# NuTufts/ubresnet

Hardware: AMD Instinct MI355X
Metric: images/sec, 512x512 U-ResNet train step (fwd+loss+bwd+Adam) (higher is better)
Workload: dtype bf16; 1 GPU; ub_uresnet 3-class ip16 bf16, batch 16 per GPU (global 16), 512x512x1 synthetic LArTPC crops, Adam(1e-5, wd 1e-4); parallelism=dp1, global_batch=16, optimizer=ubresnet_amd.optim.FlatAdam

## Files before the change

include/ubresnet_hip.h:

```cpp
#ifndef UBRESNET_HIP_H
#define UBRESNET_HIP_H

#include <stdint.h>

#ifdef __cplusplus
extern "C" {
#endif

#define UBR_F32 0
#define UBR_BF16 1
#define UBR_F16 2

#define UBR_OK 0
#define UBR_EINVAL (-1)
#define UBR_ELAUNCH (-2)

#define UBR_MAX_TAPS 64
#define UBR_STAT_SLOTS 32
#define UBR_RED_SLOTS 8

typedef struct {
  void* p;
  int64_t sn, sy, sx;
} ubr_tensor;

typedef struct {
  const float* sub;
  const float* scale;
  const float* shift;
  const float* lo;
} ubr_chan_affine;

typedef struct {
  int32_t dtype;
  int32_t N, H, W, Cin;
  ubr_tensor x;
  ubr_chan_affine xf;
  const void* w;
  int32_t Cout, Cout_pad;
  int32_t ntaps;
  int8_t dy[UBR_MAX_TAPS], dx[UBR_MAX_TAPS];
  uint8_t wt[UBR_MAX_TAPS];
  int32_t S, iy0, ix0;
  int32_t OH, OW;
  ubr_tensor y;
  ubr_tensor addend;
  const float* bias;
  double* stats;
  int32_t epilogue;
  int32_t tile_hint;
  int32_t act;
  int32_t pad_;
  const uint8_t* addend_mask;
  ubr_tensor bnb_c;
  const float *bnb_mean, *bnb_scale, *bnb_shift, *bnb_invstd;
  int32_t nphase;
  int32_t phase_tap0[4], phase_ntaps[4];
  int32_t pad3_;
  int64_t phase_yoff[4], phase_aoff[4];
  int32_t stats_slots;
  int32_t pad2_;
} ubr_conv_desc;

int ubr_conv(const ubr_conv_desc* d, void* stream);
void ubr_conv_last_config(int* fw, int* nt, int* twf, int* pipe);
int ubr_conv_last_kernel(char* buf, int n);

int ubr_pack_weights(int dtype, const float* src, void* dst, int M, int Mpad, int Kvalid, int Kpad,
                     int64_t sm, int64_t sk, int ntaps, const int32_t* tapidx_host, void* stream);

typedef struct {
  const float* src;
  void* dst;
  int64_t sm, sk, tap_stride;
  const float* oscale;
  int32_t M, Mpad, Kvalid, KU, ntaps, pad_;
} ubr_pack_item;
int ubr_pack_weights_batched(int dtype, const ubr_pack_item* items_dev, int nitems, void* stream);

typedef struct {
  const float *gamma, *beta, *running_mean, *running_var;
  const float* conv_bias;
  float *scale, *bias;
  int32_t C;
  float eps;
} ubr_bn_fold_item;
int ubr_bn_fold_batched(const ubr_bn_fold_item* items_dev, int nitems, void* stream);

typedef struct {
  int32_t dtype;
  int32_t N, H, W, C;
  int32_t pad_;
  ubr_tensor x;
  const void* w;
  const float* bias;
  ubr_tensor y;
} ubr_aspp_front_desc;
int ubr_aspp_front(const ubr_aspp_front_desc* d, void* stream);

typedef struct {
  int32_t dtype;
  int32_t N, H, W, Cin;
  ubr_tensor x;
  ubr_chan_affine xf;
  int32_t GH, GW, Cout;
  ubr_tensor g;
  int32_t ntaps;
  int8_t dy[UBR_MAX_TAPS], dx[UBR_MAX_TAPS];
  int32_t S, iy0, ix0;
  float* slabs;
  int32_t nsplit;
  int32_t exclusive;
} ubr_wgrad_desc;

int ubr_wgrad_plan(const ubr_wgrad_desc* d, int32_t* nsplit, int64_t* workspace_bytes);
int ubr_wgrad(const ubr_wgrad_desc* d, void* stream);
void ubr_wgrad_last_config(int* ma, int* nb, int* tpg, int* nsplit_mode, int* bigx);
int ubr_wgrad_last_pc(void);
int ubr_wgrad_reduce(float* slabs , int nsplit, int ntaps, int Cout_pad, int Cin,
                     int Cout_valid, int Cin_valid, float* dst, int64_t sm, int64_t sk,
                     const int32_t* tapidx_host, int accumulate, void* stream);
#define UBR_REDUCE_BATCH 16
typedef struct {
  float* slabs;
  float* dst;
  int32_t nsplit, ntaps, Cout_pad, Cin, Cout_valid, Cin_valid, accumulate, pad_;
  int64_t sm, sk;
  int32_t tapidx[UBR_MAX_TAPS];
} ubr_wgrad_reduce_item;
int ubr_wgrad_reduce_batched(const ubr_wgrad_reduce_item* items_host, int nitems, void* stream);

int ubr_stem_forward(int dtype, const float* x_nchw, int N, int Cin, int H, int W,
                     const float* weight , const float* bias, int Cout,
                     ubr_tensor y, double* stats, void* stream);
int ubr_stem_wgrad(int dtype, const float* x_nchw, int N, int Cin, int H, int W, ubr_tensor g, int Cout,
                   float* partial , int64_t partial_bytes, float* dweight, float* dbias,
                   int accumulate, void* stream);
int64_t ubr_stem_wgrad_workspace(int N, int Cin, int H, int W, int Cout);
int ubr_stem_expand(int dtype, const float* x_nchw, int N, int Cin, int H, int W, void* out, int64_t out_ps, void* stream);

int ubr_bn_finalize(const double* stats, double count, const float* gamma, const float* beta,
                    float* running_mean, float* running_var, int64_t* num_batches_tracked,
                    float momentum, float eps, int C,
                    float* scale, float* shift, float* mean, float* invstd, void* stream);
int ubr_bn_eval_affine(const float* gamma, const float* beta, const float* running_mean,
                       const float* running_var, float eps, int C, float* scale, float* shift,
                       float* mean, float* invstd, void* stream);

int ubr_bn_bwd_reduce(int dtype, int64_t npix, int C, const void* ga, int64_t ga_ps, const void* ga2, int64_t ga2_ps,
                      const void* c, int64_t c_ps, const float* scale, const float* shift, const float* mean,
                      const float* invstd, int relu, double* red, void* stream);
int ubr_bn_bwd_finalize(const double* red, double count, const float* scale , const float* invstd,
                        int C, float* dgamma, float* dbeta, int accumulate, float* k1, float* k2, void* stream);
int ubr_bn_bwd_apply(int dtype, int64_t npix, int C, const void* ga, int64_t ga_ps, const void* ga2, int64_t ga2_ps,
                     const void* c, int64_t c_ps, const float* scale, const float* shift, const float* mean,
                     const float* invstd, int relu, const float* k1, const float* k2,
                     void* gc, int64_t gc_ps, void* stream);

int ubr_bn_bwd_apply_fin(int dtype, int64_t npix, int C, const void* ga, int64_t ga_ps, const void* ga2, int64_t ga2_ps,
                         const void* c, int64_t c_ps, const float* scale, const float* shift, const float* mean,
                         const float* invstd, int relu, const double* red, double count, float* dgamma, float* dbeta,
                         void* gc, int64_t gc_ps, void* stream);

int ubr_block_tail_fwd(int dtype, int64_t npix, int C, const void* c2, int64_t c2_ps, const float* mean2,
                       const float* scale2, const float* shift2, const void* sc, int64_t sc_ps, const float* mean_b,
                       const float* scale_b, const float* shift_b ,
                       void* out, int64_t out_ps, void* stream);
int ubr_block_tail_bwd_reduce(int dtype, int64_t npix, int C, const void* go, int64_t go_ps, const void* go2, int64_t go2_ps,
                              const void* out, int64_t out_ps, const void* c2, int64_t c2_ps,
                              const float* scale2, const float* shift2, const float* mean2, const float* invstd2,
                              const void* cb, int64_t cb_ps, const float* mean_b, const float* invstd_b,
                              double* red2, double* red_b, void* stream);
int ubr_block_tail_bwd_apply(int dtype, int64_t npix, int C, const void* go, int64_t go_ps, const void* go2, int64_t go2_ps,
                             const void* out, int64_t out_ps, const void* c2, int64_t c2_ps,
                             const float* scale2, const float* shift2, const float* mean2, const float* invstd2,
                             const float* k1_2, const float* k2_2,
                             const void* cb, int64_t cb_ps, const float* scale_b, const float* mean_b, const float* invstd_b,
                             const float* k1_b, const float* k2_b,
                             void* g_c2, int64_t g_c2_ps, void* g_sc, int64_t g_sc_ps, void* stream);

typedef struct {
  const double* stats;
  const float *gamma, *beta;
  float *running_mean, *running_var; int64_t* num_batches_tracked;
  float momentum, eps;
  float *scale, *shift, *mean, *invstd;
} ubr_bn_fwd_fin;
int ubr_block_tail_fwd_fin(int dtype, int64_t npix, int C, const void* c2, int64_t c2_ps, const ubr_bn_fwd_fin* bn2,
                           const void* sc, int64_t sc_ps, const ubr_bn_fwd_fin* bn_b, double count,
                           void* out, int64_t out_ps, uint8_t* relu_mask, void* stream);

int ubr_block_tail_fwd_masked(int dtype, int64_t npix, int C, const void* c2, int64_t c2_ps, const float* mean2,
                              const float* scale2, const float* shift2, const void* sc, int64_t sc_ps, const float* mean_b,
                              const float* scale_b, const float* shift_b, void* out, int64_t out_ps, uint8_t* relu_mask, void* stream);
int ubr_block_tail_bwd_reduce_masked(int dtype, int64_t npix, int C, const void* go, int64_t go_ps, const void* go2, int64_t go2_ps,
                                     const uint8_t* relu_mask, const void* c2, int64_t c2_ps,
                                     const float* scale2, const float* shift2, const float* mean2, const float* invstd2,
                                     const void* cb, int64_t cb_ps, const float* mean_b, const float* invstd_b,
                                     double* red2, double* red_b, void* stream);
int ubr_block_tail_bwd_apply_masked(int dtype, int64_t npix, int C, const void* go, int64_t go_ps, const void* go2, int64_t go2_ps,
                                    const uint8_t* relu_mask, const void* c2, int64_t c2_ps,
                                    const float* scale2, const float* shift2, const float* mean2, const float* invstd2,
                                    const float* k1_2, const float* k2_2,
                                    const void* cb, int64_t cb_ps, const float* scale_b, const float* mean_b, const float* invstd_b,
                                    const float* k1_b, const float* k2_b,
                                    void* g_c2, int64_t g_c2_ps, void* g_sc, int64_t g_sc_ps, void* stream);

int ubr_block_tail_bwd_apply_fin(int dtype, int64_t npix, int C, const void* go, int64_t go_ps, const void* go2, int64_t go2_ps,
                                 const uint8_t* relu_mask, const void* c2, int64_t c2_ps,
                                 const float* scale2, const float* shift2, const float* mean2, const float* invstd2,
                                 const double* red2, float* dgamma2, float* dbeta2,
                                 const void* cb, int64_t cb_ps, const float* scale_b, const float* mean_b, const float* invstd_b,
                                 const double* red_b, float* dgamma_b, float* dbeta_b, double count,
                                 void* g_c2, int64_t g_c2_ps, void* g_sc, int64_t g_sc_ps, void* stream);

int ubr_bn_bwd_frozen(int dtype, int64_t npix, int C, const void* ga, int64_t ga_ps, const void* ga2, int64_t ga2_ps,
                      const void* c, int64_t c_ps, const float* scale, const float* shift, const float* mean,
// ... 63 lines not shown
```

ubresnet_amd/_lib.py:

```python
from __future__ import annotations

import ctypes as C
import os
import threading

import torch

HERE = os.path.dirname(os.path.abspath(__file__))
LIB_PATH = os.environ.get("UBR_LIB", os.path.join(HERE, "libubresnet_hip.so"))

F32, BF16, F16 = 0, 1, 2
MAX_TAPS = 64
MAX_TILES = 64
STAT_SLOTS = 32
RED_SLOTS = 8
_DT = {torch.float32: F32, torch.bfloat16: BF16, torch.float16: F16}
_CPU = {F32: 4, BF16: 8, F16: 8}


def dtype_id(dt: torch.dtype) -> int:
    try:
        return _DT[dt]
    except KeyError:
        raise RuntimeError("ubresnet_amd: unsupported compute dtype %s" % dt)


def chans_per_unit(dt: torch.dtype) -> int:
    return _CPU[dtype_id(dt)]


class Tensor(C.Structure):
    _fields_ = [("p", C.c_void_p), ("sn", C.c_int64), ("sy", C.c_int64), ("sx", C.c_int64)]


class ChanAffine(C.Structure):
    _fields_ = [("sub", C.c_void_p), ("scale", C.c_void_p), ("shift", C.c_void_p), ("lo", C.c_void_p)]


class ConvDesc(C.Structure):
    _fields_ = [
        ("dtype", C.c_int32),
        ("N", C.c_int32), ("H", C.c_int32), ("W", C.c_int32), ("Cin", C.c_int32),
        ("x", Tensor),
        ("xf", ChanAffine),
        ("w", C.c_void_p),
        ("Cout", C.c_int32), ("Cout_pad", C.c_int32),
        ("ntaps", C.c_int32),
        ("dy", C.c_int8 * MAX_TAPS), ("dx", C.c_int8 * MAX_TAPS),
        ("wt", C.c_uint8 * MAX_TAPS),
        ("S", C.c_int32), ("iy0", C.c_int32), ("ix0", C.c_int32),
        ("OH", C.c_int32), ("OW", C.c_int32),
        ("y", Tensor),
        ("addend", Tensor),
        ("bias", C.c_void_p),
        ("stats", C.c_void_p),
        ("epilogue", C.c_int32),
        ("tile_hint", C.c_int32),
        ("act", C.c_int32),
        ("pad_", C.c_int32),
        ("addend_mask", C.c_void_p),
        ("bnb_c", Tensor),
        ("bnb_mean", C.c_void_p), ("bnb_scale", C.c_void_p), ("bnb_shift", C.c_void_p), ("bnb_invstd", C.c_void_p),
        ("nphase", C.c_int32), ("phase_tap0", C.c_int32 * 4), ("phase_ntaps", C.c_int32 * 4), ("pad3_", C.c_int32),
        ("phase_yoff", C.c_int64 * 4), ("phase_aoff", C.c_int64 * 4),
        ("stats_slots", C.c_int32), ("pad2_", C.c_int32),
    ]


class AsppFrontDesc(C.Structure):
    _fields_ = [
        ("dtype", C.c_int32),
        ("N", C.c_int32), ("H", C.c_int32), ("W", C.c_int32), ("C", C.c_int32),
        ("pad_", C.c_int32),
        ("x", Tensor),
        ("w", C.c_void_p),
        ("bias", C.c_void_p),
        ("y", Tensor),
    ]


class BnFwdFin(C.Structure):
    _fields_ = [
        ("stats", C.c_void_p), ("gamma", C.c_void_p), ("beta", C.c_void_p),
        ("running_mean", C.c_void_p), ("running_var", C.c_void_p), ("num_batches_tracked", C.c_void_p),
        ("momentum", C.c_float), ("eps", C.c_float),
        ("scale", C.c_void_p), ("shift", C.c_void_p), ("mean", C.c_void_p), ("invstd", C.c_void_p),
    ]


REDUCE_BATCH = 16


class WgradReduceItem(C.Structure):
    _fields_ = [
        ("slabs", C.c_void_p), ("dst", C.c_void_p),
        ("nsplit", C.c_int32), ("ntaps", C.c_int32), ("Cout_pad", C.c_int32), ("Cin", C.c_int32),
        ("Cout_valid", C.c_int32), ("Cin_valid", C.c_int32), ("accumulate", C.c_int32), ("pad_", C.c_int32),
        ("sm", C.c_int64), ("sk", C.c_int64),
        ("tapidx", C.c_int32 * 64),
    ]


class WgradDesc(C.Structure):
    _fields_ = [
        ("dtype", C.c_int32),
        ("N", C.c_int32), ("H", C.c_int32), ("W", C.c_int32), ("Cin", C.c_int32),
        ("x", Tensor),
        ("xf", ChanAffine),
        ("GH", C.c_int32), ("GW", C.c_int32), ("Cout", C.c_int32),
        ("g", Tensor),
        ("ntaps", C.c_int32),
        ("dy", C.c_int8 * MAX_TAPS), ("dx", C.c_int8 * MAX_TAPS),
        ("S", C.c_int32), ("iy0", C.c_int32), ("ix0", C.c_int32),
        ("slabs", C.c_void_p),
        ("nsplit", C.c_int32),
        ("exclusive", C.c_int32),
    ]


SYMBOLS = [
    "ubr_conv", "ubr_conv_last_config", "ubr_conv_last_kernel", "ubr_pack_weights", "ubr_pack_weights_batched", "ubr_bn_fold_batched", "ubr_aspp_front", "ubr_wgrad_plan", "ubr_wgrad", "ubr_wgrad_last_config", "ubr_wgrad_last_pc", "ubr_wgrad_reduce", "ubr_wgrad_reduce_batched",
    "ubr_stem_forward", "ubr_stem_wgrad", "ubr_stem_wgrad_workspace", "ubr_stem_expand",
    "ubr_bn_finalize", "ubr_bn_eval_affine", "ubr_bn_bwd_reduce", "ubr_bn_bwd_finalize", "ubr_bn_bwd_apply",
    "ubr_block_tail_fwd", "ubr_block_tail_bwd_reduce", "ubr_block_tail_bwd_apply",
    "ubr_block_tail_fwd_masked", "ubr_block_tail_bwd_reduce_masked", "ubr_block_tail_bwd_apply_masked",
    "ubr_bn_bwd_apply_fin", "ubr_block_tail_bwd_apply_fin", "ubr_block_tail_fwd_fin",
    "ubr_bn_bwd_frozen", "ubr_block_tail_bwd_frozen", "ubr_bn_bwd_finalize_frozen",
    "ubr_maxpool_fwd", "ubr_maxpool_bwd",
    "ubr_logsoftmax_bwd", "ubr_pixelwise_nll_fwd", "ubr_pixelwise_nll_bwd", "ubr_confusion",
    "ubr_channel_sum", "ubr_cast_f64_to_f32", "ubr_zero", "ubr_adam_step", "ubr_sgd_step", "ubr_crop_tiles", "ubr_stitch_tiles", "ubr_last_error", "ubr_version",
    "ubr_tape_create", "ubr_tape_destroy", "ubr_tape_begin", "ubr_tape_end", "ubr_tape_pause", "ubr_tape_fork", "ubr_tape_mark",
    "ubr_tape_wait_mark", "ubr_tape_size", "ubr_tape_replay", "ubr_tape_set_label", "ubr_tape_replay_timed",
]

_lib = None
_lock = threading.Lock()
vp, i32, i64, f32, f64 = C.c_void_p, C.c_int32, C.c_int64, C.c_float, C.c_double


def _declare(lib):
    lib.ubr_last_error.restype = C.c_char_p
    lib.ubr_version.restype = C.c_int
    lib.ubr_stem_wgrad_workspace.restype = C.c_int64
    lib.ubr_stem_wgrad_workspace.argtypes = [i32] * 5
    lib.ubr_conv.argtypes = [C.POINTER(ConvDesc), vp]
    lib.ubr_conv_last_config.argtypes = [C.POINTER(C.c_int)] * 4
    lib.ubr_conv_last_kernel.argtypes = [C.c_char_p, i32]
    lib.ubr_conv_last_config.restype = None
    lib.ubr_wgrad_last_config.argtypes = [C.POINTER(C.c_int)] * 5
    lib.ubr_wgrad_last_config.restype = None
    lib.ubr_wgrad_last_pc.argtypes = []
    lib.ubr_wgrad_last_pc.restype = C.c_int
    lib.ubr_pack_weights.argtypes = [i32, vp, vp, i32, i32, i32, i32, i64, i64, i32, C.POINTER(C.c_int32), vp]
    lib.ubr_pack_weights_batched.argtypes = [i32, vp, i32, vp]
    lib.ubr_bn_fold_batched.argtypes = [vp, i32, vp]
    lib.ubr_aspp_front.argtypes = [C.POINTER(AsppFrontDesc), vp]
    lib.ubr_wgrad_plan.argtypes = [C.POINTER(WgradDesc), C.POINTER(C.c_int32), C.POINTER(C.c_int64)]
    lib.ubr_wgrad.argtypes = [C.POINTER(WgradDesc), vp]
    lib.ubr_wgrad_reduce.argtypes = [vp, i32, i32, i32, i32, i32, i32, vp, i64, i64, C.POINTER(C.c_int32), i32, vp]
    lib.ubr_wgrad_reduce_batched.argtypes = [C.POINTER(WgradReduceItem), i32, vp]
    lib.ubr_stem_forward.argtypes = [i32, vp, i32, i32, i32, i32, vp, vp, i32, Tensor, vp, vp]
    lib.ubr_stem_wgrad.argtypes = [i32, vp, i32, i32, i32, i32, Tensor, i32, vp, i64, vp, vp, i32, vp]
    lib.ubr_stem_expand.argtypes = [i32, vp, i32, i32, i32, i32, vp, i64, vp]
    lib.ubr_bn_finalize.argtypes = [vp, f64, vp, vp, vp, vp, vp, f32, f32, i32, vp, vp, vp, vp, vp]
    lib.ubr_bn_eval_affine.argtypes = [vp, vp, vp, vp, f32, i32, vp, vp, vp, vp, vp]
    lib.ubr_bn_bwd_reduce.argtypes = [i32, i64, i32, vp, i64, vp, i64, vp, i64, vp, vp, vp, vp, i32, vp, vp]
    lib.ubr_bn_bwd_finalize.argtypes = [vp, f64, vp, vp, i32, vp, vp, i32, vp, vp, vp]
    lib.ubr_bn_bwd_apply.argtypes = [i32, i64, i32, vp, i64, vp, i64, vp, i64, vp, vp, vp, vp, i32, vp, vp, vp, i64, vp]
    lib.ubr_bn_bwd_apply_fin.argtypes = [i32, i64, i32, vp, i64, vp, i64, vp, i64, vp, vp, vp, vp, i32, vp, f64, vp, vp, vp, i64, vp]
    lib.ubr_block_tail_bwd_apply_fin.argtypes = [i32, i64, i32, vp, i64, vp, i64, vp, vp, i64, vp, vp, vp, vp, vp, vp, vp,
                                                 vp, i64, vp, vp, vp, vp, vp, vp, f64, vp, i64, vp, i64, vp]
    lib.ubr_bn_bwd_frozen.argtypes = [i32, i64, i32, vp, i64, vp, i64, vp, i64, vp, vp, vp, vp, i32, vp, vp, i64, vp]
    lib.ubr_block_tail_bwd_frozen.argtypes = [i32, i64, i32, vp, i64, vp, i64, vp, vp, i64, vp, vp, vp, vp, vp,
                                              vp, i64, vp, vp, vp, vp, vp, i64, vp, i64, vp]
    lib.ubr_bn_bwd_finalize_frozen.argtypes = [vp, i32, vp, vp, vp, vp, vp]
    lib.ubr_block_tail_fwd_fin.argtypes = [i32, i64, i32, vp, i64, C.POINTER(BnFwdFin), vp, i64, C.POINTER(BnFwdFin), f64, vp, i64, vp, vp]
    lib.ubr_block_tail_fwd.argtypes = [i32, i64, i32, vp, i64, vp, vp, vp, vp, i64, vp, vp, vp, vp, i64, vp]
    lib.ubr_block_tail_fwd_masked.argtypes = [i32, i64, i32, vp, i64, vp, vp, vp, vp, i64, vp, vp, vp, vp, i64, vp, vp]
    lib.ubr_block_tail_bwd_reduce_masked.argtypes = [i32, i64, i32, vp, i64, vp, i64, vp, vp, i64, vp, vp, vp, vp, vp, i64, vp, vp, vp, vp, vp]
    lib.ubr_block_tail_bwd_apply_masked.argtypes = [i32, i64, i32, vp, i64, vp, i64, vp, vp, i64, vp, vp, vp, vp, vp, vp, vp, i64, vp, vp, vp, vp, vp,
                                                    vp, i64, vp, i64, vp]
    lib.ubr_block_tail_bwd_reduce.argtypes = [i32, i64, i32, vp, i64, vp, i64, vp, i64, vp, i64, vp, vp, vp, vp,
                                              vp, i64, vp, vp, vp, vp, vp]
    lib.ubr_block_tail_bwd_apply.argtypes = [i32, i64, i32, vp, i64, vp, i64, vp, i64, vp, i64, vp, vp, vp, vp, vp, vp,
                                             vp, i64, vp, vp, vp, vp, vp, vp, i64, vp, i64, vp]
    lib.ubr_maxpool_fwd.argtypes = [i32, i32, i32, i32, i32, i32, vp, i64, ChanAffine, vp, i64, vp, i64, vp, vp]
    lib.ubr_maxpool_bwd.argtypes = [i32, i32, i32, i32, i32, i32, vp, i64, ChanAffine, vp, i64, vp, i64, vp, i64, vp, vp]
    lib.ubr_logsoftmax_bwd.argtypes = [i32, i32, i32, i32, i32, vp, vp, vp, i64, vp]
    lib.ubr_pixelwise_nll_fwd.argtypes = [vp, vp, vp, vp, i32, i32, i32, i32, i64, vp, vp, vp]
    lib.ubr_pixelwise_nll_bwd.argtypes = [vp, vp, vp, vp, i32, i32, i32, i32, i64, vp, vp]
    lib.ubr_confusion.argtypes = [vp, vp, i32, i32, i32, i32, vp, vp]
    lib.ubr_channel_sum.argtypes = [i32, i64, i32, vp, i64, vp, vp]
    lib.ubr_cast_f64_to_f32.argtypes = [vp, i32, i32, vp, i32, f64, i32, vp]
    lib.ubr_zero.argtypes = [vp, i64, vp]
    lib.ubr_adam_step.argtypes = [vp, vp, vp, vp, i64, f32, f32, f32, f32, f32, i64, f32, vp]
    lib.ubr_sgd_step.argtypes = [vp, vp, vp, i64, f32, f32, f32, f32, i32, i32, f32, vp]
    lib.ubr_crop_tiles.argtypes = [vp, i32, i32, i32, C.POINTER(C.c_int32), i32, i32, i32, vp, vp]
    lib.ubr_stitch_tiles.argtypes = [vp, i32, i32, i32, C.POINTER(C.c_int32), i32, vp, i32, i32, i32, vp]
    lib.ubr_tape_create.argtypes = []
    lib.ubr_tape_create.restype = vp
    lib.ubr_tape_destroy.argtypes = [vp]
    lib.ubr_tape_destroy.restype = None
    lib.ubr_tape_begin.argtypes = [vp, i32, C.POINTER(vp)]
    lib.ubr_tape_end.argtypes = [vp]
    lib.ubr_tape_pause.argtypes = [vp, i32]
    lib.ubr_tape_fork.argtypes = [vp, i32, i32]
    lib.ubr_tape_mark.argtypes = [vp, i32]
    lib.ubr_tape_wait_mark.argtypes = [vp, i32, vp]
    lib.ubr_tape_size.argtypes = [vp]
    lib.ubr_tape_replay.argtypes = [vp, i32, C.POINTER(vp)]
    lib.ubr_tape_set_label.argtypes = [vp, i32]
    lib.ubr_tape_replay_timed.argtypes = [vp, i32, C.POINTER(vp), C.POINTER(C.c_float), C.POINTER(C.c_int32), i32]
    for name in SYMBOLS:
        fn = getattr(lib, name)
        if name not in ("ubr_last_error", "ubr_version", "ubr_stem_wgrad_workspace", "ubr_conv_last_config", "ubr_wgrad_last_config",
                        "ubr_tape_create", "ubr_tape_destroy"):
            fn.restype = C.c_int


def lib():
    global _lib
    if _lib is None:
        with _lock:
            if _lib is None:
                if not os.path.exists(LIB_PATH):
                    raise RuntimeError(
                        "ubresnet_amd: HIP extension %s is missing; build it with "
                        "`python -m ubresnet_amd.build` (hipcc, gfx950). There is no CPU fallback." % LIB_PATH)
                try:
                    l = C.CDLL(LIB_PATH)
                except OSError as e:
                    raise RuntimeError("ubresnet_amd: cannot load %s: %s" % (LIB_PATH, e))
                _declare(l)
                _lib = l
    return _lib


def check(rc: int, what: str = ""):
    if rc != 0:
        msg = lib().ubr_last_error().decode("utf-8", "replace")
        raise RuntimeError("ubresnet_amd HIP call failed (%d) %s: %s" % (rc, what, msg))


_raw_stream = getattr(torch._C, "_cuda_getCurrentRawStream", None)


def stream_ptr() -> int:
    if _raw_stream is not None:
        return _raw_stream(torch.cuda.current_device())
    return torch.cuda.current_stream().cuda_stream


def require_cuda(t: torch.Tensor, what: str):
    if not t.is_cuda:
        raise RuntimeError("ubresnet_amd: %s must live on a ROCm device (got %s); the HIP path has no CPU fallback"
                           % (what, t.device))


def ptr(t):
    return None if t is None else t.data_ptr()
```

ubresnet_amd/csrc/ubr_conv.hip:

```cpp
#include <stdlib.h>
#include <type_traits>
#include "ubr_common.h"
#include "ubr_host.h"

namespace {

struct ConvK {
  const char* x; long x_sn, x_sy, x_sx;
  const float *in_sub, *in_scale, *in_shift, *in_lo;
  const char* w;
  char* y; long y_sn, y_sy, y_sx;
  const char* ad; long a_sn, a_sy, a_sx;
  const float* bias;
  double* stats;
  int H, W;
  int CU, UPB, lgUPB, nblk;
  int Cout, Cout_pad;
  int ntaps, S, iy0, ix0, OH, OW;
  int dymin, dxmin, HH, HW;
  int tiles_x, tiles_y;
  unsigned tx_magic, ty_magic;
  int nunits, steps;
  int pixb;
  unsigned rw, rw_magic;
  int x_sy32, x_sx32;
  int step_j, step_hy, step_goff, wrap_goff;
  int wl_off, halo_off, red_off, xfc_off;
  int epilogue, act, wide_store, dbg, wlinear, N;
  int buf_stride, ncot;
  const uint8_t* ad_mask; int ad_mask_cu;
  const char* bc; long bc_sn, bc_sy, bc_sx;
  const float *bmean, *bscale, *bshift, *binvstd;
  int nslots;
  int pair_store;
  int fast_epi;
  int ptap0[4], pnunits[4], psteps[4];
  long pyoff[4], paoff[4];
  int8_t dy[UBR_MAX_TAPS], dx[UBR_MAX_TAPS];
  uint8_t wt[UBR_MAX_TAPS];
  unsigned long long* stamps;
};

template <typename T> __device__ __forceinline__ void store4(char* p, const float* v);
template <> __device__ __forceinline__ void store4<float>(char* p, const float* v) {
  *reinterpret_cast<float4*>(p) = make_float4(v[0], v[1], v[2], v[3]);
}
template <> __device__ __forceinline__ void store4<bf16_t>(char* p, const float* v) {
  *reinterpret_cast<uint2*>(p) = make_uint2(ET<bf16_t>::pk2(v[0], v[1]), ET<bf16_t>::pk2(v[2], v[3]));
}
template <> __device__ __forceinline__ void store4<f16_t>(char* p, const float* v) {
  f16x4_t h; h[0] = (_Float16)v[0]; h[1] = (_Float16)v[1]; h[2] = (_Float16)v[2]; h[3] = (_Float16)v[3];
  *reinterpret_cast<uint2*>(p) = __builtin_bit_cast(uint2, h);
}
template <typename T> __device__ __forceinline__ void load4(const char* p, float* v);
template <> __device__ __forceinline__ void load4<float>(const char* p, float* v) {
  float4 f = *reinterpret_cast<const float4*>(p); v[0] = f.x; v[1] = f.y; v[2] = f.z; v[3] = f.w;
}
template <> __device__ __forceinline__ void load4<bf16_t>(const char* p, float* v) {
  uint2 u = *reinterpret_cast<const uint2*>(p);
  v[0] = __uint_as_float(u.x << 16); v[1] = __uint_as_float(u.x & 0xffff0000u);
  v[2] = __uint_as_float(u.y << 16); v[3] = __uint_as_float(u.y & 0xffff0000u);
}
template <> __device__ __forceinline__ void load4<f16_t>(const char* p, float* v) {
  f16x4_t h = __builtin_bit_cast(f16x4_t, *reinterpret_cast<const uint2*>(p));
  v[0] = (float)h[0]; v[1] = (float)h[1]; v[2] = (float)h[2]; v[3] = (float)h[3];
}

template <typename T> __device__ __forceinline__ void round4(const float* v, float* r);
template <> __device__ __forceinline__ void round4<float>(const float* v, float* r) { r[0] = v[0]; r[1] = v[1]; r[2] = v[2]; r[3] = v[3]; }
template <> __device__ __forceinline__ void round4<bf16_t>(const float* v, float* r) {
#pragma unroll
  for (int i = 0; i < 4; ++i) {
    const uint32_t u = __float_as_uint(v[i]);
    const uint32_t rne = (u + 0x7fffu + ((u >> 16) & 1u)) & 0xffff0000u;
    r[i] = __uint_as_float((u & 0x7fffffffu) > 0x7f800000u ? (u | 0x00400000u) & 0xffff0000u : rne);
  }
}
template <> __device__ __forceinline__ void round4<f16_t>(const float* v, float* r) {
#pragma unroll
  for (int i = 0; i < 4; ++i) r[i] = (float)(_Float16)v[i];
}
__device__ __forceinline__ void bnb_accumulate(const float* g, const float* c, const float4& mu, const float4& sc, const float4& sh, const float4& is,
                                               float* s1, float* s2) {
  const float m[4] = {mu.x, mu.y, mu.z, mu.w}, a[4] = {sc.x, sc.y, sc.z, sc.w}, b[4] = {sh.x, sh.y, sh.z, sh.w}, iv[4] = {is.x, is.y, is.z, is.w};
#pragma unroll
  for (int r = 0; r < 4; ++r) {
    const float d = c[r] - m[r];
    const float bn = __builtin_fmaf(d, a[r], b[r]);
    const float xh = d * iv[r];
    const float gy = bn > 0.f ? g[r] : 0.f;
    s1[r] += gy;
    s2[r] += gy * xh;
  }
}

__host__ __device__ constexpr int conv_pixb(int upb) { return upb == 2 ? 32 : upb * 16 + 16; }

#ifndef UBR_THIN_PIXB4
#define UBR_THIN_PIXB4 80
#endif
__host__ __device__ constexpr int thin_pixb(int upb) { return upb == 4 ? UBR_THIN_PIXB4 : conv_pixb(upb); }

__host__ __device__ constexpr int conv_pipe_hslots(int fw, int twf) { return ((4 * fw / twf + 2) * (twf * 16 + 2) * 4 + 255) / 256; }
__host__ __device__ constexpr int conv_pipe_wslots(int nt) { return (36 * nt * 16 + 255) / 256; }

template <typename T> __device__ __forceinline__ uint4 pack_swap_pair(const float* v0, const float* v1);
template <> __device__ __forceinline__ uint4 pack_swap_pair<bf16_t>(const float* v0, const float* v1) {
  uint2 X, Y;
  asm volatile("v_cvt_pk_bf16_f32 %0, %4, %5\n\tv_cvt_pk_bf16_f32 %1, %6, %7\n\tv_cvt_pk_bf16_f32 %2, %8, %9\n\t"
               "v_cvt_pk_bf16_f32 %3, %10, %11\n\ts_nop 1\n\tv_permlane16_swap_b32 %0, %2\n\tv_permlane16_swap_b32 %1, %3\n\ts_nop 3"
               : "=&v"(X.x), "=&v"(X.y), "=&v"(Y.x), "=&v"(Y.y)
               : "v"(v0[0]), "v"(v0[1]), "v"(v0[2]), "v"(v0[3]), "v"(v1[0]), "v"(v1[1]), "v"(v1[2]), "v"(v1[3]));
  return make_uint4(X.x, X.y, Y.x, Y.y);
}
template <> __device__ __forceinline__ uint4 pack_swap_pair<f16_t>(const float* v0, const float* v1) {
  f16x4_t a, b;
#pragma unroll
  for (int r = 0; r < 4; ++r) { a[r] = (_Float16)v0[r]; b[r] = (_Float16)v1[r]; }
  uint2 X = __builtin_bit_cast(uint2, a), Y = __builtin_bit_cast(uint2, b);
  asm volatile("s_nop 1\n\tv_permlane16_swap_b32 %0, %1\n\tv_permlane16_swap_b32 %2, %3\n\ts_nop 3" : "+v"(X.x), "+v"(Y.x), "+v"(X.y), "+v"(Y.y));
  return make_uint4(X.x, X.y, Y.x, Y.y);
}
template <> __device__ __forceinline__ uint4 pack_swap_pair<float>(const float* v0, const float* v1) { return make_uint4(0u, 0u, 0u, 0u); }

template <typename T> __device__ __forceinline__ void store_frag_pair(char* p0, char* p1, bool ok0, bool ok1, const float* v0, const float* v1, int q) {
  if constexpr (std::is_same<T, float>::value) {
    if (ok0) store4<float>(p0, v0);
    if (ok1) store4<float>(p1, v1);
  } else {
    const uint4 v = pack_swap_pair<T>(v0, v1);
    const bool odd = (q & 1) != 0;
    char* p = odd ? (p1 - 8) : p0;
    if (odd ? ok1 : ok0) *reinterpret_cast<uint4*>(p) = v;
  }
}

typedef __attribute__((ext_vector_type(2))) unsigned ubr_u2;
__device__ __forceinline__ unsigned udiv_magic(unsigned n, unsigned magic) { return magic == 0u ? n : __umulhi(n, magic); }

__device__ __forceinline__ void buf_store16(const ubr_u4& v, __amdgpu_buffer_rsrc_t r, int voff, int soff) {
  __builtin_amdgcn_raw_buffer_store_b128(v, r, voff + soff, 0, 0);
}

template <typename T, int FW, int NT, int TWF, bool PIPE>
__global__ __launch_bounds__(256, ((NT == 4 && FW <= 2 && !PIPE) ? 4 : 2)) void conv_igemm_kernel(const ConvK k) {
  ubr_main_prio();
  constexpr int TN = NT * 16;
  constexpr int F = 4 * FW;
  constexpr int TH = F / TWF;
  constexpr int TW = TWF * 16;
  constexpr int CPU = ET<T>::CPU;
  constexpr int ESZ = 16 / CPU;
  static_assert(F % TWF == 0, "tile shape");

  extern __shared__ __attribute__((aligned(16))) char smem[];
  int* tbl = reinterpret_cast<int*>(smem);
  char* wl = smem + k.wl_off;
  char* halo = smem + k.halo_off;
  float* red = reinterpret_cast<float*>(smem + k.red_off);

#ifdef UBR_CONV_STAMPS
  const unsigned long long t_entry = __builtin_amdgcn_s_memtime();
#endif
  const int tid = threadIdx.x, lane = tid & 63, wave = tid >> 6, q = lane >> 4, l16 = lane & 15;
  const int ph = blockIdx.z;
  const int tap0 = k.ptap0[ph], p_nunits = k.pnunits[ph], p_steps = k.psteps[ph];
  char* const yb = k.y + k.pyoff[ph];
  const char* const adb = k.ad != nullptr ? k.ad + k.paoff[ph] : nullptr;
  const unsigned tile_l = blockIdx.x;
  const unsigned tile_r = udiv_magic(tile_l, k.tx_magic);
  const int tx = (int)(tile_l - tile_r * (unsigned)k.tiles_x);
  const int n = (int)udiv_magic(tile_r, k.ty_magic);
  const int ty = (int)(tile_r - (unsigned)n * (unsigned)k.tiles_y);
  const int n0 = blockIdx.y * TN;
  const int tb_tap = min(tap0 + (tid >> k.lgUPB), k.ntaps - 1);
  const int tb_dy = k.dy[tb_tap], tb_dx = k.dx[tb_tap], tb_wt = k.wt[tb_tap];
  const int oy0 = ty * TH, ox0 = tx * TW;
  const int hy0 = oy0 * k.S + k.iy0 + k.dymin, hx0 = ox0 * k.S + k.ix0 + k.dxmin;

  constexpr int HS_P = PIPE ? conv_pipe_hslots(FW, TWF) : 1;
  constexpr int kOOR = (int)0x80000000;
  ubr_u4 hv[HS_P];
  int hoff[HS_P];
  unsigned hok = 0u;
  float xfr[PIPE ? 8 : 1];
  const bool xf_early = PIPE && k.in_scale != nullptr && k.CU * ET<T>::CPU <= 512;
  if constexpr (PIPE) {
    const int c = tid & (k.UPB - 1);
    const int nit = k.HH * (int)k.rw;
    int hy = (int)__umulhi((unsigned)tid, k.rw_magic);
    int j = tid - hy * (int)k.rw;
#pragma unroll
    for (int u = 0; u < HS_P; ++u) {
// ... 374 lines not shown
#pragma unroll
  for (int j = 0; j < NT; ++j) {
    const int ch = n0 + j * 16 + 4 * q;
    float4 bmu = make_float4(0.f, 0.f, 0.f, 0.f), bsc = bmu, bsh = bmu, bis = bmu;
    const bool bnb = k.bc != nullptr && ch < k.Cout;
    if (bnb) {
      bmu = *reinterpret_cast<const float4*>(k.bmean + ch); bsc = *reinterpret_cast<const float4*>(k.bscale + ch);
      bsh = *reinterpret_cast<const float4*>(k.bshift + ch); bis = *reinterpret_cast<const float4*>(k.binvstd + ch);
    }
    auto finish = [&](int i, float* v, int& oy, int& ox) -> bool {
      const int f = wave * FW + i;
      oy = oy0 + f / TWF; ox = ox0 + (f % TWF) * 16 + l16;
      const bool valid = (oy < k.OH) && (ox < k.OW);
#pragma unroll
      for (int r = 0; r < 4; ++r) v[r] = acc[i][j][r] + bs[j][r];
      if (k.act & 1) {
#pragma unroll
        for (int r = 0; r < 4; ++r) v[r] = fmaxf(v[r], 0.f);
      }
      if (adb != nullptr && valid && ch < k.Cout) {
        float a4[4];
        load4<T>(adb + (long)n * k.a_sn + (long)oy * k.a_sy + (long)ox * k.a_sx + (long)ch * ESZ, a4);
        if (k.ad_mask != nullptr) {
          const unsigned mb = (unsigned)k.ad_mask[(((long)n * k.OH + oy) * k.OW + ox) * k.ad_mask_cu + ch / CPU] >> (ch % CPU);
#pragma unroll
          for (int r = 0; r < 4; ++r) a4[r] = ((mb >> r) & 1u) ? a4[r] : 0.f;
        }
#pragma unroll
        for (int r = 0; r < 4; ++r) v[r] += a4[r];
      }
      if (k.act & 2) {
#pragma unroll
        for (int r = 0; r < 4; ++r) v[r] = fmaxf(v[r], 0.f);
      }
      if (k.stats != nullptr && valid) {
        if (k.bc != nullptr) {
          if (bnb) {
            float g4[4], c4[4];
            round4<T>(v, g4);
            load4<T>(k.bc + (long)n * k.bc_sn + (long)oy * k.bc_sy + (long)ox * k.bc_sx + (long)ch * ESZ, c4);
            bnb_accumulate(g4, c4, bmu, bsc, bsh, bis, s1[j], s2[j]);
          }
        } else {
#pragma unroll
          for (int r = 0; r < 4; ++r) { s1[j][r] += v[r]; s2[j][r] += v[r] * v[r]; }
        }
      }
      return valid;
    };
    constexpr bool PAIRS = (FW % 2 == 0) && sizeof(T) == 2;
    if (PAIRS && k.pair_store && k.epilogue == 0) {
#pragma unroll
      for (int i = 0; i < FW; i += 2) {
        float v0[4], v1[4];
        int oy_a, ox_a, oy_b, ox_b;
        const bool ok0 = finish(i, v0, oy_a, ox_a) && ch < k.Cout;
        const bool ok1 = finish(i + (FW > 1 ? 1 : 0), v1, oy_b, ox_b) && ch < k.Cout;
        store_frag_pair<T>(yb + (long)n * k.y_sn + (long)oy_a * k.y_sy + (long)ox_a * k.y_sx + (long)ch * ESZ,
                           yb + (long)n * k.y_sn + (long)oy_b * k.y_sy + (long)ox_b * k.y_sx + (long)ch * ESZ, ok0, ok1, v0, v1, q);
      }
    } else {
#pragma unroll
    for (int i = 0; i < FW; ++i) {
      float v[4];
      int oy, ox;
      const bool valid = finish(i, v, oy, ox);
      if (k.epilogue == 0) {
        if (valid && ch < k.Cout)
          store4<T>(yb + (long)n * k.y_sn + (long)oy * k.y_sy + (long)ox * k.y_sx + (long)ch * ESZ, v);
      } else if (j == 0) {
        float m = -3.0e38f;
#pragma unroll
        for (int r = 0; r < 4; ++r) if (ch + r < k.Cout) m = fmaxf(m, v[r]);
        m = fmaxf(m, __shfl_xor(m, 16, 64));
        m = fmaxf(m, __shfl_xor(m, 32, 64));
        float e = 0.f;
#pragma unroll
        for (int r = 0; r < 4; ++r) if (ch + r < k.Cout) e += expf(v[r] - m);
        e += __shfl_xor(e, 16, 64);
        e += __shfl_xor(e, 32, 64);
        const float lse = m + logf(e);
        if (valid) {
          float* o = reinterpret_cast<float*>(k.y);
#pragma unroll
          for (int r = 0; r < 4; ++r)
            if (ch + r < k.Cout) o[(((long)n * k.Cout + ch + r) * k.OH + oy) * k.OW + ox] = v[r] - lse;
        }
      }
    }
    }
  }

#ifdef UBR_CONV_STAMPS
  const unsigned long long te1 = __builtin_amdgcn_s_memtime();
#endif
  if (k.stats != nullptr) {
#pragma unroll
    for (int j = 0; j < NT; ++j)
#pragma unroll
      for (int r = 0; r < 4; ++r) {
        const float a = wave_quadrow_sum16(s1[j][r]);
        const float b = wave_quadrow_sum16(s2[j][r]);
        if (l16 == 0) {
          red[(wave * TN + j * 16 + 4 * q + r) * 2 + 0] = a;
          red[(wave * TN + j * 16 + 4 * q + r) * 2 + 1] = b;
        }
      }
    __syncthreads();
    if (tid < TN) {
      const int ch = n0 + tid;
      if (ch < k.Cout) {
        double a = 0.0, b = 0.0;
#pragma unroll
        for (int w = 0; w < 4; ++w) { a += (double)red[(w * TN + tid) * 2]; b += (double)red[(w * TN + tid) * 2 + 1]; }
        double* st = k.stats + (size_t)(blockIdx.x % k.nslots) * 2 * k.Cout;
        atomicAdd(&st[ch], a);
        atomicAdd(&st[k.Cout + ch], b);
      }
    }
  }
#ifdef UBR_CONV_STAMPS
  if (PIPE && k.stamps != nullptr) {
    const unsigned long long te2 = __builtin_amdgcn_s_memtime();
    __syncthreads();
    if (tid == 0) {
      unsigned long long* o = k.stamps + ((size_t)blockIdx.y * gridDim.x + blockIdx.x) * 16;
      o[9] = __builtin_amdgcn_s_memtime(); o[11] = te0; o[12] = te1; o[13] = te2;
    }
  }
#endif
}

struct ThinK {
  const char* x; long x_sn; int x_sy, x_sx; unsigned x_bytes;
  const float *in_sub, *in_scale, *in_shift, *in_lo;
  const char* w;
  char* y; long y_sn; int y_sy, y_sx; unsigned y_bytes;
  const char* ad; long a_sn; int a_sy, a_sx; unsigned a_bytes;
  const float* bias; double* stats;
  int H, W, HW, nitems; unsigned hw_magic;
  int tiles_x, tiles_y, ntiles; unsigned tx_magic, ty_magic;
  int steps, nunits, hy_org, hx_org, dymin, dxmin;
  int Cout, Cout_pad, CU, OH, OW;
  int act, epilogue, wlinear, dbg;
  int wl_off, halo_off, red_off;
  int8_t dy[UBR_MAX_TAPS], dx[UBR_MAX_TAPS];
  uint8_t wt[UBR_MAX_TAPS];
  unsigned long long* stamps;
  const uint8_t* ad_mask; int ad_mask_cu; unsigned mask_bytes;
  const char* bc; long bc_sn; int bc_sy, bc_sx; unsigned bc_bytes;
  const float *bmean, *bscale, *bshift, *binvstd;
  int nslots;
  int nphase, pstep0[4], psteps[4], pyoff[4];
};


template <typename T, int FW, int NT, int TWF, int UPB, bool XF, bool LSM, bool ROW7 = false, int EXT = 0>
__global__ __launch_bounds__(256, ((ROW7 || (EXT == 1 && NT == 2)) ? 2 : 3)) void conv_thin_kernel(const ThinK k) {
  ubr_main_prio();
  static_assert(EXT == 0 || (!XF && !LSM), "the training epilogues belong to the data-gradient convs (no transform on load, NHWC output)");
  constexpr int TN = NT * 16;
  constexpr int TH = 4 * FW / TWF;
  constexpr int TW = TWF * 16;
  constexpr int CPU = ET<T>::CPU;
  constexpr int ESZ = 16 / CPU;
  constexpr int LG = UPB == 4 ? 2 : (UPB == 2 ? 1 : 0);
  constexpr int PIXB = thin_pixb(UPB);
  constexpr int HS = ROW7 ? 7 : (UPB == 4 ? 6 : 5);
  constexpr int PPS = 256 / UPB;
  constexpr int WB = 4;
  constexpr int FH = ROW7 ? 8 : 4;
  static_assert(TWF == 2 && FW % FH == 0, "tile shape");
  static_assert(!ROW7 || (FW == 8 && NT == 1 && UPB == 2), "ROW7 is the 16x32-pixel, 16-cout, 16-cin tile");
  constexpr bool WIDE = ESZ == 2;

  extern __shared__ __attribute__((aligned(16))) char smem[];
  int* tbl = reinterpret_cast<int*>(smem);
  char* wl = smem + k.wl_off;
  char* halo = smem + k.halo_off;
  float* red = reinterpret_cast<float*>(smem + k.red_off);

  const int tid = threadIdx.x, lane = tid & 63, wave = tid >> 6, q = lane >> 4, l16 = lane & 15;
  const int n0 = blockIdx.y * TN;
  const int c = tid & (UPB - 1);
  const int nw = 4 * k.steps * TN;

  int hxu[HS], relu[HS];
  int hyu[XF ? HS : 1];
#pragma unroll
  for (int u = 0; u < HS; ++u) {
    const int pix = (tid >> LG) + u * PPS;
    const int hy = (int)udiv_magic((unsigned)pix, k.hw_magic), hx = pix - hy * k.HW;
    const bool in = tid + u * 256 < k.nitems;
    hxu[u] = in ? hx : -(1 << 24);
    relu[u] = hy * k.x_sy + hx * k.x_sx + c * 16;
    if constexpr (XF) hyu[u] = hy;
  }
  char* const halo_w = halo + (tid >> LG) * PIXB + c * 16;

  ubr_u4 hv[HS];
  unsigned hok = 0u;
  auto load_halo = [&](int tile) {
    const unsigned t = (unsigned)__builtin_amdgcn_readfirstlane(tile);
    const unsigned r = udiv_magic(t, k.tx_magic), tx = t - r * (unsigned)k.tiles_x;
    const unsigned n = udiv_magic(r, k.ty_magic), ty = r - n * (unsigned)k.tiles_y;
    const int hy0 = (int)ty * TH + k.hy_org, hx0 = (int)tx * TW + k.hx_org;
    __amdgpu_buffer_rsrc_t xr = __builtin_amdgcn_make_buffer_rsrc((void*)(k.x + (long)n * k.x_sn), 0, (int)k.x_bytes, 0x00020000);
    const int goff = hy0 * k.x_sy + hx0 * k.x_sx;
    hok = 0u;
#pragma unroll
    for (int u = 0; u < HS; ++u) {
      const bool ok = (unsigned)(hx0 + hxu[u]) < (unsigned)k.W;
      int vo = ok ? relu[u] + goff : -1;
      if (k.dbg & 1) vo = -1;
      hv[u] = __builtin_amdgcn_raw_buffer_load_b128(xr, vo, 0, 0);
      if constexpr (XF) hok |= (unsigned)(ok & ((unsigned)(hy0 + hyu[u]) < (unsigned)k.H)) << u;
    }
  };

  const int ntiles = k.ntiles;
  int tile = blockIdx.x;
  load_halo(tile);
  uint4 wv[WB];
  if (k.wlinear) {
    const int nvalid = k.nunits * TN;
#pragma unroll
    for (int u = 0; u < WB; ++u) {
      const int i = tid + u * 256;
      wv[u] = make_uint4(0u, 0u, 0u, 0u);
      if (i < nvalid) wv[u] = ldg16(k.w + (long)i * 16);
    }
  }
  float bs[NT][4];
#pragma unroll
  for (int j = 0; j < NT; ++j)
#pragma unroll
    for (int r = 0; r < 4; ++r) {
      const int ch = n0 + j * 16 + 4 * q + r;
      bs[j][r] = (k.bias != nullptr && ch < k.Cout) ? k.bias[ch] : 0.f;
    }
  float* xfc = red + 4 * TN * 2;
  if constexpr (XF) {
    for (int i = tid; i < 4 * UPB * CPU; i += 256) {
      const int which = i / (UPB * CPU), ch = i - which * (UPB * CPU);
      const float* src = which == 0 ? k.in_sub : (which == 1 ? k.in_scale : (which == 2 ? k.in_shift : k.in_lo));
      xfc[i] = src[ch];
    }
  }
  if constexpr (EXT == 1) {
    for (int i = tid; i < 4 * TN; i += 256) {
      const int which = i / TN, ch = n0 + (i - which * TN);
      const float* src = which == 0 ? k.bmean : (which == 1 ? k.bscale : (which == 2 ? k.bshift : k.binvstd));
      xfc[i] = ch < k.Cout ? src[ch] : 0.f;
    }
  }
  int* wsrc = tbl + 4 * k.steps;
  for (int u = tid; u < 4 * k.steps; u += 256) {
    int off = 0, v = -1;
    if (u < k.nunits) {
      const int tap = u >> LG, cc = u & (UPB - 1);
      off = ((k.dy[tap] - k.dymin) * k.HW + (k.dx[tap] - k.dxmin)) * PIXB + cc * 16;
      v = k.wt[tap] == 255 ? -1 : ((int)k.wt[tap] * k.CU + cc) * k.Cout_pad;
    }
    tbl[u] = off;
    wsrc[u] = v;
  }
  if (k.wlinear) {
#pragma unroll
    for (int u = 0; u < WB; ++u) {
      const int i = tid + u * 256;
      if (i < nw) *reinterpret_cast<uint4*>(wl + (long)i * 16) = wv[u];
    }
    const int nvalid = k.nunits * TN;
    for (int ib = tid + 256 * WB; ib < nw; ib += 256 * WB) {
#pragma unroll
      for (int u = 0; u < WB; ++u) {
        const int i = ib + u * 256;
        wv[u] = make_uint4(0u, 0u, 0u, 0u);
        if (i < nvalid) wv[u] = ldg16(k.w + (long)i * 16);
      }
#pragma unroll
      for (int u = 0; u < WB; ++u) {
        const int i = ib + u * 256;
        if (i < nw) *reinterpret_cast<uint4*>(wl + (long)i * 16) = wv[u];
      }
    }
  } else {
    __syncthreads();
    for (int ib = tid; ib < nw; ib += 256 * WB) {
#pragma unroll
      for (int u = 0; u < WB; ++u) {
        const int i = ib + u * 256;
        wv[u] = make_uint4(0u, 0u, 0u, 0u);
        if (i < nw) {
          const int src = wsrc[i / TN];
          if (src >= 0) wv[u] = ldg16(k.w + ((long)(src + n0 + (i % TN))) * 16);
        }
      }
#pragma unroll
      for (int u = 0; u < WB; ++u) {
        const int i = ib + u * 256;
        if (i < nw) *reinterpret_cast<uint4*>(wl + (long)i * 16) = wv[u];
      }
    }
  }

  if constexpr (XF || EXT == 1) __syncthreads();
  const int fb0 = (((wave * FW) / TWF) * k.HW + l16) * PIXB;
  const int rowb = k.HW * PIXB;
  int vo_out[NT];
#pragma unroll
  for (int j = 0; j < NT; ++j) {
    if constexpr (WIDE) vo_out[j] = ((wave * FW) / TWF) * k.y_sy + ((q & 1) * 16 + l16) * k.y_sx + (n0 + j * 16 + 8 * (q >> 1)) * ESZ;
    else vo_out[j] = ((wave * FW) / TWF) * k.y_sy + l16 * k.y_sx + (n0 + j * 16 + 4 * q) * ESZ;
  }
  int vo_ad[NT];
#pragma unroll
  for (int j = 0; j < NT; ++j) vo_ad[j] = ((wave * FW) / TWF) * k.a_sy + l16 * k.a_sx + (n0 + j * 16 + 4 * q) * ESZ;
  int vo_c[EXT == 1 ? NT : 1], vo_m[EXT == 2 ? NT : 1];
  if constexpr (EXT == 1) {
#pragma unroll
    for (int j = 0; j < NT; ++j) vo_c[j] = ((wave * FW) / TWF) * k.bc_sy + l16 * k.bc_sx + (n0 + j * 16 + 4 * q) * ESZ;
  }
  if constexpr (EXT == 2) {
#pragma unroll
    for (int j = 0; j < NT; ++j) vo_m[j] = (((wave * FW) / TWF) * k.OW + l16) * k.ad_mask_cu + (n0 + j * 16 + 4 * q) / CPU;
  }
  float s1[NT][4], s2[NT][4];
#pragma unroll
  for (int j = 0; j < NT; ++j)
#pragma unroll
    for (int r = 0; r < 4; ++r) { s1[j][r] = 0.f; s2[j][r] = 0.f; }

#ifdef UBR_CONV_STAMPS
  unsigned long long tS = 0, tL = 0, tC = 0, tE = 0, tB = 0, tW = 0, t_ = __builtin_amdgcn_s_memtime();
  const unsigned long long t_begin = t_;
#define UBR_TSTAMP(acc_) do { unsigned long long n_ = __builtin_amdgcn_s_memtime(); acc_ += n_ - t_; t_ = n_; } while (0)
#else
#define UBR_TSTAMP(acc_) do { } while (0)
#endif
  while (tile < ntiles) {
#ifdef UBR_CONV_STAMPS
    asm volatile("s_waitcnt vmcnt(0)" ::: "memory");
    UBR_TSTAMP(tW);
#endif
    float xsub[XF ? CPU : 1], xsc[XF ? CPU : 1], xsh[XF ? CPU : 1], xlo[XF ? CPU : 1];
    if constexpr (XF) {
#pragma unroll
      for (int e = 0; e < CPU; ++e) {
        xsub[e] = xfc[0 * UPB * CPU + c * CPU + e]; xsc[e] = xfc[1 * UPB * CPU + c * CPU + e];
        xsh[e] = xfc[2 * UPB * CPU + c * CPU + e]; xlo[e] = xfc[3 * UPB * CPU + c * CPU + e];
      }
    }
#pragma unroll
    for (int u = 0; u < HS; ++u) {
      uint4 v = __builtin_bit_cast(uint4, hv[u]);
      if constexpr (XF) {
        if ((hok >> u) & 1u) {
          float f[CPU];
          ET<T>::unpack(v, f);
          ubr_bnrelu<CPU>(f, xsub, xsc, xsh, xlo);
          v = ET<T>::pack(f);
        }
      }
      if (tid + u * 256 < k.nitems) *reinterpret_cast<uint4*>(halo_w + u * (PPS * PIXB)) = v;
    }
    UBR_TSTAMP(tS);
    __syncthreads();
    UBR_TSTAMP(tB);
    const unsigned t = (unsigned)__builtin_amdgcn_readfirstlane(tile);
    const unsigned rr = udiv_magic(t, k.tx_magic), tx = t - rr * (unsigned)k.tiles_x;
    const unsigned n = udiv_magic(rr, k.ty_magic), ty = rr - n * (unsigned)k.tiles_y;
    const int oy0 = (int)ty * TH, ox0 = (int)tx * TW;
    const int next = tile + gridDim.x;
    if (next < ntiles) load_halo(next);
    __amdgpu_buffer_rsrc_t yr = __builtin_amdgcn_make_buffer_rsrc((void*)(k.y + (long)n * k.y_sn), 0, (int)k.y_bytes, 0x00020000);
    __amdgpu_buffer_rsrc_t ar = __builtin_amdgcn_make_buffer_rsrc((void*)(k.ad != nullptr ? k.ad + (long)n * k.a_sn : k.x), 0, k.ad != nullptr ? (int)k.a_bytes : 0, 0x00020000);
    const int ybase = oy0 * k.y_sy + ox0 * k.y_sx, abase = oy0 * k.a_sy + ox0 * k.a_sx;
    __amdgpu_buffer_rsrc_t cr = yr, mr = yr;
    int cbase = 0, mbase = 0;
    if constexpr (EXT == 1) {
      cr = __builtin_amdgcn_make_buffer_rsrc((void*)(k.bc + (long)n * k.bc_sn), 0, (int)k.bc_bytes, 0x00020000);
      cbase = oy0 * k.bc_sy + ox0 * k.bc_sx;
    }
    if constexpr (EXT == 2) {
      mr = __builtin_amdgcn_make_buffer_rsrc((void*)(k.ad_mask + (long)n * k.mask_bytes), 0, (int)k.mask_bytes, 0x00020000);
      mbase = (oy0 * k.OW + ox0) * k.ad_mask_cu;
    }
    UBR_TSTAMP(tL);

#pragma unroll 1
    for (int g0 = 0; g0 < FW; g0 += FH) {
      ubr_u4 adv4[FH][NT];
      ubr_u2 adv2[FH][NT];
      if (k.ad != nullptr) {
#pragma unroll
        for (int i = 0; i < FH; ++i)
#pragma unroll
          for (int j = 0; j < NT; ++j) {
            const int so = abase + ((g0 + i) / TWF) * k.a_sy;
            if constexpr (WIDE) adv2[i][j] = __builtin_amdgcn_raw_buffer_load_b64(ar, vo_ad[j] + (i % TWF) * 16 * k.a_sx, so, 0);
            else adv4[i][j] = __builtin_amdgcn_raw_buffer_load_b128(ar, vo_ad[j] + (i % TWF) * 16 * k.a_sx, so, 0);
          }
      }
      unsigned admk[EXT == 2 ? FH : 1][EXT == 2 ? NT : 1];
      ubr_u4 cv4[EXT == 1 ? FH : 1][EXT == 1 ? NT : 1];
      ubr_u2 cv2[EXT == 1 ? FH : 1][EXT == 1 ? NT : 1];
      if constexpr (EXT == 2) {
#pragma unroll
        for (int i = 0; i < FH; ++i)
#pragma unroll
          for (int j = 0; j < NT; ++j)
            admk[i][j] = __builtin_amdgcn_raw_buffer_load_b8(mr, vo_m[j] + (i % TWF) * 16 * k.ad_mask_cu, mbase + ((g0 + i) / TWF) * k.OW * k.ad_mask_cu, 0);
      }
      if constexpr (EXT == 1) {
#pragma unroll
        for (int i = 0; i < FH; ++i)
#pragma unroll
          for (int j = 0; j < NT; ++j) {
            const int so = cbase + ((g0 + i) / TWF) * k.bc_sy;
            if constexpr (WIDE) cv2[i][j] = __builtin_amdgcn_raw_buffer_load_b64(cr, vo_c[j] + (i % TWF) * 16 * k.bc_sx, so, 0);
            else cv4[i][j] = __builtin_amdgcn_raw_buffer_load_b128(cr, vo_c[j] + (i % TWF) * 16 * k.bc_sx, so, 0);
          }
      }
      const int nph = (ROW7 || LSM || EXT != 0) ? 1 : k.nphase;
#pragma unroll 1
      for (int ph = 0; ph < nph; ++ph) {
      const int s_lo = nph > 1 ? k.pstep0[ph] : 0;
      const int s_cnt = nph > 1 ? k.psteps[ph] : k.steps;
      const int y_ph = nph > 1 ? k.pyoff[ph] : 0;
      f32x4 acc[FH][NT];
#pragma unroll
      for (int i = 0; i < FH; ++i)
#pragma unroll
        for (int j = 0; j < NT; ++j) acc[i][j] = f32x4{0.f, 0.f, 0.f, 0.f};
      const char* hb = halo + fb0 + (g0 / TWF) * rowb;
      if constexpr (ROW7) {
        constexpr int ROWB = (TW + 6) * PIXB;
#pragma unroll 1
        for (int pp = 0; pp < 4; ++pp) {
          const char* pb = hb + tbl[4 * pp + q];
          const char* pw = wl + ((4 * pp + q) * TN + l16) * 16;
          uint4 w7[7];
#pragma unroll
          for (int dy = 0; dy < 7; ++dy) w7[dy] = *reinterpret_cast<const uint4*>(pw + dy * (16 * TN * 16));
#pragma unroll
          for (int ir = 0; ir < 10; ++ir) {
            const uint4 b0 = *reinterpret_cast<const uint4*>(pb + ir * ROWB);
            const uint4 b1 = *reinterpret_cast<const uint4*>(pb + ir * ROWB + 16 * PIXB);
#pragma unroll
            for (int r = 0; r < 4; ++r) {
              const int dy = ir - r;
              if (dy >= 0 && dy <= 6) {
                acc[2 * r][0] = mma_step<T>(acc[2 * r][0], w7[dy], b0);
                acc[2 * r + 1][0] = mma_step<T>(acc[2 * r + 1][0], w7[dy], b1);
              }
            }
          }
        }
      } else {
      int off_n = tbl[4 * s_lo + q];
      uint4 wf_n[NT];
#pragma unroll
      for (int j = 0; j < NT; ++j) wf_n[j] = *reinterpret_cast<const uint4*>(wl + (((4 * s_lo + q) * TN) + j * 16 + l16) * 16);
      const int nsteps = s_lo + ((k.dbg & 2) ? 1 : s_cnt);
      for (int s = s_lo; s < nsteps; ++s) {
        const char* pa = hb + off_n;
        uint4 wf[NT];
#pragma unroll
        for (int j = 0; j < NT; ++j) wf[j] = wf_n[j];
        if (s + 1 < nsteps) {
          off_n = tbl[4 * (s + 1) + q];
#pragma unroll
          for (int j = 0; j < NT; ++j) wf_n[j] = *reinterpret_cast<const uint4*>(wl + (((4 * (s + 1) + q) * TN) + j * 16 + l16) * 16);
        }
        uint4 a[FH];
        a[0] = *reinterpret_cast<const uint4*>(pa);
        a[1] = *reinterpret_cast<const uint4*>(pa + 16 * PIXB);
        a[2] = *reinterpret_cast<const uint4*>(pa + rowb);
        a[3] = *reinterpret_cast<const uint4*>(pa + rowb + 16 * PIXB);
#pragma unroll
        for (int i = 0; i < FH; ++i)
#pragma unroll
          for (int j = 0; j < NT; ++j) acc[i][j] = mma_step<T>(acc[i][j], wf[j], a[i]);
      }
      }
      UBR_TSTAMP(tC);

#pragma unroll
      for (int i = 0; i < FH; i += 2) {
#pragma unroll
        for (int j = 0; j < NT; ++j) {
          float v[2][4];
#pragma unroll
          for (int h = 0; h < 2; ++h) {
#pragma unroll
            for (int r = 0; r < 4; ++r) v[h][r] = acc[i + h][j][r] + bs[j][r];
            if (k.act & 1) {
#pragma unroll
              for (int r = 0; r < 4; ++r) v[h][r] = fmaxf(v[h][r], 0.f);
            }
            if (k.ad != nullptr) {
              float a4[4];
              if constexpr (WIDE) {
                const uint2 raw = make_uint2(adv2[i + h][j][0], adv2[i + h][j][1]);
                load4<T>(reinterpret_cast<const char*>(&raw), a4);
              } else {
                const uint4 raw = __builtin_bit_cast(uint4, adv4[i + h][j]);
                ET<T>::unpack(raw, a4);
              }
              if constexpr (EXT == 2) {
                const unsigned mb = (admk[i + h][j] & 0xffu) >> ((n0 + j * 16 + 4 * q) % CPU);
#pragma unroll
                for (int r = 0; r < 4; ++r) v[h][r] = __builtin_fmaf(a4[r], (float)((mb >> r) & 1u), v[h][r]);
              } else {
#pragma unroll
                for (int r = 0; r < 4; ++r) v[h][r] += a4[r];
              }
// ... 514 lines not shown
#pragma unroll
          for (int j = 0; j < NT; ++j) {
            const int ch = n0 + j * 16 + 4 * q;
            float v[4];
#pragma unroll
            for (int r = 0; r < 4; ++r) v[r] = acc[i2][j][r] + bs[j][r];
            if (k.act & 1) {
#pragma unroll
              for (int r = 0; r < 4; ++r) v[r] = fmaxf(v[r], 0.f);
            }
            if (k.ad != nullptr && valid && ch < k.Cout) {
              float a4[4];
              load4<T>(k.ad + (long)n * k.a_sn + (long)oy * k.a_sy + (long)ox * k.a_sx + (long)ch * ESZ, a4);
#pragma unroll
              for (int r = 0; r < 4; ++r) v[r] += a4[r];
            }
            if (k.act & 2) {
#pragma unroll
              for (int r = 0; r < 4; ++r) v[r] = fmaxf(v[r], 0.f);
            }
            if (k.stats != nullptr && valid) {
#pragma unroll
              for (int r = 0; r < 4; ++r) { s1[j][r] += v[r]; s2[j][r] += v[r] * v[r]; }
            }
            if (valid && ch < k.Cout)
              store4<T>(k.y + (long)n * k.y_sn + (long)oy * k.y_sy + (long)ox * k.y_sx + (long)ch * ESZ, v);
          }
        }
      }
      UBR_PSTAMP(tE);
      __syncthreads();
      UBR_PSTAMP(tB);
    }
    if (k.stats != nullptr && stat_n0 >= 0) flush_stats(stat_n0);
#ifdef UBR_CONV_STAMPS
    UBR_PSTAMP(tE);
    if (k.stamps != nullptr && tid == 0) {
      unsigned long long* o = k.stamps + (size_t)blockIdx.x * 16;
      o[0] = tC; o[1] = tE; o[2] = tB; o[3] = t_ - t_begin; o[4] = (unsigned long long)niter;
    }
#endif
  }
}

static thread_local int g_last_conv_cfg[4] = {0, 0, 0, 0};
static thread_local char g_last_conv_name[160] = "";
struct TileCfg { int FW, NT, TWF; };
static const TileCfg kCfgs[] = {
    {8, 1, 2},
    {4, 1, 2},
    {4, 2, 2},
    {4, 4, 2},
    {2, 4, 1},
    {1, 4, 1},
    {2, 2, 1},
    {2, 1, 1},
    {1, 2, 1},
    {1, 1, 1},
};
constexpr int kNumCfgs = sizeof(kCfgs) / sizeof(kCfgs[0]);

template <typename T, int FW, int NT, int TWF, bool PIPE>
int launch_one(const ConvK& k, dim3 grid, size_t lds, hipStream_t st) {
  auto fn = conv_igemm_kernel<T, FW, NT, TWF, PIPE>;
  if (lds > 64 * 1024) {
    static thread_local size_t maxset = 0;
    if (lds > maxset) {
      hipError_t e = hipFuncSetAttribute(reinterpret_cast<const void*>(fn), hipFuncAttributeMaxDynamicSharedMemorySize, (int)lds);
      if (e != hipSuccess) { ubr_set_error("ubr_conv: cannot raise LDS limit to %zu: %s", lds, hipGetErrorString(e)); return UBR_ELAUNCH; }
      maxset = lds;
    }
  }
  ubr_launch(fn, grid, dim3(256), lds, st, k);
  UBR_LAUNCH_CHECK("ubr_conv");
  return UBR_OK;
}

template <typename T, int FW, int NT, int TWF, int UPB, bool XF, bool LSM = false, bool ROW7 = false, int EXT = 0>
int launch_thin(const ThinK& k, dim3 grid, size_t lds, hipStream_t st) {
  auto fn = conv_thin_kernel<T, FW, NT, TWF, UPB, XF, LSM, ROW7, EXT>;
  if (lds > 64 * 1024) {
    static thread_local size_t maxset = 0;
    if (lds > maxset) {
      hipError_t e = hipFuncSetAttribute(reinterpret_cast<const void*>(fn), hipFuncAttributeMaxDynamicSharedMemorySize, (int)lds);
      if (e != hipSuccess) { ubr_set_error("ubr_conv: cannot raise LDS limit to %zu: %s", lds, hipGetErrorString(e)); return UBR_ELAUNCH; }
      maxset = lds;
    }
  }
  ubr_launch(fn, grid, dim3(256), lds, st, k);
  UBR_LAUNCH_CHECK("ubr_conv");
  return UBR_OK;
}

static unsigned magic_u32(unsigned d) { return d <= 1 ? 0u : (unsigned)((0x100000000ull + d - 1) / d); }

template <typename T, int FW, int NT, int TWF>
int try_thin(const ConvK& c, dim3 grid, hipStream_t st, int* rc) {
  constexpr int TH = 4 * FW / TWF, TW = TWF * 16, TN = NT * 16;
  static const bool thin_on = [] { const char* e = getenv("UBR_CONV_THIN"); return !e || atoi(e) != 0; }();
  const int esz = 16 / ET<T>::CPU;
  if (!thin_on || c.nblk != 1 || c.S != 1 || (c.UPB != 2 && c.UPB != 4)) return 0;
  const int nph = (int)grid.z;
  int steps_tot = c.steps, nunits_tot = c.nunits;
  if (nph > 1) {
    if (nph > 4 || c.ad != nullptr || c.stats != nullptr || c.epilogue != 0 || c.bc != nullptr || c.ad_mask != nullptr) return 0;
    steps_tot = 0; nunits_tot = 0;
    for (int p = 0; p < nph; ++p) {
      if (c.pnunits[p] % 4 || c.ptap0[p] * c.UPB != nunits_tot || c.pyoff[p] < 0 || c.pyoff[p] >= (1L << 30)) return 0;
      steps_tot += c.psteps[p]; nunits_tot += c.pnunits[p];
    }
    if (nunits_tot != c.ntaps * c.UPB) return 0;
  }
  int map7[7][7];
  bool row7 = false;
  if constexpr (FW == 8 && NT == 1 && sizeof(T) == 2) {
    static const bool row7_on = [] { const char* e = getenv("UBR_CONV_ROW7"); return !e || atoi(e) != 0; }();
    row7 = row7_on && c.ntaps == 49 && c.UPB == 2 && c.dymin == -3 && c.dxmin == -3 && c.HW == TW + 6 && c.HH == TH + 6;
    if (row7) {
      for (int a = 0; a < 7; ++a) for (int b = 0; b < 7; ++b) map7[a][b] = -1;
      for (int t = 0; t < 49 && row7; ++t) {
        const int a = c.dy[t] + 3, b = c.dx[t] + 3;
        if (a < 0 || a > 6 || b < 0 || b > 6 || map7[a][b] >= 0 || c.wt[t] == 255) row7 = false; else map7[a][b] = c.wt[t];
      }
    }
  }
  const int HSn = row7 ? 7 : (c.UPB == 4 ? 6 : 5);
  if (c.HH * (int)c.rw > 256 * HSn) return 0;
  if (c.OH % TH || c.OW % TW) return 0;
  if (c.epilogue == 0 && esz == 2 && !c.wide_store) return 0;
  if (c.epilogue == 0 && (c.Cout % 4 || c.Cout_pad != (int)grid.y * TN)) return 0;
  if (c.x_sy >= (1L << 24) || c.y_sy >= (1L << 24) || (long)c.H * c.x_sy >= (1L << 31) || (long)c.OH * c.y_sy >= (1L << 31)) return 0;
  if (c.ad != nullptr && (c.a_sy >= (1L << 24) || (long)c.OH * c.a_sy >= (1L << 31))) return 0;
  const int ntiles = c.tiles_x * c.tiles_y * c.N;
  if ((unsigned long long)ntiles * (unsigned)c.tiles_x >= (1ull << 32)) return 0;
  ThinK k{};
  k.x = c.x; k.x_sn = c.x_sn; k.x_sy = (int)c.x_sy; k.x_sx = (int)c.x_sx; k.x_bytes = (unsigned)((long)c.H * c.x_sy);
  k.in_sub = c.in_sub; k.in_scale = c.in_scale; k.in_shift = c.in_shift; k.in_lo = c.in_lo;
  k.w = c.w;
  k.y = c.y; k.y_sn = c.y_sn; k.y_sy = (int)c.y_sy; k.y_sx = (int)c.y_sx; k.y_bytes = (unsigned)((long)c.OH * c.y_sy);
  k.ad = c.ad; k.a_sn = c.a_sn; k.a_sy = (int)c.a_sy; k.a_sx = (int)c.a_sx; k.a_bytes = c.ad ? (unsigned)((long)c.OH * c.a_sy) : 0u;
  k.bias = c.bias; k.stats = c.stats;
  k.H = c.H; k.W = c.W; k.HW = c.HW; k.nitems = c.HH * (int)c.rw; k.hw_magic = magic_u32((unsigned)c.HW);
  k.tiles_x = c.tiles_x; k.tiles_y = c.tiles_y; k.ntiles = ntiles;
  k.tx_magic = magic_u32((unsigned)c.tiles_x); k.ty_magic = magic_u32((unsigned)c.tiles_y);
  k.steps = steps_tot; k.nunits = nunits_tot; k.hy_org = c.iy0 + c.dymin; k.hx_org = c.ix0 + c.dxmin; k.dymin = c.dymin; k.dxmin = c.dxmin;
  k.nphase = nph;
  for (int p = 0, s0 = 0; p < 4; ++p) {
    k.pstep0[p] = s0; k.psteps[p] = p < nph ? c.psteps[p] : 0; k.pyoff[p] = p < nph ? (int)c.pyoff[p] : 0;
    s0 += k.psteps[p];
  }
  k.Cout = c.Cout; k.Cout_pad = c.Cout_pad; k.CU = c.CU; k.OH = c.OH; k.OW = c.OW;
  k.act = c.act; k.epilogue = c.epilogue; k.wlinear = nph > 1 ? 0 : c.wlinear; k.dbg = c.dbg; k.stamps = c.stamps;
  for (int t = 0; t < c.ntaps; ++t) { k.dy[t] = c.dy[t]; k.dx[t] = c.dx[t]; k.wt[t] = c.wt[t]; }
  const int ext = c.bc != nullptr ? 1 : (c.ad_mask != nullptr ? 2 : 0);
  if (ext != 0 && (c.in_scale != nullptr || c.epilogue != 0)) return 0;
  k.nslots = c.nslots;
  if (ext == 1) {
    if (c.bc_sy >= (1L << 24) || (long)c.OH * c.bc_sy >= (1L << 31)) return 0;
    k.bc = c.bc; k.bc_sn = c.bc_sn; k.bc_sy = (int)c.bc_sy; k.bc_sx = (int)c.bc_sx; k.bc_bytes = (unsigned)((long)c.OH * c.bc_sy);
    k.bmean = c.bmean; k.bscale = c.bscale; k.bshift = c.bshift; k.binvstd = c.binvstd;
  }
  if (ext == 2) {
    if ((long)c.OH * c.OW * c.ad_mask_cu >= (1L << 31)) return 0;
    k.ad_mask = c.ad_mask; k.ad_mask_cu = c.ad_mask_cu; k.mask_bytes = (unsigned)((long)c.OH * c.OW * c.ad_mask_cu);
  }
  if (row7) {
    for (int a = 0; a < 7; ++a)
      for (int b = 0; b < 8; ++b) {
        const int t = a * 8 + b;
        k.dy[t] = (int8_t)(a - 3); k.dx[t] = (int8_t)((b < 7 ? b : 6) - 3); k.wt[t] = (uint8_t)(b < 7 ? map7[a][b] : 255);
      }
    k.nunits = 56 * 2; k.steps = 28; k.wlinear = 0;
  }
  const int pixb = thin_pixb(c.UPB);
  size_t off = ((size_t)2 * 16 * k.steps + 15) & ~(size_t)15;
  k.wl_off = (int)off; off += (size_t)4 * k.steps * TN * 16;
  k.halo_off = (int)off; off += ((size_t)c.HH * c.HW * pixb + 15) & ~(size_t)15;
  k.red_off = (int)off; off += (size_t)4 * TN * 2 * sizeof(float) + (size_t)4 * 4 * 8 * sizeof(float);
  const size_t lds = off;
  if (lds > 150 * 1024) return 0;
  const size_t lds_budget = 159 * 1024;
  static const int wg_per_cu = [] { const char* e = getenv("UBR_CONV_THIN_WGS"); return e ? atoi(e) : 0; }();
  int per_cu = (int)(lds_budget / lds);
  const int reg_cap = (row7 || (ext == 1 && NT == 2)) ? 2 : (NT == 1 ? (ext == 1 ? 3 : 4) : 3);
  if (per_cu > reg_cap) per_cu = reg_cap;
  if (wg_per_cu > 0) per_cu = wg_per_cu;
  if (per_cu < 1) per_cu = 1;
  dim3 g(grid.x, grid.y);
  const unsigned cap = 256u * (unsigned)per_cu / (grid.y ? grid.y : 1);
  if (g.x > cap && cap > 0) g.x = cap;
  g_last_conv_cfg[3] = 2;
  const bool xf = c.in_scale != nullptr;
  snprintf(g_last_conv_name, sizeof(g_last_conv_name), "conv_thin_kernel<%s, %d, %d, %d, %d, %s, %s, false, 0>", sizeof(T) == 4 ? "float" : (std::is_same<T, bf16_t>::value ? "bf16_t" : "f16_t"),
           FW, NT, TWF, c.UPB, xf ? "true" : "false", c.epilogue == 1 ? "true" : "false");
  if (ext != 0)
    snprintf(g_last_conv_name, sizeof(g_last_conv_name), "conv_thin_kernel<%s, %d, %d, %d, %d, false, false, %s, %d>", sizeof(T) == 4 ? "float" : (std::is_same<T, bf16_t>::value ? "bf16_t" : "f16_t"),
             FW, NT, TWF, c.UPB, row7 ? "true" : "false", ext);
  if constexpr (FW == 8 && NT == 1 && sizeof(T) == 2) {
    if (row7) {
      if (ext == 0)
      snprintf(g_last_conv_name, sizeof(g_last_conv_name), "conv_thin_kernel<%s, 8, 1, 2, 2, %s, %s, true, 0>", std::is_same<T, bf16_t>::value ? "bf16_t" : "f16_t",
               xf ? "true" : "false", c.epilogue == 1 ? "true" : "false");
      if (c.epilogue == 1) *rc = xf ? launch_thin<T, 8, 1, 2, 2, true, true, true>(k, g, lds, st) : launch_thin<T, 8, 1, 2, 2, false, true, true>(k, g, lds, st);
      else if (ext == 1) *rc = launch_thin<T, 8, 1, 2, 2, false, false, true, 1>(k, g, lds, st);
      else if (ext == 2) *rc = launch_thin<T, 8, 1, 2, 2, false, false, true, 2>(k, g, lds, st);
      else *rc = xf ? launch_thin<T, 8, 1, 2, 2, true, false, true>(k, g, lds, st) : launch_thin<T, 8, 1, 2, 2, false, false, true>(k, g, lds, st);
      return 1;
    }
  }
  if (c.epilogue == 1) {
    if constexpr (FW == 4 && NT == 1) {
      if (c.UPB != 2) return 0;
      *rc = xf ? launch_thin<T, FW, NT, TWF, 2, true, true>(k, g, lds, st) : launch_thin<T, FW, NT, TWF, 2, false, true>(k, g, lds, st);
      return 1;
    } else {
      return 0;
    }
  }
  if (ext == 1) *rc = c.UPB == 2 ? launch_thin<T, FW, NT, TWF, 2, false, false, false, 1>(k, g, lds, st) : launch_thin<T, FW, NT, TWF, 4, false, false, false, 1>(k, g, lds, st);
  else if (ext == 2) *rc = c.UPB == 2 ? launch_thin<T, FW, NT, TWF, 2, false, false, false, 2>(k, g, lds, st) : launch_thin<T, FW, NT, TWF, 4, false, false, false, 2>(k, g, lds, st);
  else if (c.UPB == 2) *rc = xf ? launch_thin<T, FW, NT, TWF, 2, true>(k, g, lds, st) : launch_thin<T, FW, NT, TWF, 2, false>(k, g, lds, st);
  else *rc = xf ? launch_thin<T, FW, NT, TWF, 4, true>(k, g, lds, st) : launch_thin<T, FW, NT, TWF, 4, false>(k, g, lds, st);
  return 1;
}

template <typename T, int FW, int NT, int TWF>
int launch_cfg(const ConvK& k, dim3 grid, size_t lds, hipStream_t st) {
  if constexpr (NT <= 2 && TWF == 2) {
    int rc = UBR_OK;
    if (try_thin<T, FW, NT, TWF>(k, grid, st, &rc)) return rc;
  }
  if constexpr (NT == 4) {
    static const bool enabled = [] { const char* e = getenv("UBR_CONV_PIPE"); return !e || atoi(e) != 0; }();
    if (enabled && k.nblk >= 2 && k.HH * (int)k.rw <= 256 * conv_pipe_hslots(FW, TWF) && 4 * k.steps * NT * 16 <= 256 * conv_pipe_wslots(NT))
      { g_last_conv_cfg[3] = 1; return launch_one<T, FW, NT, TWF, true>(k, grid, lds, st); }
  }
  g_last_conv_cfg[3] = 0;
  return launch_one<T, FW, NT, TWF, false>(k, grid, lds, st);
}

template <typename T, int FW, int TWF, int STEPS>
int launch_pc_steps(const ConvK& k, dim3 grid, size_t lds, hipStream_t st) {
  auto fn = conv_pc_kernel<T, FW, TWF, STEPS>;
  if (lds > 64 * 1024) {
    static thread_local size_t maxset = 0;
    if (lds > maxset) {
      hipError_t e = hipFuncSetAttribute(reinterpret_cast<const void*>(fn), hipFuncAttributeMaxDynamicSharedMemorySize, (int)lds);
      if (e != hipSuccess) { ubr_set_error("ubr_conv: cannot raise LDS limit to %zu: %s", lds, hipGetErrorString(e)); return UBR_ELAUNCH; }
      maxset = lds;
    }
  }
  ubr_launch(fn, grid, dim3(512), lds, st, k);
  UBR_LAUNCH_CHECK("ubr_conv");
  return UBR_OK;
}

template <typename T, int FW, int TWF>
int launch_pc_one(const ConvK& k, dim3 grid, size_t lds, hipStream_t st) {
  if (k.steps == 9) return launch_pc_steps<T, FW, TWF, 9>(k, grid, lds, st);
  if (k.steps == 4) return launch_pc_steps<T, FW, TWF, 4>(k, grid, lds, st);
  return launch_pc_steps<T, FW, TWF, 0>(k, grid, lds, st);
}

template <typename T>
int launch_pc(int pi, const ConvK& k, dim3 grid, size_t lds, hipStream_t st) {
  g_last_conv_cfg[3] = 3;
  switch (pi) {
    case 0: return launch_pc_one<T, 4, 2>(k, grid, lds, st);
    case 1: return launch_pc_one<T, 2, 2>(k, grid, lds, st);
    case 2: return launch_pc_one<T, 4, 1>(k, grid, lds, st);
    case 3: return launch_pc_one<T, 2, 1>(k, grid, lds, st);
  }
  ubr_set_error("ubr_conv: bad producer/consumer tile %d", pi);
  return UBR_EINVAL;
}

template <typename T>
int launch_T(int cfg, const ConvK& k, dim3 grid, size_t lds, hipStream_t st) {
  if (cfg >= 100) return launch_pc<T>(cfg - 100, k, grid, lds, st);
  switch (cfg) {
    case 0: return launch_cfg<T, 8, 1, 2>(k, grid, lds, st);
    case 1: return launch_cfg<T, 4, 1, 2>(k, grid, lds, st);
    case 2: return launch_cfg<T, 4, 2, 2>(k, grid, lds, st);
    case 3: return launch_cfg<T, 4, 4, 2>(k, grid, lds, st);
    case 4: return launch_cfg<T, 2, 4, 1>(k, grid, lds, st);
    case 5: return launch_cfg<T, 1, 4, 1>(k, grid, lds, st);
    case 6: return launch_cfg<T, 2, 2, 1>(k, grid, lds, st);
    case 7: return launch_cfg<T, 2, 1, 1>(k, grid, lds, st);
    case 8: return launch_cfg<T, 1, 2, 1>(k, grid, lds, st);
    case 9: return launch_cfg<T, 1, 1, 1>(k, grid, lds, st);
  }
  ubr_set_error("ubr_conv: bad tile config %d", cfg);
  return UBR_EINVAL;
}

struct Plan { int cfg; size_t lds; int UPB, steps, HH, HW, pixb, wl_off, halo_off, red_off, xfc_off, tiles_x, tiles_y, pc_buf; };

static int eff_ntaps(const ubr_conv_desc* d) {
  if (d->nphase <= 1) return d->ntaps;
  int m = 0;
  for (int p = 0; p < d->nphase && p < 4; ++p) m = d->phase_ntaps[p] > m ? d->phase_ntaps[p] : m;
  return m;
}

static bool plan_tile(const ubr_conv_desc* d, int cfg, int TH, int TW, int TN, int dymin, int dymax, int dxmin, int dxmax, Plan* p) {
  if (d->Cout_pad % TN) return false;
  if (d->epilogue == 1 && TN != 16) return false;
  const int cpu = ubr_cpu(d->dtype);
  const int CU = d->Cin / cpu;
  int UPB = (CU % 4 == 0) ? 4 : (CU % 2 == 0 ? 2 : 1);
  if (UPB == 4 && (d->S == 2 || eff_ntaps(d) >= 16)) UPB = 2;
  const int nunits = eff_ntaps(d) * UPB;
  const int steps = (nunits + 3) / 4;
  const int HH = (TH - 1) * d->S + 1 + (dymax - dymin);
  const int HW = (TW - 1) * d->S + 1 + (dxmax - dxmin);
  const int pixb = conv_pixb(UPB);
  size_t off = ((size_t)2 * 16 * steps + 15) & ~(size_t)15;
  p->wl_off = (int)off; off += (size_t)4 * steps * TN * 16;
  p->halo_off = (int)off; off += (size_t)HH * HW * pixb;
  off = (off + 15) & ~(size_t)15;
  p->red_off = (int)off; off += (size_t)4 * TN * 2 * sizeof(float);
  p->xfc_off = (int)off;
  if (d->xf.scale != nullptr && CU / UPB >= 2) off += (size_t)d->Cin * 4 * sizeof(float);
  p->cfg = cfg; p->lds = off; p->UPB = UPB; p->steps = steps; p->HH = HH; p->HW = HW; p->pixb = pixb;
  p->tiles_x = ubr_cdiv(d->OW, TW); p->tiles_y = ubr_cdiv(d->OH, TH);
  if ((size_t)HH * HW * UPB >= 60000) return false;
  return off <= 160 * 1024;
}

static bool plan_for(const ubr_conv_desc* d, int cfg, int dymin, int dymax, int dxmin, int dxmax, Plan* p) {
  const TileCfg& c = kCfgs[cfg];
  return plan_tile(d, cfg, 4 * c.FW / c.TWF, c.TWF * 16, c.NT * 16, dymin, dymax, dxmin, dxmax, p);
}

struct PcCfg { int FW, TWF; };
static const PcCfg kPc[] = {
    {4, 2},
    {2, 2},
    {4, 1},
    {2, 1},
};
constexpr int kNumPc = sizeof(kPc) / sizeof(kPc[0]);

static bool plan_pc(const ubr_conv_desc* d, int pi, int dymin, int dymax, int dxmin, int dxmax, Plan* p) {
  const PcCfg& c = kPc[pi];
  const int TH = 4 * c.FW / c.TWF, TW = c.TWF * 16, TN = 64;
  const int cpu = ubr_cpu(d->dtype);
  if (d->S != 1 || d->epilogue != 0 || d->ntaps > 9 || d->Cout_pad % TN || d->Cin % (4 * cpu)) return false;
  if (c.TWF == 2 && d->OW < 32) return false;
  const int steps = d->ntaps;
  const int HH = TH + (dymax - dymin), HW = TW + (dxmax - dxmin);
  static const int pixb = [] { const char* e = getenv("UBR_PC_PIXB"); return e ? atoi(e) : 96; }();
  if ((long)HH * HW * 4 > 256L * conv_pipe_hslots(c.FW, c.TWF)) return false;
  if (4L * steps * TN > 256L * conv_pipe_wslots(4)) return false;
  size_t off = ((size_t)2 * 16 * steps + 15) & ~(size_t)15;
  p->wl_off = (int)off;
  const size_t wlb = (size_t)4 * steps * TN * 16;
  p->halo_off = (int)(off + wlb);
  const size_t buf = (wlb + (size_t)HH * HW * pixb + 15) & ~(size_t)15;
  off += 2 * buf;
  p->pc_buf = (int)buf;
  p->red_off = (int)off; off += (size_t)4 * 2 * TN * sizeof(float);
  p->xfc_off = (int)off;
  if (d->xf.scale != nullptr) off += (size_t)d->Cin * 4 * sizeof(float);
  p->cfg = 100 + pi; p->lds = off; p->UPB = 4; p->steps = steps; p->HH = HH; p->HW = HW; p->pixb = pixb;
  p->tiles_x = ubr_cdiv(d->OW, TW); p->tiles_y = ubr_cdiv(d->OH, TH);
  if ((size_t)HH * HW * 4 >= 60000) return false;
  return off <= 160 * 1024;
}

}

extern "C" int ubr_conv_last_kernel(char* buf, int n) {
  if (buf == nullptr || n <= 0) return UBR_EINVAL;
  snprintf(buf, (size_t)n, "%s", g_last_conv_name);
  return UBR_OK;
}

extern "C" void ubr_conv_last_config(int* fw, int* nt, int* twf, int* pipe) {
  if (fw) *fw = g_last_conv_cfg[0];
  if (nt) *nt = g_last_conv_cfg[1];
  if (twf) *twf = g_last_conv_cfg[2];
  if (pipe) *pipe = g_last_conv_cfg[3];
}

static bool thin_eligible(const ubr_conv_desc* d, int cfg, const Plan& p, bool wide_ok) {
  static const bool thin_on = [] { const char* e = getenv("UBR_CONV_THIN"); return !e || atoi(e) != 0; }();
  const TileCfg& c = kCfgs[cfg];
  if (!thin_on || c.TWF != 2 || c.NT > 2 || (c.FW % 4)) return false;
  const int cpu = ubr_cpu(d->dtype), esz = ubr_esize(d->dtype);
  const int CU = d->Cin / cpu, TH = 4 * c.FW / c.TWF, TW = c.TWF * 16;
  if (p.UPB != CU || d->S != 1 || (p.UPB != 2 && p.UPB != 4)) return false;
  if (d->OH % TH || d->OW % TW) return false;
  if (d->nphase > 1) {
    static const bool ph_on = [] { const char* e = getenv("UBR_THIN_PHASES"); return !e || atoi(e) != 0; }();
    if (!ph_on || d->addend.p != nullptr || d->stats != nullptr || d->epilogue != 0) return false;
    int t0 = 0;
    for (int q = 0; q < d->nphase; ++q) {
      if ((d->phase_ntaps[q] * p.UPB) % 4 || d->phase_tap0[q] != t0) return false;
      t0 += d->phase_ntaps[q];
    }
    if (t0 != d->ntaps) return false;
  }
  static const bool row7_on = [] { const char* e = getenv("UBR_CONV_ROW7"); return !e || atoi(e) != 0; }();
  const bool row7 = row7_on && cfg == 0 && esz == 2 && d->ntaps == 49 && p.UPB == 2 && p.HW == TW + 6 && p.HH == TH + 6;
  if ((long)p.HH * p.HW * p.UPB > 256L * (row7 ? 7 : (p.UPB == 4 ? 6 : 5))) return false;
  if (d->epilogue == 1) return (cfg == 1 || row7) && p.UPB == 2;
  if (esz == 2 && !wide_ok) return false;
  return d->Cout % 4 == 0;
}

extern "C" int ubr_conv(const ubr_conv_desc* d, void* stream) {
  UBR_CHECK(d != nullptr, "ubr_conv: null descriptor");
  UBR_CHECK(ubr_dtype_ok(d->dtype), "ubr_conv: bad dtype %d", d->dtype);
  const int cpu = ubr_cpu(d->dtype), esz = ubr_esize(d->dtype);
  UBR_CHECK(d->N > 0 && d->H > 0 && d->W > 0 && d->OH > 0 && d->OW > 0, "ubr_conv: empty extent");
  UBR_CHECK(d->Cin > 0 && d->Cin % cpu == 0, "ubr_conv: Cin=%d must be a positive multiple of %d", d->Cin, cpu);
  UBR_CHECK(d->Cout > 0 && d->Cout_pad % 16 == 0 && d->Cout <= d->Cout_pad && d->Cout_pad - d->Cout < 16,
            "ubr_conv: bad Cout=%d Cout_pad=%d", d->Cout, d->Cout_pad);
  UBR_CHECK(d->ntaps >= 1 && d->ntaps <= UBR_MAX_TAPS, "ubr_conv: ntaps=%d out of range", d->ntaps);
  UBR_CHECK(d->S == 1 || d->S == 2, "ubr_conv: S=%d unsupported", d->S);
  UBR_CHECK(d->x.p && d->w && d->y.p, "ubr_conv: null tensor");
  UBR_CHECK(ubr_aligned16(d->x.p) && ubr_aligned16(d->w), "ubr_conv: x/w must be 16-byte aligned");
  UBR_CHECK((d->x.sx * esz) % 16 == 0 && (d->x.sy * esz) % 16 == 0 && (d->x.sn * esz) % 16 == 0,
            "ubr_conv: input strides must keep 16-byte alignment");
  UBR_CHECK(d->x.sx >= d->Cin, "ubr_conv: x pixel stride %ld < Cin %d", (long)d->x.sx, d->Cin);
  const bool xf = d->xf.scale != nullptr;
  UBR_CHECK(xf == (d->xf.shift != nullptr) && xf == (d->xf.lo != nullptr) && xf == (d->xf.sub != nullptr), "ubr_conv: xf needs sub, scale, shift and lo together");
  if (d->epilogue == 0) {
    UBR_CHECK(d->Cout % 4 == 0, "ubr_conv: NHWC store needs Cout %% 4 == 0 (got %d)", d->Cout);
    UBR_CHECK((((uintptr_t)d->y.p) % (4 * esz)) == 0 && d->y.sx % 4 == 0 && d->y.sy % 4 == 0 && d->y.sn % 4 == 0,
              "ubr_conv: output view must be aligned to 4 elements");
    UBR_CHECK(d->y.sx >= d->Cout, "ubr_conv: y pixel stride %ld < Cout %d", (long)d->y.sx, d->Cout);
    if (d->addend.p)
      UBR_CHECK((((uintptr_t)d->addend.p) % (4 * esz)) == 0 && d->addend.sx % 4 == 0 && d->addend.sy % 4 == 0 && d->addend.sn % 4 == 0,
                "ubr_conv: addend view must be aligned to 4 elements");
  } else {
    UBR_CHECK(d->epilogue == 1 && d->Cout <= 16 && d->Cout_pad == 16, "ubr_conv: log-softmax epilogue needs Cout<=16");
    UBR_CHECK(d->addend.p == nullptr && d->stats == nullptr && d->act == 0, "ubr_conv: log-softmax epilogue takes no addend/stats/act");
  }
  UBR_CHECK((d->act & ~3) == 0, "ubr_conv: bad act flags %d", d->act);
  if (d->addend_mask != nullptr)
    UBR_CHECK(d->addend.p != nullptr && d->epilogue == 0 && d->Cout % cpu == 0 && d->bnb_c.p == nullptr, "ubr_conv: addend_mask needs an addend, NHWC output, whole channel units, and excludes bnb_c");
  if (d->bnb_c.p != nullptr) {
    UBR_CHECK(d->stats != nullptr && d->epilogue == 0 && d->act == 0 && d->Cout % 4 == 0 && d->bnb_mean && d->bnb_scale && d->bnb_shift && d->bnb_invstd,
              "ubr_conv: bnb_c needs stats, the four BatchNorm vectors, NHWC output and no activation");
    UBR_CHECK((((uintptr_t)d->bnb_c.p) % (4 * esz)) == 0 && d->bnb_c.sx % 4 == 0 && d->bnb_c.sy % 4 == 0 && d->bnb_c.sn % 4 == 0 && d->bnb_c.sx >= d->Cout &&
              ubr_aligned16(d->bnb_mean) && ubr_aligned16(d->bnb_scale) && ubr_aligned16(d->bnb_shift) && ubr_aligned16(d->bnb_invstd),
              "ubr_conv: bnb_c view must be aligned to 4 elements, the BatchNorm vectors to 16 bytes");
  }
  const bool train_epi = d->addend_mask != nullptr || d->bnb_c.p != nullptr;
  const int nphase = d->nphase > 1 ? d->nphase : 1;
  if (nphase > 1) {
    UBR_CHECK(nphase <= 4 && d->epilogue == 0 && !train_epi && d->stats == nullptr, "ubr_conv: a phased launch takes 2..4 phases, NHWC output, no statistics or training epilogue");
    int covered = 0;
    for (int p = 0; p < nphase; ++p) {
      UBR_CHECK(d->phase_ntaps[p] >= 1 && d->phase_tap0[p] == covered, "ubr_conv: phase tap ranges must tile [0, ntaps) in order");
      covered += d->phase_ntaps[p];
      UBR_CHECK(d->phase_yoff[p] % 4 == 0 && d->phase_aoff[p] % 4 == 0, "ubr_conv: phase offsets must keep 4-element alignment");
    }
    UBR_CHECK(covered == d->ntaps, "ubr_conv: phase tap ranges must tile [0, ntaps)");
  }
  int dymin = 127, dymax = -128, dxmin = 127, dxmax = -128;
  for (int t = 0; t < d->ntaps; ++t) {
    dymin = d->dy[t] < dymin ? d->dy[t] : dymin; dymax = d->dy[t] > dymax ? d->dy[t] : dymax;
    dxmin = d->dx[t] < dxmin ? d->dx[t] : dxmin; dxmax = d->dx[t] > dxmax ? d->dx[t] : dxmax;
  }
  UBR_CHECK(dymax - dymin <= 16 && dxmax - dxmin <= 16, "ubr_conv: tap extent too large");

  const bool wide_ok = d->epilogue == 0 && esz == 2 && d->Cout % 8 == 0 && (((uintptr_t)d->y.p) % 16) == 0 && (d->y.sx * esz) % 16 == 0 &&
                       (d->y.sy * esz) % 16 == 0 && (d->y.sn * esz) % 16 == 0;
  Plan best{}; bool have = false;
  if (d->tile_hint > 100) {
    UBR_CHECK(d->tile_hint <= 100 + kNumPc && !train_epi, "ubr_conv: tile_hint %d out of range (or a training epilogue on conv_pc_kernel)", d->tile_hint);
    have = plan_pc(d, d->tile_hint - 101, dymin, dymax, dxmin, dxmax, &best);
    UBR_CHECK(have, "ubr_conv: producer/consumer tile_hint %d does not fit this shape", d->tile_hint);
  } else if (d->tile_hint > 0) {
    UBR_CHECK(d->tile_hint <= kNumCfgs, "ubr_conv: tile_hint %d out of range", d->tile_hint);
    have = plan_for(d, d->tile_hint - 1, dymin, dymax, dxmin, dxmax, &best);
    UBR_CHECK(have, "ubr_conv: tile_hint %d does not fit this shape", d->tile_hint);
  } else {
    const int order_by_nt[3][4] = {{3, 4, 5, -1}, {2, 6, 8, -1}, {0, 1, 7, 9}};
    {
      static const int pc_mode = [] { const char* e = getenv("UBR_CONV_PC"); return e ? atoi(e) : 1; }();
      const int nblk_pc = d->Cin / (4 * cpu);
      const bool pick = pc_mode == 2 || (pc_mode == 1 && (nblk_pc <= 2 || (long)d->OH * d->OW <= 256) && !(d->Cin == d->Cout_pad && nblk_pc == 2));
      if (pick && !train_epi && nphase == 1 && d->Cout_pad % 64 == 0 && d->ntaps >= 4) {
        Plan cand{}; bool any = false;
        const int wide[] = {0, 1}, narrow[] = {2, 3};
        const int* ord = d->OW >= 32 ? wide : narrow;
        for (int i = 0; i < 2 && !have; ++i) {
          Plan p{};
          if (!plan_pc(d, ord[i], dymin, dymax, dxmin, dxmax, &p)) continue;
          const long units = (long)p.tiles_x * p.tiles_y * d->N * (d->Cout_pad / 64);
          cand = p; any = true;
          if (units >= 256) { best = p; have = true; }
        }
        if (!have && any) { best = cand; have = true; }
      }
    }
    if (d->Cout_pad <= 32) {
      const int g = d->Cout_pad == 32 ? 1 : 2;
      for (int i = 0; i < 4 && !have; ++i) {
        const int cfg = order_by_nt[g][i];
        if (cfg < 0 || kCfgs[cfg].TWF != 2) continue;
        Plan p{};
        if (!plan_for(d, cfg, dymin, dymax, dxmin, dxmax, &p)) continue;
        if (thin_eligible(d, cfg, p, wide_ok)) { best = p; have = true; }
      }
    }
    for (int g = 0; g < 3 && !have; ++g) {
      Plan cand{}; bool any = false;
      for (int i = 0; i < 4; ++i) {
        const int cfg = order_by_nt[g][i];
        if (cfg < 0) continue;
        Plan p{};
        if (!plan_for(d, cfg, dymin, dymax, dxmin, dxmax, &p)) continue;
        const TileCfg& c = kCfgs[cfg];
        if (c.TWF == 2 && d->OW < 32) continue;
        const long wgs = (long)p.tiles_x * p.tiles_y * d->N * (d->Cout_pad / (c.NT * 16));
        cand = p; any = true;
        if (wgs >= 512 && p.lds <= 80 * 1024) break;
      }
      if (any) { best = cand; have = true; }
    }
    UBR_CHECK(have, "ubr_conv: no tile configuration fits (Cout_pad=%d ntaps=%d)", d->Cout_pad, d->ntaps);
  }

  ConvK k{};
  k.x = (const char*)d->x.p; k.x_sn = d->x.sn * esz; k.x_sy = d->x.sy * esz; k.x_sx = d->x.sx * esz;
  k.in_sub = d->xf.sub; k.in_scale = d->xf.scale; k.in_shift = d->xf.shift; k.in_lo = d->xf.lo;
  k.w = (const char*)d->w;
  k.y = (char*)d->y.p; k.y_sn = d->y.sn * esz; k.y_sy = d->y.sy * esz; k.y_sx = d->y.sx * esz;
  k.ad = (const char*)d->addend.p; k.a_sn = d->addend.sn * esz; k.a_sy = d->addend.sy * esz; k.a_sx = d->addend.sx * esz;
  k.bias = d->bias; k.stats = d->stats;
  k.ad_mask = d->addend_mask; k.ad_mask_cu = d->Cout / cpu;
  k.bc = (const char*)d->bnb_c.p; k.bc_sn = d->bnb_c.sn * esz; k.bc_sy = d->bnb_c.sy * esz; k.bc_sx = d->bnb_c.sx * esz;
  k.bmean = d->bnb_mean; k.bscale = d->bnb_scale; k.bshift = d->bnb_shift; k.binvstd = d->bnb_invstd;
  UBR_CHECK(d->stats_slots == 0 || d->stats_slots == UBR_RED_SLOTS || d->stats_slots == UBR_STAT_SLOTS, "ubr_conv: stats_slots must be 0, %d or %d", UBR_RED_SLOTS, UBR_STAT_SLOTS);
  k.nslots = (d->bnb_c.p != nullptr || d->stats_slots == UBR_RED_SLOTS) ? UBR_RED_SLOTS : UBR_STAT_SLOTS;
  k.H = d->H; k.W = d->W;
  k.CU = d->Cin / cpu; k.UPB = best.UPB; k.lgUPB = ubr_ilog2(best.UPB); k.nblk = k.CU / best.UPB;
  k.Cout = d->Cout; k.Cout_pad = d->Cout_pad;
  k.ntaps = d->ntaps; k.S = d->S; k.iy0 = d->iy0; k.ix0 = d->ix0; k.OH = d->OH; k.OW = d->OW;
  k.dymin = dymin; k.dxmin = dxmin; k.HH = best.HH; k.HW = best.HW;
  k.tiles_x = best.tiles_x; k.tiles_y = best.tiles_y;
  k.tx_magic = magic_u32((unsigned)best.tiles_x); k.ty_magic = magic_u32((unsigned)best.tiles_y);
  k.nunits = eff_ntaps(d) * best.UPB; k.steps = best.steps; k.pixb = best.pixb;
  for (int p = 0; p < 4; ++p) {
    const bool on = p < nphase;
    const int nt = nphase > 1 ? (on ? d->phase_ntaps[p] : 0) : d->ntaps;
    k.ptap0[p] = nphase > 1 && on ? d->phase_tap0[p] : 0;
    k.pnunits[p] = nt * best.UPB;
    k.psteps[p] = (nt * best.UPB + 3) / 4;
    k.pyoff[p] = nphase > 1 && on ? d->phase_yoff[p] * (long)esz : 0;
    k.paoff[p] = nphase > 1 && on ? d->phase_aoff[p] * (long)esz : 0;
  }
  k.rw = (unsigned)(best.HW * best.UPB);
  k.rw_magic = (unsigned)((0x100000000ull + k.rw - 1) / k.rw);
  UBR_CHECK((long)d->H * k.x_sy < (1L << 31) && k.x_sx < (1L << 20), "ubr_conv: image too large for 32-bit offsets");
  k.x_sy32 = (int)k.x_sy; k.x_sx32 = (int)k.x_sx;
  k.step_j = (int)(256 % k.rw); k.step_hy = (int)(256 / k.rw);
  k.step_goff = k.step_hy * k.x_sy32 + (k.step_j >> k.lgUPB) * k.x_sx32;
  k.wrap_goff = k.x_sy32 - best.HW * k.x_sx32;
  k.wl_off = best.wl_off; k.halo_off = best.halo_off; k.red_off = best.red_off; k.xfc_off = best.xfc_off;
  k.epilogue = d->epilogue; k.act = d->act; k.N = d->N;
  {
    bool nat = best.cfg < 100 && d->Cout_pad == kCfgs[best.cfg].NT * 16;
    for (int t = 0; t < d->ntaps && nat; ++t) nat = d->wt[t] == t;
    k.wlinear = nat ? 1 : 0;
  }
#ifdef UBR_CONV_STAMPS
  { static const int dbg = [] { const char* e = getenv("UBR_CONV_DBG"); return e ? atoi(e) : 0; }(); k.dbg = dbg; }
  { static const char* sp = getenv("UBR_CONV_STAMP_PTR"); k.stamps = sp ? (unsigned long long*)strtoull(sp, nullptr, 0) : nullptr; }
#else
  k.dbg = 0; k.stamps = nullptr;
#endif
  k.wide_store = wide_ok ? 1 : 0;
  { static const bool pairs = [] { const char* e = getenv("UBR_CONV_PAIRS"); return e && atoi(e) != 0; }(); k.pair_store = (wide_ok && pairs) ? 1 : 0; }
  {
    static const bool fe = [] { const char* e = getenv("UBR_CONV_FAST_EPI"); return !e || atoi(e) != 0; }();
    const long lim = 1L << 26;
    k.fast_epi = (fe && k.y_sy < lim && (k.ad == nullptr || k.a_sy < lim) && (long)k.OW * k.ad_mask_cu < lim) ? 1 : 0;
  }
  for (int t = 0; t < d->ntaps; ++t) { k.dy[t] = d->dy[t]; k.dx[t] = d->dx[t]; k.wt[t] = d->wt[t]; }

  TileCfg c{};
  int tn;
  if (best.cfg >= 100) { const PcCfg& w = kPc[best.cfg - 100]; c = TileCfg{w.FW, 4, w.TWF}; tn = 64; }
  else { c = kCfgs[best.cfg]; tn = c.NT * 16; }
  g_last_conv_cfg[0] = c.FW; g_last_conv_cfg[1] = c.NT; g_last_conv_cfg[2] = c.TWF;
  dim3 grid((unsigned)(best.tiles_x * best.tiles_y * d->N), (unsigned)(d->Cout_pad / tn), (unsigned)nphase);
  if (best.cfg >= 100) {
    static const int ncu = [] { hipDeviceProp_t pr; int dev = 0; return (hipGetDevice(&dev) == hipSuccess && hipGetDeviceProperties(&pr, dev) == hipSuccess && pr.multiProcessorCount > 0) ? pr.multiProcessorCount : 256; }();
    k.ncot = d->Cout_pad / 64;
    k.buf_stride = best.pc_buf;
    const long units = (long)grid.x * k.ncot;
    UBR_CHECK(units < (1L << 30), "ubr_conv: too many tiles");
    grid = dim3((unsigned)(units < ncu ? units : ncu), 1);
  }
  hipStream_t st = (hipStream_t)stream;
  {
    static const bool dbg = [] { const char* e = getenv("UBR_CONV_DEBUG"); return e && atoi(e) != 0; }();
    if (dbg)
      fprintf(stderr, "ubr_conv plan: N%d %dx%d Cin%d Cout%d taps%d S%d | cfg%d (%d,%d,%d) UPB%d nblk%d lds %zu wgs %u x %u\n", d->N, d->OH, d->OW,
              d->Cin, d->Cout, d->ntaps, d->S, best.cfg, c.FW, c.NT, c.TWF, best.UPB, k.nblk, best.lds, grid.x, grid.y);
  }
  {
    const char* tn = d->dtype == UBR_F32 ? "float" : (d->dtype == UBR_BF16 ? "bf16_t" : "f16_t");
    g_last_conv_name[0] = 0;
    int rc;
    switch (d->dtype) {
      case UBR_F32: rc = launch_T<float>(best.cfg, k, grid, best.lds, st); break;
      case UBR_BF16: rc = launch_T<bf16_t>(best.cfg, k, grid, best.lds, st); break;
      default: rc = launch_T<f16_t>(best.cfg, k, grid, best.lds, st); break;
    }
    if (g_last_conv_name[0] == 0) {
      if (best.cfg >= 100) { const PcCfg& w = kPc[best.cfg - 100]; snprintf(g_last_conv_name, sizeof(g_last_conv_name), "conv_pc_kernel<%s, %d, %d, %d>", tn, w.FW, w.TWF, (best.steps == 9 || best.steps == 4) ? best.steps : 0); }
      else snprintf(g_last_conv_name, sizeof(g_last_conv_name), "conv_igemm_kernel<%s, %d, %d, %d, %s>", tn, c.FW, c.NT, c.TWF, g_last_conv_cfg[3] == 1 ? "true" : "false");
    }
    return rc;
  }
}

namespace {
struct PackK {
  const float* src; char* dst;
  int M, Mpad, Kvalid, KU, ntaps;
  long sm, sk;
  int tapidx[UBR_MAX_TAPS];
};
template <typename T>
__global__ __launch_bounds__(256) void pack_kernel(const PackK k) {
  constexpr int CPU = ET<T>::CPU;
  const long total = (long)k.ntaps * k.KU * k.Mpad;
  for (long i = (long)blockIdx.x * 256 + threadIdx.x; i < total; i += (long)gridDim.x * 256) {
    const int m = (int)(i % k.Mpad);
    long r = i / k.Mpad;
    const int ku = (int)(r % k.KU);
    const int t = (int)(r / k.KU);
    float f[CPU];
#pragma unroll
    for (int e = 0; e < CPU; ++e) {
      const int kc = ku * CPU + e;
      f[e] = (m < k.M && kc < k.Kvalid) ? k.src[(long)m * k.sm + (long)kc * k.sk + k.tapidx[t]] : 0.f;
    }
    *reinterpret_cast<uint4*>(k.dst + i * 16) = ET<T>::pack(f);
  }
}
}

namespace {
constexpr int kPackLdsFloats = 8192;
template <typename T>
__global__ __launch_bounds__(256) void pack_batched_kernel(const ubr_pack_item* items) {
  constexpr int CPU = ET<T>::CPU;
  __shared__ float lds[kPackLdsFloats + 256];
  const ubr_pack_item it = items[blockIdx.y];
  const int nt = it.ntaps;
  const bool modeA = it.tap_stride == 1 && it.sk == nt;
  const bool modeB = it.tap_stride == 1 && it.sm == nt && !modeA;
  if (!modeA && !modeB) {
    const long total = (long)nt * it.KU * it.Mpad;
    for (long i = (long)blockIdx.x * 256 + threadIdx.x; i < total; i += (long)gridDim.x * 256) {
      const int m = (int)(i % it.Mpad);
      long r = i / it.Mpad;
      const int ku = (int)(r % it.KU);
      const int t = (int)(r / it.KU);
      const float sc = (it.oscale != nullptr && m < it.M) ? it.oscale[m] : 1.f;
      float f[CPU];
#pragma unroll
      for (int e = 0; e < CPU; ++e) {
        const int kc = ku * CPU + e;
        f[e] = (m < it.M && kc < it.Kvalid) ? it.src[(long)m * it.sm + (long)kc * it.sk + (long)t * it.tap_stride] * sc : 0.f;
      }
      *reinterpret_cast<uint4*>((char*)it.dst + i * 16) = ET<T>::pack(f);
    }
    return;
  }
  int KB = kPackLdsFloats / (16 * CPU * nt);
  if (KB > it.KU) KB = it.KU;
  if (KB > 16) KB = 16;
  if (KB < 1) KB = 1;
  const int mtiles = it.Mpad / 16, ktiles = (it.KU + KB - 1) / KB;
  for (int tile = blockIdx.x; tile < mtiles * ktiles; tile += gridDim.x) {
    const int m0 = (tile % mtiles) * 16, ku0 = (tile / mtiles) * KB;
    const int kb = min(KB, it.KU - ku0);
    const int k0 = ku0 * CPU;
    const int kn = max(0, min(kb * CPU, it.Kvalid - k0));
    const int mn = max(0, min(16, it.M - m0));
    __syncthreads();
    int rowlen;
    if (modeA) {
      rowlen = (kb * CPU * nt) | 1;
      const int run = kn * nt;
      for (int i = threadIdx.x; i < mn * run; i += 256) {
        const int m = i / run, c = i - m * run;
        lds[m * rowlen + c] = it.src[(long)(m0 + m) * it.sm + (long)k0 * nt + c];
      }
    } else {
      rowlen = (16 * nt) | 1;
      const int run = mn * nt;
      for (int i = threadIdx.x; i < kn * run; i += 256) {
        const int kk = i / run, c = i - kk * run;
        lds[kk * rowlen + c] = it.src[(long)(k0 + kk) * it.sk + (long)m0 * nt + c];
      }
    }
    __syncthreads();
    for (int o = threadIdx.x; o < nt * kb * 16; o += 256) {
      const int m = o & 15;
      const int kul = (o >> 4) % kb, t = (o >> 4) / kb;
      const float sc = (it.oscale != nullptr && m < mn) ? it.oscale[m0 + m] : 1.f;
      float f[CPU];
#pragma unroll
      for (int e = 0; e < CPU; ++e) {
        const int kl = kul * CPU + e;
        float v = 0.f;
        if (m < mn && kl < kn) v = modeA ? lds[m * rowlen + kl * nt + t] : lds[kl * rowlen + m * nt + t];
        f[e] = v * sc;
      }
      *reinterpret_cast<uint4*>((char*)it.dst + (((long)t * it.KU + ku0 + kul) * it.Mpad + m0 + m) * 16) = ET<T>::pack(f);
    }
  }
}

__global__ void bn_fold_batched_kernel(const ubr_bn_fold_item* items) {
  const ubr_bn_fold_item it = items[blockIdx.y];
  for (int c = blockIdx.x * blockDim.x + threadIdx.x; c < it.C; c += gridDim.x * blockDim.x) {
    const double s = (double)it.gamma[c] / sqrt((double)it.running_var[c] + (double)it.eps);
    const double b = it.conv_bias != nullptr ? (double)it.conv_bias[c] : 0.0;
    it.scale[c] = (float)s;
    it.bias[c] = (float)((b - (double)it.running_mean[c]) * s + (double)it.beta[c]);
  }
}
}

extern "C" int ubr_bn_fold_batched(const ubr_bn_fold_item* items_dev, int nitems, void* stream) {
  UBR_CHECK(items_dev != nullptr && nitems >= 1 && nitems <= 65535, "ubr_bn_fold_batched: bad arguments");
  ubr_launch(bn_fold_batched_kernel, dim3(4, (unsigned)nitems), dim3(256), 0, (hipStream_t)stream, items_dev);
  UBR_LAUNCH_CHECK("ubr_bn_fold_batched");
  return UBR_OK;
}

extern "C" int ubr_pack_weights_batched(int dtype, const ubr_pack_item* items_dev, int nitems, void* stream) {
  UBR_CHECK(ubr_dtype_ok(dtype), "ubr_pack_weights_batched: bad dtype");
  UBR_CHECK(items_dev != nullptr && nitems >= 1 && nitems <= 65535, "ubr_pack_weights_batched: bad arguments");
  hipStream_t st = (hipStream_t)stream;
  dim3 grid(128, (unsigned)nitems);
  if (dtype == UBR_F32) ubr_launch(pack_batched_kernel<float>, grid, dim3(256), 0, st, items_dev);
  else if (dtype == UBR_BF16) ubr_launch(pack_batched_kernel<bf16_t>, grid, dim3(256), 0, st, items_dev);
  else ubr_launch(pack_batched_kernel<f16_t>, grid, dim3(256), 0, st, items_dev);
  UBR_LAUNCH_CHECK("ubr_pack_weights_batched");
  return UBR_OK;
}

extern "C" int ubr_pack_weights(int dtype, const float* src, void* dst, int M, int Mpad, int Kvalid, int Kpad,
                                int64_t sm, int64_t sk, int ntaps, const int32_t* tapidx_host, void* stream) {
  UBR_CHECK(ubr_dtype_ok(dtype), "ubr_pack_weights: bad dtype");
  const int cpu = ubr_cpu(dtype);
  UBR_CHECK(src && dst && tapidx_host, "ubr_pack_weights: null pointer");
  UBR_CHECK(M > 0 && Mpad >= M && Mpad % 16 == 0 && Kvalid > 0 && Kpad >= Kvalid && Kpad % cpu == 0,
            "ubr_pack_weights: bad extents M=%d Mpad=%d K=%d Kpad=%d", M, Mpad, Kvalid, Kpad);
  UBR_CHECK(ntaps >= 1 && ntaps <= UBR_MAX_TAPS, "ubr_pack_weights: ntaps out of range");
  UBR_CHECK(ubr_aligned16(dst), "ubr_pack_weights: dst must be 16-byte aligned");
  PackK k{};
  k.src = src; k.dst = (char*)dst; k.M = M; k.Mpad = Mpad; k.Kvalid = Kvalid; k.KU = Kpad / cpu; k.ntaps = ntaps;
  k.sm = sm; k.sk = sk;
  for (int t = 0; t < ntaps; ++t) k.tapidx[t] = tapidx_host[t];
  const long total = (long)ntaps * k.KU * Mpad;
  int blocks = (int)((total + 255) / 256);
  if (blocks > 4096) blocks = 4096;
  hipStream_t st = (hipStream_t)stream;
  if (dtype == UBR_F32) ubr_launch(pack_kernel<float>, dim3(blocks), dim3(256), 0, st, k);
  else if (dtype == UBR_BF16) ubr_launch(pack_kernel<bf16_t>, dim3(blocks), dim3(256), 0, st, k);
  else ubr_launch(pack_kernel<f16_t>, dim3(blocks), dim3(256), 0, st, k);
// ... 4 lines not shown
```

ubresnet_amd/engine.py:

```python
from __future__ import annotations

from typing import Callable, Dict, List, Optional

import torch

from . import _lib as L
from . import ops
from .ops import Affine

T3 = ops.conv_taps(3, 1, 1)
T1 = ops.conv_taps(1, 1, 0)
T7 = ops.conv_taps(7, 1, 3)
DG3 = ops.conv_dgrad_taps_s1(3, 1, 1)
DG1 = ops.conv_dgrad_taps_s1(1, 1, 0)
DG7 = ops.conv_dgrad_taps_s1(7, 1, 3)


import os as _os
_INFER_FOLD = _os.environ.get("UBR_INFER_FOLD", "1") != "0"
_RELU_MASK = _os.environ.get("UBR_RELU_MASK", "1") != "0"
_FIN_MAX_C = int(_os.environ.get("UBR_FIN_MAX_C", "1024"))
_BNB_FUSE = _os.environ.get("UBR_BNB_FUSE", "0") != "0"
_MASK_ADDEND = _os.environ.get("UBR_MASK_ADDEND", "1") != "0"
_WG_MAIN_EVERY = int(_os.environ.get("UBR_WGRAD_MAIN_EVERY", "0"))
_WG_AFTER = _os.environ.get("UBR_WGRAD_ORDER", "before") == "after"
_DEFER_REDUCE = _os.environ.get("UBR_DEFER_REDUCE", "1") != "0"
_TAIL_FIN = _os.environ.get("UBR_TAIL_FIN", "1") != "0"
_PHASE_MIN_C = int(_os.environ.get("UBR_PHASE_MIN_C", "16"))


def _phased(k, pad):
    ph = [(ry, rx, ops.transposed_phase_taps(k, 1, pad, 2, ry, rx)) for ry in range(2) for rx in range(2)]
    ph = [p for p in ph if p[2]]
    return ph, [t for p in ph for t in p[2]]


_PH4 = _phased(4, 1)
_PH3 = _phased(3, 1)


def _phase(t, ry, rx):
    return t[:, ry::2, rx::2, :]


class BNSite:
    __slots__ = ("mod", "C", "stats", "scale", "shift", "mean", "invstd", "red", "k1", "k2", "frozen")

    def __init__(self, mod):
        self.mod = mod
        self.C = mod.num_features
        self.frozen = False


def _module_frozen(mod) -> bool:
    return not mod.training and mod.running_mean is not None and mod.running_var is not None


class Saved:
    pass


class Engine:
    def __init__(self, model, kind: str):
        self.model = model
        self.kind = kind
        self._plans: Dict[tuple, dict] = {}
        self._images: Dict[tuple, torch.Tensor] = {}
        self._const: Dict[tuple, torch.Tensor] = {}
        self.wws = ops.WgradWorkspace()
        self.side = None
        self._side_on = False
        self._wg_count = 0
        self._evs, self._ev_next, self._main = [], 0, None
        self._red_buf, self._red_off, self._red_elems = None, 0, 0
        self._bwd_packed, self._pack_evs = None, None
        self._rec = None
        self._planned: Dict[tuple, object] = {}
        self.wws.pin = True
        self.bn_sites: List[BNSite] = []
        self._bn_of: Dict[int, BNSite] = {}
        for m in model.modules():
            if isinstance(m, torch.nn.BatchNorm2d):
                s = BNSite(m)
                self.bn_sites.append(s)
                self._bn_of[id(m)] = s
        self.grad_order = list(model._grad_completion_order())
        self.grad_offsets = {}
        off = 0
        for name, p in self.grad_order:
            self.grad_offsets[name] = off
            off += (p.numel() + 3) // 4 * 4
        self.grad_numel = off

    def bn(self, mod) -> BNSite:
        return self._bn_of[id(mod)]

    def any_training(self) -> bool:
        return any(not _module_frozen(s.mod) for s in self.bn_sites)

    def frozen_pattern(self, training: bool) -> tuple:
        if training:
            return tuple(_module_frozen(s.mod) for s in self.bn_sites)
        return tuple(s.mod.running_mean is not None and s.mod.running_var is not None for s in self.bn_sites)

    def const(self, device, value: float, n: int) -> torch.Tensor:
        key = (device, value)
        t = self._const.get(key)
        if t is None or t.numel() < n:
            t = torch.full((max(n, 2048),), value, dtype=torch.float32, device=device)
            self._const[key] = t
        return t

    def _new(self, shape, dtype=None, device=None):
        t = torch.empty(shape, dtype=dtype, device=device)
        if self._rec is not None:
            self._rec.keep.append(t)
        return t

    @staticmethod
    def _fresh(shape, dtype=None, device=None):
        return torch.empty(shape, dtype=dtype, device=device)

    def _untaped(self, fn):
        if self._rec is None:
            return fn()
        self._rec.tape.pause()
        try:
            return fn()
        finally:
            self._rec.tape.resume()

    def _fork(self, a, b):
        if self._rec is not None and self._rec.nstreams > 1:
            self._rec.tape.fork(a, b)

    def relu_affine(self, site: BNSite) -> Affine:
        return Affine(site.mean, site.scale, site.shift, self.const(site.scale.device, 0.0, site.C))

    def _plan_items(self):
        m = self.model
        items = []
        conv1 = getattr(m, "conv1", None)
        conv11 = getattr(m, "conv11", None)
        for mod in m.modules():
            if isinstance(mod, torch.nn.ConvTranspose2d):
                w = mod.weight
                d0, d1, kh, kw = w.shape
                kk = kh * kw
                items.append(("fwd", (id(w), "tfwd"), w, 0, d1, d0, None, kk, d1 * kk, kk, 1))
                items.append(("bwd", (id(w), "tdgrad"), w, 0, d0, d1, None, d1 * kk, kk, kk, 1))
            elif isinstance(mod, torch.nn.Conv2d):
                w = mod.weight
                d0, d1, kh, kw = w.shape
                kk = kh * kw
                if mod is conv1 and self.kind != "custom":
                    for ci in range(d1):
                        items.append(("fwd", (id(w), "stem%d" % ci), w, ci * 49, d0, 7, 16, d1 * 49, 1, 7, 7))
                    continue
                items.append(("fwd", (id(w), "fwd"), w, 0, d0, d1, None, d1 * kk, kk, kk, 1))
                if mod is conv11 and self.kind != "custom":
                    items.append(("bwd", (id(w), "dgrad"), w, 0, d1, d0, 16, kk, d1 * kk, kk, 1))
                else:
                    items.append(("bwd", (id(w), "dgrad"), w, 0, d1, d0, None, kk, d1 * kk, kk, 1))
        if self.kind == "custom":
            for mod in m.modules():
                if isinstance(mod, torch.nn.Conv2d) and mod.kernel_size == (7, 7) and mod.in_channels <= 4:
                    w = mod.weight
                    for ci in range(w.shape[1]):
                        items.append(("fwd", (id(w), "stem%d" % ci), w, ci * 49, w.shape[0], 7, 16, w.shape[1] * 49, 1, 7, 7))
        return items

    def _pack_plan(self, dt, device):
        import struct
        key = (dt, device)
        plan = self._plans.get(key)
        ptrs = tuple(p.data_ptr() for _, p in self.grad_order)
        if plan is not None and plan["ptrs"] == ptrs:
            return plan
        cpu = L.chans_per_unit(dt)
        images, tables = {}, {"fwd": b"", "bwd": b""}
        counts = {"fwd": 0, "bwd": 0}
        for group, k, w, soff, M, Kv, Kpad, sm, sk, ntaps, tstride in self._plan_items():
            if not w.is_contiguous() or w.dtype != torch.float32 or w.device != device:
                raise RuntimeError("ubresnet_amd: parameters must be contiguous float32 on %s" % device)
            Mpad = (M + 15) // 16 * 16
            Kp = Kpad if Kpad is not None else (Kv + cpu - 1) // cpu * cpu
            dst = self._new((ntaps, Kp // cpu, Mpad, cpu), dtype=dt, device=device)
            images[k] = dst
            tables[group] += struct.pack("<QQqqqQiiiiii", w.data_ptr() + 4 * soff, dst.data_ptr(), sm, sk, tstride, 0, M, Mpad, Kv, Kp // cpu, ntaps, 0)
            counts[group] += 1
        plan = {"ptrs": ptrs, "images": images, "counts": counts}
        for g in ("fwd", "bwd"):
            plan[g] = torch.frombuffer(bytearray(tables[g]), dtype=torch.uint8).to(device) if counts[g] else None
        self._plans[key] = plan
        return plan

    def pack_all(self, dt, device, group, stream=None):
        plan = self._pack_plan(dt, device)
        if plan["counts"][group]:
            st = L.stream_ptr() if stream is None else stream.cuda_stream
            L.check(L.lib().ubr_pack_weights_batched(L.dtype_id(dt), plan[group].data_ptr(), plan["counts"][group], st),
                    "pack_weights_batched")
        self._images = plan["images"]

    def _pack_bwd_early(self, dt, dev):
        import os
        self._bwd_packed = None
        if dev.type != "cuda" or os.environ.get("UBR_WGRAD_STREAM", "1") == "0":
            return
        self._ensure_side(dev)
        if self._pack_evs is None:
            self._pack_evs = (torch.cuda.Event(), torch.cuda.Event())
        e0, e1 = self._pack_evs
        e0.record(torch.cuda.current_stream(dev))
        self.side.wait_event(e0)
        self._fork(0, 1)
        self.pack_all(dt, dev, "bwd", stream=self.side)
        e1.record(self.side)
        self._bwd_packed = (dt, dev)

    def _pack_bwd(self, dt, dev):
        if self._bwd_packed == (dt, dev):
            torch.cuda.current_stream(dev).wait_event(self._pack_evs[1])
            self._fork(1, 0)
            self._bwd_packed = None
            self._images = self._pack_plan(dt, dev)["images"]
        else:
            self.pack_all(dt, dev, "bwd")

    def packed(self, param: torch.Tensor, dtype, orient: str) -> torch.Tensor:
        return self._images[(id(param), orient)]
# ... 69 lines not shown
            ops.conv(x, self.packed(blk.bypass.weight, dt, "fwd"), cb, T1, Cout, S=S, xf=xf_in, stats=bnb.stats, stats_slots=slots)
            if not fuse:
                self._finish_bn(bnb, cnt, training)
        mask = None
        if self._save and _RELU_MASK:
            mask = self._new((cnt * (Cout // L.chans_per_unit(dt)),), dtype=torch.uint8, device=dev)
        if fuse:
            f2 = ops.bn_fwd_fin(bn2.stats, blk.bn2, bn2.scale, bn2.shift, bn2.mean, bn2.invstd)
            fb = ops.bn_fwd_fin(bnb.stats, blk.bnpass, bnb.scale, bnb.shift, bnb.mean, bnb.invstd) if blk.bypass is not None else None
            ops.block_tail_fwd_fin(c2, f2, cb if blk.bypass is not None else x, fb, cnt, out, relu_mask=mask)
        elif blk.bypass is not None:
            ops.block_tail_fwd(c2, bn2.mean, bn2.scale, bn2.shift, cb, bnb.mean, bnb.scale, bnb.shift, out, relu_mask=mask)
        else:
            ops.block_tail_fwd(c2, bn2.mean, bn2.scale, bn2.shift, x, None, None, None, out, relu_mask=mask)
        if not self._save:
            return None
        rec = Saved()
        rec.blk, rec.x, rec.c1, rec.c2, rec.cb, rec.out, rec.xf_in = blk, x, c1, c2, cb, out, xf_in
        rec.mask = mask
        return rec

    def _red_begin(self, dev):
        if self._red_elems == 0:
            NS = L.STAT_SLOTS
            tot = 0
            for s_ in self.bn_sites:
                tot += 2 * s_.C * NS
            self._red_elems = 2 * tot + 64 * NS * 8
        self._red_buf = self._new(self._red_elems, dtype=torch.float64, device=dev)
        ops.zero_(self._red_buf)
        self._red_off = 0

    def _red(self, n, dev):
        k = L.STAT_SLOTS * n
        if self._red_buf is None or self._red_off + k > self._red_buf.numel() or self._red_buf.device != dev:
            t = ops.stat_buffer(n, dev)
            if self._rec is not None:
                self._rec.keep.append(t)
            return t
        t = self._red_buf[self._red_off:self._red_off + k]
        self._red_off += k
        return t

    def _side_begin(self, dev):
        import os
        self._side_on = dev.type == "cuda" and os.environ.get("UBR_WGRAD_STREAM", "1") != "0"
        self._wg_count = 0
        if self._side_on:
            self._ensure_side(dev)
        if self._side_on:
            self._main = torch.cuda.current_stream(dev)
            self._ev_next = 0

    def _ensure_side(self, dev):
        if self.side is not None:
            return
        import os
        import torch.distributed as _dist
        in_job = _dist.is_available() and _dist.is_initialized()
        prio = int(os.environ.get("UBR_SIDE_PRIORITY", "-1" if in_job else "0"))
        self.side = torch.cuda.Stream(device=dev, priority=prio)

    def _wg_flush(self):
        b = self.__dict__.get("_red_batch")
        if b is not None:
            b.flush()

    def _fin_flush(self):
        pend = self.__dict__.get("_fin_pending")
        if pend:
            for red, site, G in pend:
                ops.bn_bwd_finalize_frozen(red, site.C, G(site.mod.weight), G(site.mod.bias))
            del pend[:]

    def _fin_later(self, red, site, G):
        self.__dict__.setdefault("_fin_pending", []).append((red, site, G))

    def _side_end(self, dev):
        self._fin_flush()
        self._wg_flush()
        if self._side_on:
            torch.cuda.current_stream(dev).wait_stream(self.side)
            self._fork(1, 0)
            self._side_on = False

    def _wg(self, x, g, *args, **kw):
        self._wg_count += 1
        if _DEFER_REDUCE and "defer" not in kw:
            b = self.__dict__.get("_red_batch")
            if b is None:
                b = self.__dict__["_red_batch"] = ops.ReduceBatch(self.wws)
            kw["defer"] = b
        if not self._side_on or (_WG_MAIN_EVERY > 0 and self._wg_count % _WG_MAIN_EVERY == 0):
            return ops.wgrad(x, g, *args, **kw)
        ev = self._event()
        ev.record(self._main)
        self.side.wait_event(ev)
        self._fork(0, 1)
        ops.wgrad(x, g, *args, stream=self.side, **kw)
        x.record_stream(self.side)
        g.record_stream(self.side)

    def _event(self):
        i = self._ev_next
        if i == len(self._evs):
            self._evs.append(torch.cuda.Event())
        self._ev_next = i + 1
        return self._evs[i]

    def _bn_bwd(self, site: BNSite, ga, ga2, c, relu, G, cnt, red=None):
        if site.frozen:
            gc = self._new(c.shape, dtype=c.dtype, device=c.device)
            if red is None:
                red = self._red(2 * site.C, c.device)
                ops.bn_bwd_frozen(ga, ga2, c, site.scale, site.shift, site.mean, site.invstd, relu, red, gc)
            else:
                ops.bn_bwd_frozen(ga, ga2, c, site.scale, site.shift, site.mean, site.invstd, relu, None, gc)
            self._fin_later(red, site, G)
            return gc
        if red is None:
            red = self._red(2 * site.C, c.device)
            ops.bn_bwd_reduce(ga, ga2, c, site.scale, site.shift, site.mean, site.invstd, relu, red)
        gc = self._new(c.shape, dtype=c.dtype, device=c.device)
        if site.C <= _FIN_MAX_C:
            ops.bn_bwd_apply_fin(ga, ga2, c, site.scale, site.shift, site.mean, site.invstd, relu, red, cnt,
                                 G(site.mod.weight), G(site.mod.bias), gc)
            return gc
        k = self._new(2 * site.C, dtype=torch.float32, device=c.device)
        k1, k2 = k[:site.C], k[site.C:]
        ops.bn_bwd_finalize(red, cnt, site.C, G(site.mod.weight), G(site.mod.bias), False, k1, k2)
        ops.bn_bwd_apply(ga, ga2, c, site.scale, site.shift, site.mean, site.invstd, relu, k1, k2, gc)
        return gc

    def _conv_dgrad(self, conv_mod, g, gx, S, addend=None, k=3, addend_mask=None, bnb=None, stats=None):
        dt = g.dtype
        wp = self.packed(conv_mod.weight, dt, "dgrad")
        Cin = gx.shape[3]
        pad = k // 2
        if S == 1:
            taps = DG3 if k == 3 else (DG1 if k == 1 else DG7)
            ops.conv(g, wp, gx, taps, Cin, addend=addend, addend_mask=addend_mask, bnb=bnb, stats=stats)
        else:
            if k == 3 and Cin >= _PHASE_MIN_C and len(_PH3[0]) == 4 and addend_mask is None and bnb is None:
                ops.conv_phases(g, wp, _phase(gx, 0, 0), _PH3[1], Cin, phases=_PH3[0], y_full=gx, addend_full=addend)
                return
            for ry in range(2):
                for rx in range(2):
                    taps = ops.transposed_phase_taps(k, 1, pad, 2, ry, rx)
                    if not taps:
                        continue
                    yv = _phase(gx, ry, rx)
                    av = _phase(addend, ry, rx) if addend is not None else None
                    ops.conv(g, wp, yv, taps, Cin, addend=av)

    def block_bwd(self, rec, go, go2, G, need_gx=True):
        blk, x, c1, c2, cb, out = rec.blk, rec.x, rec.c1, rec.c2, rec.cb, rec.out
        dt, dev = c2.dtype, c2.device
        N, OH, OW, Cout = c2.shape
        cnt = N * OH * OW
        S = blk.stride
        bn1, bn2 = self.bn(blk.bn1), self.bn(blk.bn2)
        byp = cb is not None
        bnb = self.bn(blk.bnpass) if byp else None
        NS = L.STAT_SLOTS
        red = self._red((4 if byp else 2) * Cout, dev)
        red2 = red[:2 * Cout * NS]
        redb = red[2 * Cout * NS:] if byp else None
        mask = getattr(rec, "mask", None)
        nfrozen = int(bn2.frozen) + int(byp and bnb.frozen)
        onepass = mask is not None and nfrozen == (2 if byp else 1)
        fin = mask is not None and Cout <= _FIN_MAX_C and nfrozen == 0
        if not onepass:
            ops.block_tail_bwd_reduce(go, go2, out, c2, bn2.scale, bn2.shift, bn2.mean, bn2.invstd,
                                      cb, bnb.mean if byp else None, bnb.invstd if byp else None, red2, redb, relu_mask=mask)
        g_c2 = self._new(c2.shape, dtype=dt, device=dev)
        lazy_sc = _MASK_ADDEND and not byp and go2 is None and need_gx and (fin or onepass)
        g_sc = None if lazy_sc else self._new(c2.shape, dtype=dt, device=dev)
        if onepass:
            ops.block_tail_bwd_frozen(go, go2, mask, c2, bn2.scale, bn2.shift, bn2.mean, bn2.invstd, red2,
                                      cb, bnb.scale if byp else None, bnb.mean if byp else None, bnb.invstd if byp else None, redb, g_c2, g_sc)
            self._fin_later(red2, bn2, G)
            if byp:
                self._fin_later(redb, bnb, G)
        elif fin:
            ops.block_tail_bwd_apply_fin(go, go2, mask, c2, bn2.scale, bn2.shift, bn2.mean, bn2.invstd, red2, G(blk.bn2.weight), G(blk.bn2.bias),
                                         cb, bnb.scale if byp else None, bnb.mean if byp else None, bnb.invstd if byp else None,
                                         redb, G(blk.bnpass.weight) if byp else None, G(blk.bnpass.bias) if byp else None, cnt, g_c2, g_sc)
        else:
            k = self._new(4 * Cout, dtype=torch.float32, device=dev)
            if bn2.frozen:
                ops.bn_bwd_finalize_frozen(red2, Cout, G(blk.bn2.weight), G(blk.bn2.bias), k[:Cout], k[Cout:2 * Cout])
            else:
                ops.bn_bwd_finalize(red2, cnt, Cout, G(blk.bn2.weight), G(blk.bn2.bias), False, k[:Cout], k[Cout:2 * Cout])
            if byp and bnb.frozen:
                ops.bn_bwd_finalize_frozen(redb, Cout, G(blk.bnpass.weight), G(blk.bnpass.bias), k[2 * Cout:3 * Cout], k[3 * Cout:])
            elif byp:
                ops.bn_bwd_finalize(redb, cnt, Cout, G(blk.bnpass.weight), G(blk.bnpass.bias), False, k[2 * Cout:3 * Cout], k[3 * Cout:])
            ops.block_tail_bwd_apply(go, go2, out, c2, bn2.scale, bn2.shift, bn2.mean, bn2.invstd, k[:Cout], k[Cout:2 * Cout],
                                     cb, bnb.scale if byp else None, bnb.mean if byp else None, bnb.invstd if byp else None,
                                     k[2 * Cout:3 * Cout] if byp else None, k[3 * Cout:] if byp else None, g_c2, g_sc, relu_mask=mask)
        kk = 9
        if not _WG_AFTER:
            self._wg(c1, g_c2, T3, G(blk.conv2.weight), Cout * kk, kk, Cout, Cout, self.wws, xf=self.relu_affine(bn1))
        g_a1 = self._new(c1.shape, dtype=dt, device=dev)
        if _BNB_FUSE:
            red1 = self._red(2 * Cout, dev)
            self._conv_dgrad(blk.conv2, g_c2, g_a1, 1, bnb=(c1, bn1.mean, bn1.scale, bn1.shift, bn1.invstd), stats=red1)
            if _WG_AFTER:
                self._wg(c1, g_c2, T3, G(blk.conv2.weight), Cout * kk, kk, Cout, Cout, self.wws, xf=self.relu_affine(bn1))
            del g_c2
            g_c1 = self._bn_bwd(bn1, g_a1, None, c1, True, G, cnt, red=red1)
        else:
            self._conv_dgrad(blk.conv2, g_c2, g_a1, 1)
            if _WG_AFTER:
                self._wg(c1, g_c2, T3, G(blk.conv2.weight), Cout * kk, kk, Cout, Cout, self.wws, xf=self.relu_affine(bn1))
            del g_c2
            g_c1 = self._bn_bwd(bn1, g_a1, None, c1, True, G, cnt)
        del g_a1
        Cin = x.shape[3]

        def wg_conv1():
            self._wg(x, g_c1, T3, G(blk.conv1.weight), Cin * kk, kk, Cout, Cin, self.wws, S=S, xf=rec.xf_in)
            if byp:
                self._wg(x, g_sc, T1, G(blk.bypass.weight), Cin, 1, Cout, Cin, self.wws, S=S, xf=rec.xf_in)
        if not _WG_AFTER or not need_gx:
            wg_conv1()
        if not need_gx:
            return None
        gx = self._new(x.shape, dtype=dt, device=dev)
        if byp:
            self._conv_dgrad(blk.conv1, g_c1, gx, S)
            self._conv_dgrad(blk.bypass, g_sc, gx, S, addend=gx, k=1)
        elif lazy_sc:
            self._conv_dgrad(blk.conv1, g_c1, gx, S, addend=go, addend_mask=mask)
        else:
            self._conv_dgrad(blk.conv1, g_c1, gx, S, addend=g_sc)
        if _WG_AFTER:
            wg_conv1()
        return gx

    def double_fwd(self, dbl, x, out, training, dt, xf_in=None):
        N, H, W, _ = x.shape
        S = dbl.res1.stride
        mid = self._new((N, out.shape[1], out.shape[2], out.shape[3]), dtype=dt, device=x.device)
        r1 = self.block_fwd(dbl.res1, x, mid, training, dt, xf_in)
        r2 = self.block_fwd(dbl.res2, mid, out, training, dt)
        return (r1, r2) if self._save else None

    def double_bwd(self, recs, go, go2, G, need_gx=True):
        r1, r2 = recs
        g_mid = self.block_bwd(r2, go, go2, G)
        return self.block_bwd(r1, g_mid, None, G, need_gx)

    def deconv_fwd(self, dl, x, cat, Cd, dt, xf_x=None):
        wp = self.packed(dl.deconv.weight, dt, "tfwd")
        up = cat[..., :Cd]
        if Cd >= _PHASE_MIN_C and len(_PH4[0]) == 4:
            ops.conv_phases(x, wp, _phase(up, 0, 0), _PH4[1], Cd, phases=_PH4[0], y_full=up, xf=xf_x)
            return
        for ry in range(2):
            for rx in range(2):
                ops.conv(x, wp, _phase(up, ry, rx), ops.transposed_phase_taps(4, 1, 1, 2, ry, rx), Cd, xf=xf_x)

    def declayer_fwd(self, dl, x, cat, Cd, out, training, dt, xf_x=None, xf_cat=None):
        self.deconv_fwd(dl, x, cat, Cd, dt, xf_x)
        recs = self.double_fwd(dl.res, cat, out, training, dt, xf_cat)
        if not self._save:
            return None
        rec = Saved()
        rec.dl, rec.x, rec.cat, rec.Cd, rec.recs, rec.xf_x = dl, x, cat, Cd, recs, xf_x
        return rec

    def declayer_bwd(self, rec, go, G, xf_x: Optional[Affine] = None):
        dl, x, cat, Cd = rec.dl, rec.x, rec.cat, rec.Cd
        xf_x = rec.xf_x if xf_x is None else xf_x
        g_cat = self.double_bwd(rec.recs, go, None, G)
        g_up = g_cat[..., :Cd]
        Cin = x.shape[3]
        dW = G(dl.deconv.weight)
        for ry in range(2):
            for rx in range(2):
                taps = ops.transposed_phase_taps(4, 1, 1, 2, ry, rx)
                self._wg(x, _phase(g_up, ry, rx), taps, dW, 16, Cd * 16, Cd, Cin, self.wws, xf=xf_x)
        gx = self._new(x.shape, dtype=x.dtype, device=x.device)
        wp = self.packed(dl.deconv.weight, x.dtype, "tdgrad")
        ops.conv(g_up, wp, gx, ops.conv_taps(4, 1, 1), Cin, S=2)
        return gx, g_cat

    STEM_TAPS = [(ky - 3, 0, ky) for ky in range(7)]

    def stem_fwd(self, conv1, x, c0, stats, dt):
        N, Cin, H, W = x.shape
        Cout = conv1.out_channels
        x16 = self._new((N, H, W, 16 * Cin), dtype=dt, device=x.device)
        self._untaped(lambda: ops.stem_expand(x, x16))
        if self._rec is not None:
            self._rec.pre = lambda xx: ops.stem_expand(xx, x16)
        w = conv1.weight
        for ci in range(Cin):
            last = ci == Cin - 1
            ops.conv(x16[..., 16 * ci:16 * ci + 16], self.packed(w, dt, "stem%d" % ci), c0, self.STEM_TAPS, Cout,
                     bias=conv1.bias if ci == 0 else None, addend=c0 if ci > 0 else None, stats=stats if last else None)
        return x16

    def stem_bwd(self, conv1, x16, g_c0, G):
        Cout = conv1.out_channels
        Cin = x16.shape[3] // 16
        dW = G(conv1.weight)
        taps = [(ky - 3, 0, 7 * ky) for ky in range(7)]
        for ci in range(Cin):
            self._wg(x16[..., 16 * ci:16 * ci + 16], g_c0, taps, dW, Cin * 49, 1, Cout, 7, self.wws, dst_offset=ci * 49, exclusive=True)
        red = self._red(Cout, g_c0.device)
        ops.channel_sum(g_c0, red)
        ops.cast_f64_to_f32(red, G(conv1.bias), Cout)


    def head_fwd(self, m, d1o, training, dt):
        N, H, W, _ = d1o.shape
        bn10 = self.bn(m.bn10)
        nk = m.conv10.out_channels
        c10 = self._new((N, H, W, nk), dtype=dt, device=d1o.device)
        ops.conv(d1o, self.packed(m.conv10.weight, dt, "fwd"), c10, T7, nk, bias=m.conv10.bias, stats=bn10.stats)
        self._finish_bn(bn10, N * H * W, training)
        ncls = m.conv11.out_channels
        out = self._final_logsoftmax(m, c10, self.packed(m.conv11.weight, dt, "fwd"), self.relu_affine(bn10), (N, ncls, H, W))
        return c10, out

    def head_bwd(self, m, sv, g_logp, G):
        dt, dev = sv.dt, sv.x.device
        N, ncls, H, W = sv.out.shape
        ip = m.conv10.in_channels
        g_l = self._new((N, H, W, 16), dtype=dt, device=dev)
        self._logsoftmax_bwd(g_logp, sv.out, g_l)
        bn10 = self.bn(m.bn10)
        nk = m.conv10.out_channels
        self._wg(sv.c10, g_l, T7, G(m.conv11.weight), nk * 49, 49, ncls, nk, self.wws, xf=self.relu_affine(bn10))
        NS = L.STAT_SLOTS
        red = self._red(16 + nk, dev)
        ops.channel_sum(g_l, red[:16 * NS])
        ops.cast_f64_to_f32(red[:16 * NS], G(m.conv11.bias), ncls, stride=16)
        g_a10 = self._new((N, H, W, nk), dtype=dt, device=dev)
        red10 = self._red(2 * nk, dev) if _BNB_FUSE else None
        ops.conv(g_l, self._packed_dgrad_padded(m.conv11.weight, dt), g_a10, DG7, nk,
                 bnb=(sv.c10, bn10.mean, bn10.scale, bn10.shift, bn10.invstd) if _BNB_FUSE else None, stats=red10)
        del g_l
        g_c10 = self._bn_bwd(bn10, g_a10, None, sv.c10, True, G, N * H * W, red=red10)
        del g_a10
        self._wg(sv.d1o, g_c10, T7, G(m.conv10.weight), ip * 49, 49, nk, ip, self.wws)
        ops.channel_sum(g_c10, red[16 * NS:])
        ops.cast_f64_to_f32(red[16 * NS:], G(m.conv10.bias), nk)
        g = self._new(sv.d1o.shape, dtype=dt, device=dev)
        self._conv_dgrad(m.conv10, g_c10, g, 1, k=7)
        return g

    def _final_logsoftmax(self, m, c10, wp, xf, shape):
        def head():
            out = self._fresh(shape, dtype=torch.float32, device=c10.device)
            ops.conv(c10, wp, out, T7, shape[1], xf=xf, bias=m.conv11.bias, logsoftmax=True)
            return out
        if self._rec is not None:
            self._rec.post = head
        return self._untaped(head)

    def _logsoftmax_bwd(self, g_logp, out, g_l):
        self._untaped(lambda: ops.logsoftmax_bwd(g_logp, out, g_l))
        if self._rec is not None:
            self._rec.pre = lambda g, o: ops.logsoftmax_bwd(g, o, g_l)

    def _check_input(self, x, cin):
        L.require_cuda(x, "input")
        if x.dtype != torch.float32:
            raise RuntimeError("ubresnet_amd: input must be float32 NCHW (got %s)" % x.dtype)
        if x.dim() != 4 or x.shape[1] != cin:
            raise RuntimeError("ubresnet_amd: expected input [B,%d,H,W], got %s" % (cin, tuple(x.shape)))
        if x.shape[2] % 32 or x.shape[3] % 32:
            raise RuntimeError("ubresnet_amd: H and W must be multiples of 32 (ConvTranspose2d output_size contract of the "
                               "reference, models/common_layers.py:128); got %dx%d" % (x.shape[2], x.shape[3]))
        return x if x.is_contiguous() else x.contiguous()

    def _grad_views(self, dev):
        flat = self._new(self.grad_numel, dtype=torch.float32, device=dev)
        views = {}
        for name, p in self.grad_order:
# ... 586 lines not shown
```

ubresnet_amd/ops.py:

```python
from __future__ import annotations

import ctypes as C
from typing import List, Optional, Sequence, Tuple

import torch

from . import _lib as L

NEG_BIG = -3.0e38

_prof = None
_rec_sink = None


class LaunchProfiler:

    def __init__(self):
        self.records = []
        self.timed = []

    def summary(self, by="shape"):
        torch.cuda.synchronize()
        agg = {}
        for name, kern, sig, nbytes, flops, e0, e1 in self.records:
            k = (name, sig) if by == "shape" else kern
            a = agg.setdefault(k, [0, 0.0, 0, 0.0])
            a[0] += 1
            a[1] += e0.elapsed_time(e1) * 1e-3
            a[2] += nbytes
            a[3] += flops
        for name, kern, sig, nbytes, flops, sec in self.timed:
            k = (name, sig) if by == "shape" else kern
            a = agg.setdefault(k, [0, 0.0, 0, 0.0])
            a[0] += 1
            a[1] += sec
            a[2] += nbytes
            a[3] += flops
        return agg


_DT_NAME = {torch.float32: "float", torch.bfloat16: "bf16_t", torch.float16: "f16_t"}


def _act_bytes(args):
    n = 0
    for a in args:
        if isinstance(a, torch.Tensor) and a.dim() == 4:
            n += a.numel() * a.element_size()
    return n


def _timed(name):
    def deco(fn):
        def wrapper(*args, **kwargs):
            sink = _rec_sink
            if _prof is None and sink is None:
                return fn(*args, **kwargs)
            acts = [a for a in list(args) + list(kwargs.values()) if isinstance(a, torch.Tensor) and a.dim() == 4]
            sig = " ".join("x".join(map(str, a.shape)) for a in acts[:3])
            taps = kwargs.get("taps", args[3] if name in ("conv",) and len(args) > 3 else (args[2] if name == "wgrad" and len(args) > 2 else None))
            ntaps = len(taps) if isinstance(taps, (list, tuple)) else 0
            if ntaps:
                sig += " taps%d" % ntaps
            if "S" in kwargs:
                sig += " S%d" % kwargs["S"]
            lab = sink.label_begin() if sink is not None else -1
            if _prof is not None:
                e0, e1 = torch.cuda.Event(enable_timing=True), torch.cuda.Event(enable_timing=True)
                e0.record()
            r = fn(*args, **kwargs)
            if _prof is not None:
                e1.record()
            kern, flops = name, 0.0
            if name == "conv":
                x, wp, y = args[0], args[1], args[2]
                cout = args[4]
                npix = y.shape[0] * (y.shape[2] * y.shape[3] if y.shape[1] == cout and y.dtype == torch.float32 and kwargs.get("logsoftmax") else y.shape[1] * y.shape[2])
                flops = 2.0 * npix * x.shape[3] * cout * ntaps
                buf = C.create_string_buffer(160)
                L.lib().ubr_conv_last_kernel(buf, 160)
                kern = buf.value.decode()
            if sink is not None:
                sink.label_end(lab, (name, kern, sig, _act_bytes(acts), flops))
            if _prof is not None:
                _prof.records.append((name, kern, sig, _act_bytes(acts), flops, e0, e1))
            return r
        wrapper.__name__ = fn.__name__
        wrapper.__doc__ = fn.__doc__
        wrapper.__wrapped__ = fn
        return wrapper
    return deco


def last_conv_kernel() -> str:
    buf = C.create_string_buffer(160)
    L.lib().ubr_conv_last_kernel(buf, 160)
    return buf.value.decode()


def _tv(t: Optional[torch.Tensor]) -> L.Tensor:
    if t is None:
        return L.Tensor(None, 0, 0, 0)
    assert t.dim() == 4 and t.stride(3) == 1, "NHWC view with contiguous channels expected"
    return L.Tensor(t.data_ptr(), t.stride(0), t.stride(1), t.stride(2))


def _ps(t: torch.Tensor) -> int:
    n, h, w, c = t.shape
    ps = t.stride(2)
    if not (t.stride(3) == 1 and t.stride(1) == w * ps and (n == 1 or t.stride(0) == h * w * ps)):
        raise RuntimeError("ubresnet_amd: expected a pixel-dense NHWC view, got shape %s strides %s" % (tuple(t.shape), t.stride()))
    return ps


class Affine:
    __slots__ = ("sub", "scale", "shift", "lo")

    def __init__(self, sub, scale, shift, lo):
        self.sub, self.scale, self.shift, self.lo = sub, scale, shift, lo

    def c(self) -> L.ChanAffine:
        return L.ChanAffine(self.sub.data_ptr(), self.scale.data_ptr(), self.shift.data_ptr(), self.lo.data_ptr())


def _xf(a: Optional[Affine]) -> L.ChanAffine:
    return a.c() if a is not None else L.ChanAffine(None, None, None, None)


def conv_taps(k: int, dil: int, pad: int) -> List[Tuple[int, int, int]]:
    return [(ky * dil - pad, kx * dil - pad, ky * k + kx) for ky in range(k) for kx in range(k)]


def conv_dgrad_taps_s1(k: int, dil: int, pad: int):
    return [(pad - ky * dil, pad - kx * dil, ky * k + kx) for ky in range(k) for kx in range(k)]


def transposed_phase_taps(k: int, dil: int, pad: int, s: int, ry: int, rx: int):
    out = []
    for ky in range(k):
        if (ry + pad - ky * dil) % s:
            continue
        for kx in range(k):
            if (rx + pad - kx * dil) % s:
                continue
            out.append(((ry + pad - ky * dil) // s, (rx + pad - kx * dil) // s, ky * k + kx))
    return out


@_timed("pack_weights")
def pack_weights(src: torch.Tensor, dtype: torch.dtype, M: int, K: int, sm: int, sk: int, ntaps: int,
                 tapidx: Optional[Sequence[int]] = None, Kpad: Optional[int] = None, src_offset: int = 0) -> torch.Tensor:
    L.require_cuda(src, "weights")
    assert src.dtype == torch.float32 and src.is_contiguous()
    cpu = L.chans_per_unit(dtype)
    Mpad = (M + 15) // 16 * 16
    if Kpad is None:
        Kpad = (K + cpu - 1) // cpu * cpu
    dst = torch.empty((ntaps, Kpad // cpu, Mpad, cpu), dtype=dtype, device=src.device)
    idx = (C.c_int32 * ntaps)(*(tapidx if tapidx is not None else range(ntaps)))
    L.check(L.lib().ubr_pack_weights(L.dtype_id(dtype), src.data_ptr() + 4 * src_offset, dst.data_ptr(), M, Mpad, K, Kpad, sm, sk,
                                     ntaps, idx, L.stream_ptr()), "pack_weights")
    return dst


_TAP_CACHE = {}


def _tap_arrays(taps):
    key = tuple(taps)
    r = _TAP_CACHE.get(key)
    if r is None:
        n = len(key)
        r = ((C.c_int8 * n)(*[t[0] for t in key]), (C.c_int8 * n)(*[t[1] for t in key]), (C.c_uint8 * n)(*[t[2] for t in key]),
             max(t[2] for t in key))
        _TAP_CACHE[key] = r
    return r


@_timed("conv")
def conv(x: torch.Tensor, wp: torch.Tensor, y: torch.Tensor, taps, Cout: int, S: int = 1, iy0: int = 0, ix0: int = 0,
         xf: Optional[Affine] = None, bias: Optional[torch.Tensor] = None, addend: Optional[torch.Tensor] = None,
         stats: Optional[torch.Tensor] = None, logsoftmax: bool = False, tile_hint: int = 0, in_hw=None, act: int = 0,
         addend_mask: Optional[torch.Tensor] = None, bnb=None, stats_slots: int = 0):
    d = L.ConvDesc()
    d.dtype = L.dtype_id(x.dtype)
    N, H, W, Cin = x.shape
    d.N, d.H, d.W, d.Cin = N, H, W, Cin
    d.x = _tv(x)
    d.xf = _xf(xf)
    d.w = wp.data_ptr()
    d.Cout, d.Cout_pad = Cout, wp.shape[2]
    if wp.shape[1] * wp.shape[3] != Cin:
        raise RuntimeError("conv: packed weights expect %d input channels, tensor has %d" % (wp.shape[1] * wp.shape[3], Cin))
    d.ntaps = len(taps)
    if not 1 <= len(taps) <= L.MAX_TAPS:
        raise RuntimeError("conv: %d taps unsupported" % len(taps))
    dy_a, dx_a, wt_a, wt_max = _tap_arrays(taps)
    C.memmove(d.dy, dy_a, len(taps)); C.memmove(d.dx, dx_a, len(taps)); C.memmove(d.wt, wt_a, len(taps))
    if wt_max >= wp.shape[0]:
        raise RuntimeError("conv: tap index %d outside packed image" % wt_max)
    d.S, d.iy0, d.ix0 = S, iy0, ix0
    if logsoftmax:
        assert y.dtype == torch.float32 and y.is_contiguous() and y.shape[1] == Cout
        d.OH, d.OW = y.shape[2], y.shape[3]
        d.y = L.Tensor(y.data_ptr(), 0, 0, 0)
        d.epilogue = 1
        if y.shape[0] != N:
            raise RuntimeError("conv: batch mismatch")
    else:
        assert y.dtype == x.dtype
        d.OH, d.OW = y.shape[1], y.shape[2]
        d.y = _tv(y)
        d.epilogue = 0
        if y.shape[0] != N or y.shape[3] != Cout:
            raise RuntimeError("conv: output view %s does not match N=%d Cout=%d" % (tuple(y.shape), N, Cout))
    if addend is not None:
        assert addend.shape == y.shape and addend.dtype == y.dtype
        d.addend = _tv(addend)
    d.bias = L.ptr(bias)
    d.stats = L.ptr(stats)
    if stats is not None:
        assert stats.dtype == torch.float64 and stats.numel() >= 2 * Cout * L.STAT_SLOTS
    if bias is not None:
        assert bias.dtype == torch.float32 and bias.numel() >= Cout
    if xf is not None:
        assert xf.scale.numel() >= Cin
    d.tile_hint = tile_hint
    d.act = act
    d.stats_slots = stats_slots
    if addend_mask is not None:
        assert addend is not None and addend_mask.dtype == torch.uint8 and addend_mask.is_contiguous()
        assert addend_mask.numel() >= y.shape[0] * y.shape[1] * y.shape[2] * (Cout // L.chans_per_unit(x.dtype))
        d.addend_mask = addend_mask.data_ptr()
    if bnb is not None:
        cten, mean, scale, shift, invstd = bnb
        assert stats is not None and cten.shape == y.shape and cten.dtype == y.dtype
        d.bnb_c = _tv(cten)
        d.bnb_mean, d.bnb_scale, d.bnb_shift, d.bnb_invstd = mean.data_ptr(), scale.data_ptr(), shift.data_ptr(), invstd.data_ptr()
    L.check(L.lib().ubr_conv(C.byref(d), L.stream_ptr()), "conv")


@_timed("conv")
def conv_phases(x: torch.Tensor, wp: torch.Tensor, y0: torch.Tensor, taps, Cout: int, phases=None, y_full: torch.Tensor = None,
                addend_full: Optional[torch.Tensor] = None, xf: Optional[Affine] = None, bias: Optional[torch.Tensor] = None):
    d = L.ConvDesc()
    d.dtype = L.dtype_id(x.dtype)
    N, H, W, Cin = x.shape
    d.N, d.H, d.W, d.Cin = N, H, W, Cin
    d.x = _tv(x)
    d.xf = _xf(xf)
    d.w = wp.data_ptr()
    d.Cout, d.Cout_pad = Cout, wp.shape[2]
    if wp.shape[1] * wp.shape[3] != Cin:
        raise RuntimeError("conv: packed weights expect %d input channels, tensor has %d" % (wp.shape[1] * wp.shape[3], Cin))
    if not 1 <= len(taps) <= L.MAX_TAPS or not 2 <= len(phases) <= 4:
        raise RuntimeError("conv_phases: %d taps / %d phases unsupported" % (len(taps), len(phases)))
    dy_a, dx_a, wt_a, wt_max = _tap_arrays(taps)
    C.memmove(d.dy, dy_a, len(taps)); C.memmove(d.dx, dx_a, len(taps)); C.memmove(d.wt, wt_a, len(taps))
    if wt_max >= wp.shape[0]:
        raise RuntimeError("conv: tap index %d outside packed image" % wt_max)
    d.ntaps = len(taps)
    d.S, d.iy0, d.ix0 = 1, 0, 0
    assert y_full.dtype == x.dtype and y_full.shape[0] == N and y_full.shape[3] == Cout and y_full.shape[1] % 2 == 0 and y_full.shape[2] % 2 == 0
    d.OH, d.OW = y_full.shape[1] // 2, y_full.shape[2] // 2
    sn, sy, sx = y_full.stride(0), y_full.stride(1), y_full.stride(2)
    d.y = L.Tensor(y_full.data_ptr(), sn, 2 * sy, 2 * sx)
    if addend_full is not None:
        assert addend_full.shape == y_full.shape and addend_full.dtype == y_full.dtype and addend_full.stride(3) == 1
        an, ay, ax = addend_full.stride(0), addend_full.stride(1), addend_full.stride(2)
        d.addend = L.Tensor(addend_full.data_ptr(), an, 2 * ay, 2 * ax)
    d.bias = L.ptr(bias)
    d.nphase = len(phases)
    t0 = 0
    for i, (ry, rx, tp) in enumerate(phases):
        d.phase_tap0[i], d.phase_ntaps[i] = t0, len(tp)
        t0 += len(tp)
        d.phase_yoff[i] = ry * sy + rx * sx
        d.phase_aoff[i] = (ry * ay + rx * ax) if addend_full is not None else 0
    assert t0 == len(taps)
    L.check(L.lib().ubr_conv(C.byref(d), L.stream_ptr()), "conv (phased)")


class WgradWorkspace:

    def __init__(self):
        self.buf = None
        self.pin = False
        self.old = []

    def get(self, nbytes: int, device) -> torch.Tensor:
        n = (nbytes + 3) // 4
        if self.buf is None or self.buf.numel() < n or self.buf.device != device:
            if self.pin and self.buf is not None:
                self.old.append(self.buf)
            self.buf = torch.empty(max(n, 1 << 20), dtype=torch.float32, device=device)
        return self.buf

    def hold(self, nbytes: int, device, stream=None) -> torch.Tensor:
        n = ((nbytes + 3) // 4 + 63) // 64 * 64
        key = 0 if stream is None else stream.cuda_stream
        ar = self.__dict__.setdefault("_arenas", {})
        a = ar.get(key)
        if a is None or a[0].device != device or a[1] + n > a[0].numel():
            if a is not None:
                self.__dict__.setdefault("_arena_old", []).append(a[0])
            a = ar[key] = [torch.empty(max(2 * n, 64 << 20), dtype=torch.float32, device=device), 0]
        t = a[0][a[1]:a[1] + n]
        a[1] += n
        return t

    def release(self, stream=None):
        a = self.__dict__.get("_arenas", {}).get(0 if stream is None else stream.cuda_stream)
        if a is not None:
            a[1] = 0
        if not self.pin:
            self.__dict__.get("_arena_old", []).clear()


class ReduceBatch:

    def __init__(self, ws: "WgradWorkspace"):
        self.ws = ws
        self.items = []
        self.stream = None

    def add(self, item, nbytes, stream):
        assert not self.items or stream is self.stream, "a batch belongs to one stream"
        self.stream = stream
        self.items.append((item, nbytes))

    def flush(self):
        if not self.items:
            return
        lib = L.lib()
        stream = self.stream
        st = L.stream_ptr() if stream is None else stream.cuda_stream
        sink = _rec_sink
        for lo in range(0, len(self.items), L.REDUCE_BATCH):
            chunk = self.items[lo:lo + L.REDUCE_BATCH]
            arr = (L.WgradReduceItem * len(chunk))(*[c[0] for c in chunk])
            if _prof is not None:
                e0, e1 = torch.cuda.Event(enable_timing=True), torch.cuda.Event(enable_timing=True)
                e0.record(stream)
            lab = sink.label_begin() if sink is not None else -1
            L.check(lib.ubr_wgrad_reduce_batched(arr, len(chunk), st), "wgrad_reduce_batched")
            meta = ("wgrad_reduce", "wgrad_reduce_batched_kernel", "%d weight gradients" % len(chunk), sum(c[1] for c in chunk), 0.0)
            if sink is not None:
                sink.label_end(lab, meta)
            if _prof is not None:
                e1.record(stream)
                _prof.records.append(meta + (e0, e1))
        self.items = []
        self.ws.release(stream)


_TAP_CACHE_W = {}


def _tap_arrays_w(taps):
    key = tuple(taps)
    r = _TAP_CACHE_W.get(key)
    if r is None:
        n = len(key)
        r = ((C.c_int8 * n)(*[t[0] for t in key]), (C.c_int8 * n)(*[t[1] for t in key]), (C.c_int32 * n)(*[t[2] for t in key]), n)
        _TAP_CACHE_W[key] = r
    return r


def wgrad(x: torch.Tensor, g: torch.Tensor, taps, dst: torch.Tensor, sm: int, sk: int, Cout_valid: int, Cin_valid: int,
          ws: WgradWorkspace, S: int = 1, iy0: int = 0, ix0: int = 0, xf: Optional[Affine] = None, accumulate: bool = False,
          dst_offset: int = 0, stream=None, exclusive: bool = False, defer: Optional["ReduceBatch"] = None):
    if defer is not None and (accumulate or (defer.items and defer.stream is not stream)):
        defer.flush()
        if accumulate:
            defer = None
    d = L.WgradDesc()
    d.dtype = L.dtype_id(x.dtype)
    N, H, W, Cin = x.shape
    d.N, d.H, d.W, d.Cin = N, H, W, Cin
    d.x = _tv(x)
    d.xf = _xf(xf)
    assert g.dtype == x.dtype and g.shape[0] == N
    d.GH, d.GW, d.Cout = g.shape[1], g.shape[2], g.shape[3]
    d.g = _tv(g)
    d.ntaps = len(taps)
    dy_a, dx_a, _, _ = _tap_arrays_w(taps)
    C.memmove(d.dy, dy_a, len(taps)); C.memmove(d.dx, dx_a, len(taps))
    d.S, d.iy0, d.ix0 = S, iy0, ix0
    d.exclusive = 1 if exclusive else 0
    nsplit, nbytes = C.c_int32(0), C.c_int64(0)
    lib = L.lib()
    L.check(lib.ubr_wgrad_plan(C.byref(d), C.byref(nsplit), C.byref(nbytes)), "wgrad_plan")
    slabs = ws.get(nbytes.value, x.device) if defer is None else ws.hold(nbytes.value, x.device, stream)
    if stream is not None:
        slabs.record_stream(stream)
    d.slabs = slabs.data_ptr()
    d.nsplit = nsplit.value
    st = L.stream_ptr() if stream is None else stream.cuda_stream
    sink = _rec_sink
    if _prof is not None:
        e0, e1, e2 = (torch.cuda.Event(enable_timing=True) for _ in range(3))
        e0.record(stream)
    lab0 = sink.label_begin() if sink is not None else -1
    L.check(lib.ubr_wgrad(C.byref(d), st), "wgrad")
    if _prof is not None:
        e1.record(stream)
    idx = _tap_arrays_w(taps)[2]
    assert dst.dtype == torch.float32
    lab1 = -1
    if defer is not None:
        it = L.WgradReduceItem()
        it.slabs, it.dst = slabs.data_ptr(), dst.data_ptr() + 4 * dst_offset
        it.nsplit, it.ntaps, it.Cout_pad, it.Cin, it.Cout_valid, it.Cin_valid = nsplit.value, len(taps), d.Cout, Cin, Cout_valid, Cin_valid
        it.accumulate, it.sm, it.sk = 1 if accumulate else 0, sm, sk
        for i in range(len(taps)):
            it.tapidx[i] = idx[i]
        defer.add(it, nsplit.value * len(taps) * d.Cout * Cin * 4, stream)
    else:
        lab1 = sink.label_begin() if sink is not None else -1
        L.check(lib.ubr_wgrad_reduce(slabs.data_ptr(), nsplit.value, len(taps), d.Cout, Cin, Cout_valid, Cin_valid,
                                     dst.data_ptr() + 4 * dst_offset, sm, sk, idx, 1 if accumulate else 0, st), "wgrad_reduce")
    if _prof is not None or sink is not None:
        if _prof is not None and defer is None:
            e2.record(stream)
        a, b, c, dd, bx = C.c_int(0), C.c_int(0), C.c_int(0), C.c_int(0), C.c_int(0)
        lib.ubr_wgrad_last_config(C.byref(a), C.byref(b), C.byref(c), C.byref(dd), C.byref(bx))
        kern = "wgrad_kernel<%s, %d, %d, %d, %s, %s, %s>" % (_DT_NAME[x.dtype], a.value, b.value, c.value, "true" if dd.value else "false",
                                                             "true" if bx.value else "false", "true" if lib.ubr_wgrad_last_pc() else "false")
        sig = "%s %s taps%d S%d" % ("x".join(map(str, x.shape)), "x".join(map(str, g.shape)), len(taps), S)
        nbytes = (x.numel() + g.numel()) * x.element_size()
        flops = 2.0 * g.shape[0] * g.shape[1] * g.shape[2] * g.shape[3] * Cin * len(taps)
        red = ("wgrad_reduce", "wgrad_reduce_kernel", sig, nsplit.value * len(taps) * d.Cout * Cin * 4, 0.0)
        if sink is not None:
# ... 265 lines not shown
```

Measured before the change: 1400 images/sec.

## Fuse conv1 and bypass data-gradient convs into one two-source thin kernel

Adds a two-source variant of the thin conv kernel (EXT==3). It accumulates the 3x3 conv1 data-gradient and the 1x1 bypass data-gradient into the same output tile, so the residual block backward no longer launches two convs or reads gx back as an addend. The second source is staged in extra LDS rows and its weights are appended to the linear weight stream. Eligibility is narrow (bf16, Cout 32, UPB 2, stride 1, one tile config) and falls back to the two-launch path otherwise. The extra LDS may lower occupancy.

```diff
diff --git a/include/ubresnet_hip.h b/include/ubresnet_hip.h
--- a/include/ubresnet_hip.h
+++ b/include/ubresnet_hip.h
@@ -63,6 +63,16 @@
 } ubr_conv_desc;
 
 int ubr_conv(const ubr_conv_desc* d, void* stream);
+
+typedef struct {
+  ubr_conv_desc conv;
+  ubr_tensor x2;
+  const void* w2;
+  int32_t Cin2;
+  int32_t pad_;
+} ubr_conv_dual_desc;
+int ubr_conv_dual(const ubr_conv_dual_desc* d, void* stream);
+int ubr_conv_dual_supported(const ubr_conv_dual_desc* d);
 void ubr_conv_last_config(int* fw, int* nt, int* twf, int* pipe);
 int ubr_conv_last_kernel(char* buf, int n);
 
diff --git a/ubresnet_amd/_lib.py b/ubresnet_amd/_lib.py
--- a/ubresnet_amd/_lib.py
+++ b/ubresnet_amd/_lib.py
@@ -67,6 +67,10 @@
     ]
 
 
+class ConvDualDesc(C.Structure):
+    _fields_ = [("conv", ConvDesc), ("x2", Tensor), ("w2", C.c_void_p), ("Cin2", C.c_int32), ("pad_", C.c_int32)]
+
+
 class AsppFrontDesc(C.Structure):
     _fields_ = [
         ("dtype", C.c_int32),
@@ -119,7 +123,7 @@
 
 
 SYMBOLS = [
-    "ubr_conv", "ubr_conv_last_config", "ubr_conv_last_kernel", "ubr_pack_weights", "ubr_pack_weights_batched", "ubr_bn_fold_batched", "ubr_aspp_front", "ubr_wgrad_plan", "ubr_wgrad", "ubr_wgrad_last_config", "ubr_wgrad_last_pc", "ubr_wgrad_reduce", "ubr_wgrad_reduce_batched",
+    "ubr_conv", "ubr_conv_dual", "ubr_conv_dual_supported", "ubr_conv_last_config", "ubr_conv_last_kernel", "ubr_pack_weights", "ubr_pack_weights_batched", "ubr_bn_fold_batched", "ubr_aspp_front", "ubr_wgrad_plan", "ubr_wgrad", "ubr_wgrad_last_config", "ubr_wgrad_last_pc", "ubr_wgrad_reduce", "ubr_wgrad_reduce_batched",
     "ubr_stem_forward", "ubr_stem_wgrad", "ubr_stem_wgrad_workspace", "ubr_stem_expand",
     "ubr_bn_finalize", "ubr_bn_eval_affine", "ubr_bn_bwd_reduce", "ubr_bn_bwd_finalize", "ubr_bn_bwd_apply",
     "ubr_block_tail_fwd", "ubr_block_tail_bwd_reduce", "ubr_block_tail_bwd_apply",
@@ -144,6 +148,8 @@
     lib.ubr_stem_wgrad_workspace.restype = C.c_int64
     lib.ubr_stem_wgrad_workspace.argtypes = [i32] * 5
     lib.ubr_conv.argtypes = [C.POINTER(ConvDesc), vp]
+    lib.ubr_conv_dual.argtypes = [C.POINTER(ConvDualDesc), vp]
+    lib.ubr_conv_dual_supported.argtypes = [C.POINTER(ConvDualDesc)]
     lib.ubr_conv_last_config.argtypes = [C.POINTER(C.c_int)] * 4
     lib.ubr_conv_last_kernel.argtypes = [C.c_char_p, i32]
     lib.ubr_conv_last_config.restype = None
diff --git a/ubresnet_amd/csrc/ubr_conv.hip b/ubresnet_amd/csrc/ubr_conv.hip
--- a/ubresnet_amd/csrc/ubr_conv.hip
+++ b/ubresnet_amd/csrc/ubr_conv.hip
@@ -39,6 +39,9 @@
   int8_t dy[UBR_MAX_TAPS], dx[UBR_MAX_TAPS];
   uint8_t wt[UBR_MAX_TAPS];
   unsigned long long* stamps;
+  const char* x2; long x2_sn, x2_sy, x2_sx;
+  const char* w2;
+  int nunits2;
 };
 
 template <typename T> __device__ __forceinline__ void store4(char* p, const float* v);
@@ -719,6 +722,8 @@
   const float *bmean, *bscale, *bshift, *binvstd;
   int nslots;
   int nphase, pstep0[4], psteps[4], pyoff[4];
+  const char* x2; long x2_sn; int x2_sy, x2_sx; unsigned x2_bytes;
+  const char* w2; int nunits2, c2_off;
 };
 
 
@@ -726,6 +731,7 @@
 __global__ __launch_bounds__(256, ((ROW7 || (EXT == 1 && NT == 2)) ? 2 : 3)) void conv_thin_kernel(const ThinK k) {
   ubr_main_prio();
   static_assert(EXT == 0 || (!XF && !LSM), "the training epilogues belong to the data-gradient convs (no transform on load, NHWC output)");
+  static_assert(EXT != 3 || !ROW7, "the two-source form runs the generic tap loop");
   constexpr int TN = NT * 16;
   constexpr int TH = 4 * FW / TWF;
   constexpr int TW = TWF * 16;
@@ -740,6 +746,9 @@
   static_assert(TWF == 2 && FW % FH == 0, "tile shape");
   static_assert(!ROW7 || (FW == 8 && NT == 1 && UPB == 2), "ROW7 is the 16x32-pixel, 16-cout, 16-cin tile");
   constexpr bool WIDE = ESZ == 2;
+  constexpr int HS2 = EXT == 3 ? (TH * TW * UPB) / 256 : 1;
+  constexpr int RPS2 = PPS / TW;
+  static_assert(EXT != 3 || (PPS % TW == 0 && (TH * TW * UPB) % 256 == 0), "second-source slots cover whole tile rows");
 
   extern __shared__ __attribute__((aligned(16))) char smem[];
   int* tbl = reinterpret_cast<int*>(smem);
@@ -764,8 +773,13 @@
     if constexpr (XF) hyu[u] = hy;
   }
   char* const halo_w = halo + (tid >> LG) * PIXB + c * 16;
+  const int rowb = k.HW * PIXB;
+  const int row2 = (tid >> LG) / TW, col2 = (tid >> LG) % TW;
+  const int rel2 = EXT == 3 ? row2 * k.x2_sy + col2 * k.x2_sx + c * 16 : 0;
+  char* const halo2_w = halo + k.c2_off + (row2 * k.HW + col2) * PIXB + c * 16;
 
   ubr_u4 hv[HS];
+  ubr_u4 hv2[HS2];
   unsigned hok = 0u;
   auto load_halo = [&](int tile) {
     const unsigned t = (unsigned)__builtin_amdgcn_readfirstlane(tile);
@@ -783,20 +797,30 @@
       hv[u] = __builtin_amdgcn_raw_buffer_load_b128(xr, vo, 0, 0);
       if constexpr (XF) hok |= (unsigned)(ok & ((unsigned)(hy0 + hyu[u]) < (unsigned)k.H)) << u;
     }
+    if constexpr (EXT == 3) {
+      __amdgpu_buffer_rsrc_t x2r = __builtin_amdgcn_make_buffer_rsrc((void*)(k.x2 + (long)n * k.x2_sn), 0, (int)k.x2_bytes, 0x00020000);
+      const int goff2 = (int)ty * TH * k.x2_sy + (int)tx * TW * k.x2_sx;
+#pragma unroll
+      for (int u = 0; u < HS2; ++u) hv2[u] = __builtin_amdgcn_raw_buffer_load_b128(x2r, rel2 + u * RPS2 * k.x2_sy, goff2, 0);
+    }
   };
 
   const int ntiles = k.ntiles;
   int tile = blockIdx.x;
   load_halo(tile);
   uint4 wv[WB];
+  auto wlin = [&](int i) -> uint4 {
+    const int nvalid = k.nunits * TN;
+    uint4 v = make_uint4(0u, 0u, 0u, 0u);
+    if (i < nvalid) v = ldg16(k.w + (long)i * 16);
+    if constexpr (EXT == 3) {
+      if (i >= nvalid && i < nvalid + k.nunits2 * TN) v = ldg16(k.w2 + (long)(i - nvalid) * 16);
+    }
+    return v;
+  };
   if (k.wlinear) {
-    const int nvalid = k.nunits * TN;
-#pragma unroll
-    for (int u = 0; u < WB; ++u) {
-      const int i = tid + u * 256;
-      wv[u] = make_uint4(0u, 0u, 0u, 0u);
-      if (i < nvalid) wv[u] = ldg16(k.w + (long)i * 16);
-    }
+#pragma unroll
+    for (int u = 0; u < WB; ++u) wv[u] = wlin(tid + u * 256);
   }
   float bs[NT][4];
 #pragma unroll
@@ -828,6 +852,8 @@
       const int tap = u >> LG, cc = u & (UPB - 1);
       off = ((k.dy[tap] - k.dymin) * k.HW + (k.dx[tap] - k.dxmin)) * PIXB + cc * 16;
       v = k.wt[tap] == 255 ? -1 : ((int)k.wt[tap] * k.CU + cc) * k.Cout_pad;
+    } else if constexpr (EXT == 3) {
+      if (u < k.nunits + k.nunits2) off = k.c2_off + (u - k.nunits) * 16;
     }
     tbl[u] = off;
     wsrc[u] = v;
@@ -838,14 +864,9 @@
       const int i = tid + u * 256;
       if (i < nw) *reinterpret_cast<uint4*>(wl + (long)i * 16) = wv[u];
     }
-    const int nvalid = k.nunits * TN;
     for (int ib = tid + 256 * WB; ib < nw; ib += 256 * WB) {
 #pragma unroll
-      for (int u = 0; u < WB; ++u) {
-        const int i = ib + u * 256;
-        wv[u] = make_uint4(0u, 0u, 0u, 0u);
-        if (i < nvalid) wv[u] = ldg16(k.w + (long)i * 16);
-      }
+      for (int u = 0; u < WB; ++u) wv[u] = wlin(ib + u * 256);
 #pragma unroll
       for (int u = 0; u < WB; ++u) {
         const int i = ib + u * 256;
@@ -874,7 +895,6 @@
 
   if constexpr (XF || EXT == 1) __syncthreads();
   const int fb0 = (((wave * FW) / TWF) * k.HW + l16) * PIXB;
-  const int rowb = k.HW * PIXB;
   int vo_out[NT];
 #pragma unroll
   for (int j = 0; j < NT; ++j) {
@@ -931,6 +951,10 @@
         }
       }
       if (tid + u * 256 < k.nitems) *reinterpret_cast<uint4*>(halo_w + u * (PPS * PIXB)) = v;
+    }
+    if constexpr (EXT == 3) {
+#pragma unroll
+      for (int u = 0; u < HS2; ++u) *reinterpret_cast<uint4*>(halo2_w + u * RPS2 * rowb) = __builtin_bit_cast(uint4, hv2[u]);
     }
     UBR_TSTAMP(tS);
     __syncthreads();
@@ -1751,8 +1775,14 @@
   k.Cout = c.Cout; k.Cout_pad = c.Cout_pad; k.CU = c.CU; k.OH = c.OH; k.OW = c.OW;
   k.act = c.act; k.epilogue = c.epilogue; k.wlinear = nph > 1 ? 0 : c.wlinear; k.dbg = c.dbg; k.stamps = c.stamps;
   for (int t = 0; t < c.ntaps; ++t) { k.dy[t] = c.dy[t]; k.dx[t] = c.dx[t]; k.wt[t] = c.wt[t]; }
-  const int ext = c.bc != nullptr ? 1 : (c.ad_mask != nullptr ? 2 : 0);
+  const int ext = c.bc != nullptr ? 1 : (c.ad_mask != nullptr ? 2 : (c.x2 != nullptr ? 3 : 0));
   if (ext != 0 && (c.in_scale != nullptr || c.epilogue != 0)) return 0;
+  if (ext == 3) {
+    if (!(FW == 4 && NT == 2 && sizeof(T) == 2) || c.UPB != 2 || nph > 1 || row7 || c.stats != nullptr || !c.wlinear || c.nunits2 != c.UPB) return 0;
+    if (c.x2_sy >= (1L << 24) || (long)c.OH * c.x2_sy >= (1L << 31)) return 0;
+    k.x2 = c.x2; k.x2_sn = c.x2_sn; k.x2_sy = (int)c.x2_sy; k.x2_sx = (int)c.x2_sx; k.x2_bytes = (unsigned)((long)c.OH * c.x2_sy);
+    k.w2 = c.w2; k.nunits2 = c.nunits2;
+  }
   k.nslots = c.nslots;
   if (ext == 1) {
     if (c.bc_sy >= (1L << 24) || (long)c.OH * c.bc_sy >= (1L << 31)) return 0;
@@ -1775,6 +1805,7 @@
   size_t off = ((size_t)2 * 16 * k.steps + 15) & ~(size_t)15;
   k.wl_off = (int)off; off += (size_t)4 * k.steps * TN * 16;
   k.halo_off = (int)off; off += ((size_t)c.HH * c.HW * pixb + 15) & ~(size_t)15;
+  if (ext == 3) { k.c2_off = (int)off - k.halo_off; off += ((size_t)TH * c.HW * pixb + 15) & ~(size_t)15; }
   k.red_off = (int)off; off += (size_t)4 * TN * 2 * sizeof(float) + (size_t)4 * 4 * 8 * sizeof(float);
   const size_t lds = off;
   if (lds > 150 * 1024) return 0;
@@ -1818,6 +1849,10 @@
   }
   if (ext == 1) *rc = c.UPB == 2 ? launch_thin<T, FW, NT, TWF, 2, false, false, false, 1>(k, g, lds, st) : launch_thin<T, FW, NT, TWF, 4, false, false, false, 1>(k, g, lds, st);
   else if (ext == 2) *rc = c.UPB == 2 ? launch_thin<T, FW, NT, TWF, 2, false, false, false, 2>(k, g, lds, st) : launch_thin<T, FW, NT, TWF, 4, false, false, false, 2>(k, g, lds, st);
+  else if (ext == 3) {
+    if constexpr (FW == 4 && NT == 2 && sizeof(T) == 2) *rc = launch_thin<T, FW, NT, TWF, 2, false, false, false, 3>(k, g, lds, st);
+    else return 0;
+  }
   else if (c.UPB == 2) *rc = xf ? launch_thin<T, FW, NT, TWF, 2, true>(k, g, lds, st) : launch_thin<T, FW, NT, TWF, 2, false>(k, g, lds, st);
   else *rc = xf ? launch_thin<T, FW, NT, TWF, 4, true>(k, g, lds, st) : launch_thin<T, FW, NT, TWF, 4, false>(k, g, lds, st);
   return 1;
@@ -1828,6 +1863,10 @@
   if constexpr (NT <= 2 && TWF == 2) {
     int rc = UBR_OK;
     if (try_thin<T, FW, NT, TWF>(k, grid, st, &rc)) return rc;
+  }
+  if (k.x2 != nullptr) {
+    ubr_set_error("ubr_conv_dual: no kernel serves this two-source shape");
+    return UBR_EINVAL;
   }
   if constexpr (NT == 4) {
     static const bool enabled = [] { const char* e = getenv("UBR_CONV_PIPE"); return !e || atoi(e) != 0; }();
@@ -1902,14 +1941,14 @@
   return m;
 }
 
-static bool plan_tile(const ubr_conv_desc* d, int cfg, int TH, int TW, int TN, int dymin, int dymax, int dxmin, int dxmax, Plan* p) {
+static bool plan_tile(const ubr_conv_desc* d, int cfg, int TH, int TW, int TN, int dymin, int dymax, int dxmin, int dxmax, Plan* p, bool dual = false) {
   if (d->Cout_pad % TN) return false;
   if (d->epilogue == 1 && TN != 16) return false;
   const int cpu = ubr_cpu(d->dtype);
   const int CU = d->Cin / cpu;
   int UPB = (CU % 4 == 0) ? 4 : (CU % 2 == 0 ? 2 : 1);
   if (UPB == 4 && (d->S == 2 || eff_ntaps(d) >= 16)) UPB = 2;
-  const int nunits = eff_ntaps(d) * UPB;
+  const int nunits = eff_ntaps(d) * UPB + (dual ? UPB : 0);
   const int steps = (nunits + 3) / 4;
   const int HH = (TH - 1) * d->S + 1 + (dymax - dymin);
   const int HW = (TW - 1) * d->S + 1 + (dxmax - dxmin);
@@ -1918,6 +1957,7 @@
   p->wl_off = (int)off; off += (size_t)4 * steps * TN * 16;
   p->halo_off = (int)off; off += (size_t)HH * HW * pixb;
   off = (off + 15) & ~(size_t)15;
+  if (dual) off += ((size_t)TH * HW * pixb + 15) & ~(size_t)15;
   p->red_off = (int)off; off += (size_t)4 * TN * 2 * sizeof(float);
   p->xfc_off = (int)off;
   if (d->xf.scale != nullptr && CU / UPB >= 2) off += (size_t)d->Cin * 4 * sizeof(float);
@@ -1927,9 +1967,9 @@
   return off <= 160 * 1024;
 }
 
-static bool plan_for(const ubr_conv_desc* d, int cfg, int dymin, int dymax, int dxmin, int dxmax, Plan* p) {
+static bool plan_for(const ubr_conv_desc* d, int cfg, int dymin, int dymax, int dxmin, int dxmax, Plan* p, bool dual = false) {
   const TileCfg& c = kCfgs[cfg];
-  return plan_tile(d, cfg, 4 * c.FW / c.TWF, c.TWF * 16, c.NT * 16, dymin, dymax, dxmin, dxmax, p);
+  return plan_tile(d, cfg, 4 * c.FW / c.TWF, c.TWF * 16, c.NT * 16, dymin, dymax, dxmin, dxmax, p, dual);
 }
 
 struct PcCfg { int FW, TWF; };
@@ -1983,7 +2023,7 @@
   if (pipe) *pipe = g_last_conv_cfg[3];
 }
 
-static bool thin_eligible(const ubr_conv_desc* d, int cfg, const Plan& p, bool wide_ok) {
+static bool thin_eligible(const ubr_conv_desc* d, int cfg, const Plan& p, bool wide_ok, const ubr_conv_dual_desc* dual = nullptr) {
   static const bool thin_on = [] { const char* e = getenv("UBR_CONV_THIN"); return !e || atoi(e) != 0; }();
   const TileCfg& c = kCfgs[cfg];
   if (!thin_on || c.TWF != 2 || c.NT > 2 || (c.FW % 4)) return false;
@@ -1991,6 +2031,18 @@
   const int CU = d->Cin / cpu, TH = 4 * c.FW / c.TWF, TW = c.TWF * 16;
   if (p.UPB != CU || d->S != 1 || (p.UPB != 2 && p.UPB != 4)) return false;
   if (d->OH % TH || d->OW % TW) return false;
+  if (dual != nullptr) {
+    static const bool dual_on = [] { const char* e = getenv("UBR_THIN_DUAL"); return !e || atoi(e) != 0; }();
+    if (!dual_on || cfg != 2 || esz != 2 || p.UPB != 2 || d->Cout_pad != c.NT * 16 || d->nphase > 1 || d->stats != nullptr) return false;
+    for (int t = 0; t < d->ntaps; ++t) if (d->wt[t] != t) return false;
+    const long e = esz;
+    if (d->x.sy * e >= (1L << 24) || d->y.sy * e >= (1L << 24) || dual->x2.sy * e >= (1L << 24) || (long)d->H * d->x.sy * e >= (1L << 31) ||
+        (long)d->OH * d->y.sy * e >= (1L << 31) || (long)d->OH * dual->x2.sy * e >= (1L << 31)) return false;
+    if (d->addend.p != nullptr && (d->addend.sy * e >= (1L << 24) || (long)d->OH * d->addend.sy * e >= (1L << 31))) return false;
+    if ((unsigned long long)p.tiles_x * p.tiles_y * d->N * (unsigned)p.tiles_x >= (1ull << 32)) return false;
+    size_t lds = (size_t)p.lds + (size_t)4 * 4 * 8 * sizeof(float);
+    if (lds > 150 * 1024) return false;
+  }
   if (d->nphase > 1) {
     static const bool ph_on = [] { const char* e = getenv("UBR_THIN_PHASES"); return !e || atoi(e) != 0; }();
     if (!ph_on || d->addend.p != nullptr || d->stats != nullptr || d->epilogue != 0) return false;
@@ -2009,7 +2061,7 @@
   return d->Cout % 4 == 0;
 }
 
-extern "C" int ubr_conv(const ubr_conv_desc* d, void* stream) {
+static int conv_run(const ubr_conv_desc* d, const ubr_conv_dual_desc* dual, void* stream, bool plan_only) {
   UBR_CHECK(d != nullptr, "ubr_conv: null descriptor");
   UBR_CHECK(ubr_dtype_ok(d->dtype), "ubr_conv: bad dtype %d", d->dtype);
   const int cpu = ubr_cpu(d->dtype), esz = ubr_esize(d->dtype);
@@ -2050,6 +2102,15 @@
   }
   const bool train_epi = d->addend_mask != nullptr || d->bnb_c.p != nullptr;
   const int nphase = d->nphase > 1 ? d->nphase : 1;
+  if (dual != nullptr) {
+    UBR_CHECK(dual->x2.p && dual->w2 && ubr_aligned16(dual->x2.p) && ubr_aligned16(dual->w2), "ubr_conv_dual: x2 / w2 must be non-null and 16-byte aligned");
+    UBR_CHECK((dual->x2.sx * esz) % 16 == 0 && (dual->x2.sy * esz) % 16 == 0 && (dual->x2.sn * esz) % 16 == 0 && dual->x2.sx >= dual->Cin2,
+              "ubr_conv_dual: x2 strides must keep 16-byte alignment and hold Cin2 channels");
+    UBR_CHECK(dual->Cin2 > 0 && dual->Cin2 % cpu == 0, "ubr_conv_dual: Cin2=%d must be a positive multiple of %d", dual->Cin2, cpu);
+    UBR_CHECK(d->epilogue == 0 && !xf && !train_epi && d->tile_hint == 0 && d->act == 0,
+              "ubr_conv_dual: NHWC output; no transform on load, activation, training epilogue or tile hint");
+    UBR_CHECK(d->S == 1 && d->iy0 == 0 && d->ix0 == 0 && d->H == d->OH && d->W == d->OW, "ubr_conv_dual: source 1 and the output share one grid (stride 1)");
+  }
   if (nphase > 1) {
     UBR_CHECK(nphase <= 4 && d->epilogue == 0 && !train_epi && d->stats == nullptr, "ubr_conv: a phased launch takes 2..4 phases, NHWC output, no statistics or training epilogue");
     int covered = 0;
@@ -2078,6 +2139,11 @@
     UBR_CHECK(d->tile_hint <= kNumCfgs, "ubr_conv: tile_hint %d out of range", d->tile_hint);
     have = plan_for(d, d->tile_hint - 1, dymin, dymax, dxmin, dxmax, &best);
     UBR_CHECK(have, "ubr_conv: tile_hint %d does not fit this shape", d->tile_hint);
+  } else if (dual != nullptr) {
+    Plan p{};
+    if (dual->Cin2 == d->Cin && d->Cout_pad == 32 && plan_for(d, 2, dymin, dymax, dxmin, dxmax, &p, true) && thin_eligible(d, 2, p, wide_ok, dual)) { best = p; have = true; }
+    if (plan_only) return have ? 1 : 0;
+    UBR_CHECK(have, "ubr_conv_dual: no kernel serves this two-source shape (ask ubr_conv_dual_supported first)");
   } else {
     const int order_by_nt[3][4] = {{3, 4, 5, -1}, {2, 6, 8, -1}, {0, 1, 7, 9}};
     {
@@ -2136,6 +2202,10 @@
   k.ad_mask = d->addend_mask; k.ad_mask_cu = d->Cout / cpu;
   k.bc = (const char*)d->bnb_c.p; k.bc_sn = d->bnb_c.sn * esz; k.bc_sy = d->bnb_c.sy * esz; k.bc_sx = d->bnb_c.sx * esz;
   k.bmean = d->bnb_mean; k.bscale = d->bnb_scale; k.bshift = d->bnb_shift; k.binvstd = d->bnb_invstd;
+  if (dual != nullptr) {
+    k.x2 = (const char*)dual->x2.p; k.x2_sn = dual->x2.sn * esz; k.x2_sy = dual->x2.sy * esz; k.x2_sx = dual->x2.sx * esz;
+    k.w2 = (const char*)dual->w2; k.nunits2 = dual->Cin2 / cpu;
+  }
   UBR_CHECK(d->stats_slots == 0 || d->stats_slots == UBR_RED_SLOTS || d->stats_slots == UBR_STAT_SLOTS, "ubr_conv: stats_slots must be 0, %d or %d", UBR_RED_SLOTS, UBR_STAT_SLOTS);
   k.nslots = (d->bnb_c.p != nullptr || d->stats_slots == UBR_RED_SLOTS) ? UBR_RED_SLOTS : UBR_STAT_SLOTS;
   k.H = d->H; k.W = d->W;
@@ -2220,6 +2290,18 @@
     }
     return rc;
   }
+}
+
+extern "C" int ubr_conv(const ubr_conv_desc* d, void* stream) { return conv_run(d, nullptr, stream, false); }
+
+extern "C" int ubr_conv_dual(const ubr_conv_dual_desc* d, void* stream) {
+  UBR_CHECK(d != nullptr, "ubr_conv_dual: null descriptor");
+  return conv_run(&d->conv, d, stream, false);
+}
+
+extern "C" int ubr_conv_dual_supported(const ubr_conv_dual_desc* d) {
+  UBR_CHECK(d != nullptr, "ubr_conv_dual_supported: null descriptor");
+  return conv_run(&d->conv, d, nullptr, true);
 }
 
 namespace {
diff --git a/ubresnet_amd/engine.py b/ubresnet_amd/engine.py
--- a/ubresnet_amd/engine.py
+++ b/ubresnet_amd/engine.py
@@ -77,6 +77,8 @@
         self._rec = None
         self._planned: Dict[tuple, object] = {}
         self.wws.pin = True
+        self._dual_dgrad = _os.environ.get("UBR_DUAL_DGRAD", "1") != "0"
+        self._dual_ok: Dict[tuple, bool] = {}
         self.bn_sites: List[BNSite] = []
         self._bn_of: Dict[int, BNSite] = {}
         for m in model.modules():
@@ -452,6 +454,21 @@
                     yv = _phase(gx, ry, rx)
                     av = _phase(addend, ry, rx) if addend is not None else None
                     ops.conv(g, wp, yv, taps, Cin, addend=av)
+
+    def _dgrad_dual(self, blk, g_c1, g_sc, gx, S) -> bool:
+        if not self._dual_dgrad or S != 1:
+            return False
+        dt = g_c1.dtype
+        w1, wb = self.packed(blk.conv1.weight, dt, "dgrad"), self.packed(blk.bypass.weight, dt, "dgrad")
+        Cin = gx.shape[3]
+        key = (dt, tuple(g_c1.shape), g_c1.stride(), g_sc.stride(), gx.stride(), Cin, g_c1.data_ptr() % 16, g_sc.data_ptr() % 16, gx.data_ptr() % 16)
+        ok = self._dual_ok.get(key)
+        if ok is None:
+            ok = self._dual_ok[key] = ops.conv_dual_supported(g_c1, w1, gx, DG3, Cin, g_sc, wb)
+        if not ok:
+            return False
+        ops.conv_dual(g_c1, w1, gx, DG3, Cin, g_sc, wb)
+        return True
 
     def block_bwd(self, rec, go, go2, G, need_gx=True):
         blk, x, c1, c2, cb, out = rec.blk, rec.x, rec.c1, rec.c2, rec.cb, rec.out
@@ -528,7 +545,9 @@
         if not need_gx:
             return None
         gx = self._new(x.shape, dtype=dt, device=dev)
-        if byp:
+        if byp and self._dgrad_dual(blk, g_c1, g_sc, gx, S):
+            pass
+        elif byp:
             self._conv_dgrad(blk.conv1, g_c1, gx, S)
             self._conv_dgrad(blk.bypass, g_sc, gx, S, addend=gx, k=1)
         elif lazy_sc:
diff --git a/ubresnet_amd/ops.py b/ubresnet_amd/ops.py
--- a/ubresnet_amd/ops.py
+++ b/ubresnet_amd/ops.py
@@ -58,7 +58,7 @@
                 return fn(*args, **kwargs)
             acts = [a for a in list(args) + list(kwargs.values()) if isinstance(a, torch.Tensor) and a.dim() == 4]
             sig = " ".join("x".join(map(str, a.shape)) for a in acts[:3])
-            taps = kwargs.get("taps", args[3] if name in ("conv",) and len(args) > 3 else (args[2] if name == "wgrad" and len(args) > 2 else None))
+            taps = kwargs.get("taps", args[3] if name in ("conv", "conv_dual") and len(args) > 3 else (args[2] if name == "wgrad" and len(args) > 2 else None))
             ntaps = len(taps) if isinstance(taps, (list, tuple)) else 0
             if ntaps:
                 sig += " taps%d" % ntaps
@@ -72,11 +72,13 @@
             if _prof is not None:
                 e1.record()
             kern, flops = name, 0.0
-            if name == "conv":
+            if name in ("conv", "conv_dual"):
                 x, wp, y = args[0], args[1], args[2]
                 cout = args[4]
                 npix = y.shape[0] * (y.shape[2] * y.shape[3] if y.shape[1] == cout and y.dtype == torch.float32 and kwargs.get("logsoftmax") else y.shape[1] * y.shape[2])
                 flops = 2.0 * npix * x.shape[3] * cout * ntaps
+                if name == "conv_dual":
+                    flops += 2.0 * npix * args[5].shape[3] * cout
                 buf = C.create_string_buffer(160)
                 L.lib().ubr_conv_last_kernel(buf, 160)
                 kern = buf.value.decode()
@@ -279,6 +281,52 @@
         d.phase_aoff[i] = (ry * ay + rx * ax) if addend_full is not None else 0
     assert t0 == len(taps)
     L.check(L.lib().ubr_conv(C.byref(d), L.stream_ptr()), "conv (phased)")
+
+
+def _dual_desc(x, wp, y, taps, Cout, x2, wp2, addend):
+    d = L.ConvDualDesc()
+    cd = d.conv
+    cd.dtype = L.dtype_id(x.dtype)
+    N, H, W, Cin = x.shape
+    cd.N, cd.H, cd.W, cd.Cin = N, H, W, Cin
+    cd.x = _tv(x)
+    cd.w = wp.data_ptr()
+    cd.Cout, cd.Cout_pad = Cout, wp.shape[2]
+    if wp.shape[1] * wp.shape[3] != Cin or wp2.shape[1] * wp2.shape[3] != x2.shape[3] or wp2.shape[2] != wp.shape[2] or wp2.shape[0] != 1:
+        raise RuntimeError("conv_dual: packed images %s / %s do not match Cin=%d, Cin2=%d" % (tuple(wp.shape), tuple(wp2.shape), Cin, x2.shape[3]))
+    if not 1 <= len(taps) <= L.MAX_TAPS:
+        raise RuntimeError("conv_dual: %d taps unsupported" % len(taps))
+    dy_a, dx_a, wt_a, wt_max = _tap_arrays(taps)
+    C.memmove(cd.dy, dy_a, len(taps)); C.memmove(cd.dx, dx_a, len(taps)); C.memmove(cd.wt, wt_a, len(taps))
+    if wt_max >= wp.shape[0]:
+        raise RuntimeError("conv_dual: tap index %d outside packed image" % wt_max)
+    cd.ntaps = len(taps)
+    cd.S, cd.iy0, cd.ix0 = 1, 0, 0
+    if y.dtype != x.dtype or x2.dtype != x.dtype or tuple(y.shape) != (N, H, W, Cout) or tuple(x2.shape[:3]) != (N, H, W):
+        raise RuntimeError("conv_dual: x %s, x2 %s and y %s must share dtype, batch and grid" % (tuple(x.shape), tuple(x2.shape), tuple(y.shape)))
+    cd.OH, cd.OW = H, W
+    cd.y = _tv(y)
+    if addend is not None:
+        assert addend.shape == y.shape and addend.dtype == y.dtype
+        cd.addend = _tv(addend)
+    d.x2 = _tv(x2)
+    d.w2 = wp2.data_ptr()
+    d.Cin2 = x2.shape[3]
+    return d
+
+
+def conv_dual_supported(x: torch.Tensor, wp: torch.Tensor, y: torch.Tensor, taps, Cout: int, x2: torch.Tensor, wp2: torch.Tensor,
+                        addend: Optional[torch.Tensor] = None) -> bool:
+    r = L.lib().ubr_conv_dual_supported(C.byref(_dual_desc(x, wp, y, taps, Cout, x2, wp2, addend)))
+    if r < 0:
+        L.check(r, "conv_dual_supported")
+    return r == 1
+
+
+@_timed("conv_dual")
+def conv_dual(x: torch.Tensor, wp: torch.Tensor, y: torch.Tensor, taps, Cout: int, x2: torch.Tensor, wp2: torch.Tensor,
+              addend: Optional[torch.Tensor] = None):
+    L.check(L.lib().ubr_conv_dual(C.byref(_dual_desc(x, wp, y, taps, Cout, x2, wp2, addend)), L.stream_ptr()), "conv_dual")
 
 
 class WgradWorkspace:
```

Result: no change. 1411 images/sec (median of 6 runs) (+0.8%).
